# UofgCoastline/EUSIPCO-2026-Robust-Unet

Measured on AMD Instinct MI355X. Metric: train images/sec Robust U-Net 256x256 bs16/GPU, higher is better.
Workload: dtype f32; 1 GPU; Robust U-Net base64 (40.9M params) train step, 256x256 RGB+mask tiles, batch 16/GPU, fp32, BCE + Adam(lr 1e-4, wd 1e-4), dropout + batch-stat BN on; global_batch=16, image_size=256, parallelism=dp1

## Files before the change

eusipco-2026-robust-unet_amd/blocks.py:

```python
from __future__ import annotations

import os

import torch

from . import ops
from ._lib import check, lib

BN_EPS = 1e-5
BN_MOMENTUM = 0.1


class Small:

    CHUNK = 1 << 16

    def __init__(self, device):
        self.device = device
        self.buf = None
        self.off = 0

    def _take(self, n, dtype):
        n4 = (n + 3) // 4 * 4
        if n4 > self.CHUNK:
# ... 38 lines not shown

    def __init__(self, device):
        self.device = device
        self.g = {}

    def buf(self, prefix, items):
        total = sum(_numel(sh) for _, sh in items)
        flat = torch.empty(total, device=self.device, dtype=torch.float32)
        off = 0
        for name, sh in items:
            n = _numel(sh)
            self.g[prefix + name] = flat[off:off + n].view(sh)
            off += n
        return flat


def _numel(shape):
    n = 1
    for d in shape:
        n *= d
    return n


class BNState:
    __slots__ = ("weight", "bias", "running_mean", "running_var", "nbt")

    def __init__(self, weight, bias, running_mean, running_var, nbt):
        self.weight, self.bias, self.running_mean, self.running_var, self.nbt = weight, bias, running_mean, running_var, nbt


FUSED_BN_STATS = os.environ.get("RUNET_BN_STATS_3", "0") != "1"


def bn_coeff(x, bn: BNState, training, sm: Small, want_minmax=False, stats_hook=None, fused=None):
    n, h, w, c = x.shape
    hw = h * w
    st = ops.stream()
    scale, shift, mean, invstd = sm.f(c), sm.f(c), sm.f(c), sm.f(c)
    nc = None
    if training and not want_minmax and stats_hook is None and FUSED_BN_STATS and fused and "part" in fused:
        check(lib.runet_bn_stats_finalize(fused["part"].data_ptr(), fused["nparts"], c, bn.weight.data_ptr(), bn.bias.data_ptr(),
                                          bn.running_mean.data_ptr(), bn.running_var.data_ptr(), bn.nbt.data_ptr(), BN_MOMENTUM, BN_EPS,
                                          scale.data_ptr(), shift.data_ptr(), mean.data_ptr(), invstd.data_ptr(), st))
        return scale, shift, mean, invstd, None
    if training and not want_minmax and stats_hook is None and FUSED_BN_STATS:
        check(lib.runet_bn_stats(x.data_ptr(), ops.ld(x), n, hw, c, _ws(n, hw, c, x.device).data_ptr(), bn.weight.data_ptr(), bn.bias.data_ptr(),
                                 bn.running_mean.data_ptr(), bn.running_var.data_ptr(), bn.nbt.data_ptr(), BN_MOMENTUM, BN_EPS,
                                 scale.data_ptr(), shift.data_ptr(), mean.data_ptr(), invstd.data_ptr(), st))
        return scale, shift, mean, invstd, None
    if training or want_minmax:
        mean_nc, m2_nc = sm.f(n * c), sm.f(n * c)
        if want_minmax:
            max_nc, min_nc, imax, imin = sm.f(n * c), sm.f(n * c), sm.i(n * c), sm.i(n * c)
            nc = (mean_nc, m2_nc, max_nc, min_nc, imax, imin)
        ws = _ws(n, hw, c, x.device)
        check(lib.runet_chan_stats(x.data_ptr(), ops.ld(x), n, hw, c, ws.data_ptr(), mean_nc.data_ptr(), m2_nc.data_ptr(),
                                   nc[2].data_ptr() if nc else None, nc[3].data_ptr() if nc else None,
                                   nc[4].data_ptr() if nc else None, nc[5].data_ptr() if nc else None, int(want_minmax), st))
        mean_all, m2_all, n_eff = mean_nc, m2_nc, n
        if stats_hook is not None and training:
            mean_all, m2_all, n_eff = stats_hook.gather_stats(mean_nc, m2_nc, n, c)
    if training:
        check(lib.runet_bn_finalize(mean_all.data_ptr(), m2_all.data_ptr(), n_eff, c, hw, bn.weight.data_ptr(), bn.bias.data_ptr(),
                                    bn.running_mean.data_ptr(), bn.running_var.data_ptr(), bn.nbt.data_ptr(), BN_MOMENTUM, BN_EPS, 1,
                                    scale.data_ptr(), shift.data_ptr(), mean.data_ptr(), invstd.data_ptr(), st))
    else:
        check(lib.runet_bn_finalize(None, None, n, c, hw, bn.weight.data_ptr(), bn.bias.data_ptr(), bn.running_mean.data_ptr(),
                                    bn.running_var.data_ptr(), None, BN_MOMENTUM, BN_EPS, 0, scale.data_ptr(), shift.data_ptr(),
                                    mean.data_ptr(), invstd.data_ptr(), st))
    return scale, shift, mean, invstd, nc


def bn_coeff_pair(xa, bna: BNState, xb, bnb: BNState, training, sm: Small, stats_hook=None):
    if stats_hook is None or not training:
        return bn_coeff(xa, bna, training, sm)[:4], bn_coeff(xb, bnb, training, sm)[:4]
    st = ops.stream()
    local = []
    for x in (xa, xb):
        n, h, w, c = x.shape
        mean_nc, m2_nc = sm.f(n * c), sm.f(n * c)
        check(lib.runet_chan_stats(x.data_ptr(), ops.ld(x), n, h * w, c, _ws(n, h * w, c, x.device).data_ptr(), mean_nc.data_ptr(), m2_nc.data_ptr(),
                                   None, None, None, None, 0, st))
        local.append((mean_nc, m2_nc, n, c))
    res = []
    for x, bn, (mean_all, m2_all, n_eff) in zip((xa, xb), (bna, bnb), stats_hook.gather_stats_many(local)):
        n, h, w, c = x.shape
        scale, shift, mean, invstd = sm.f(c), sm.f(c), sm.f(c), sm.f(c)
        check(lib.runet_bn_finalize(mean_all.data_ptr(), m2_all.data_ptr(), n_eff, c, h * w, bn.weight.data_ptr(), bn.bias.data_ptr(),
                                    bn.running_mean.data_ptr(), bn.running_var.data_ptr(), bn.nbt.data_ptr(), BN_MOMENTUM, BN_EPS, 1,
                                    scale.data_ptr(), shift.data_ptr(), mean.data_ptr(), invstd.data_ptr(), st))
        res.append((scale, shift, mean, invstd))
    return res[0], res[1]


def bn_apply(x, scale, shift, mask=None, relu=False, out=None):
    n, h, w, c = x.shape
    if out is None:
        out = ops.empty_nhwc(n, h, w, c, x)
    check(lib.runet_bn_apply(x.data_ptr(), ops.ld(x), out.data_ptr(), ops.ld(out), n * h * w, h * w, c, scale.data_ptr(), shift.data_ptr(),
                             mask.data_ptr() if mask is not None else None, int(relu), ops.stream()))
    return out


def bn_bwd_reduce(dy, x, mean, invstd, scale, sums, act=None, mask=None, relu_shift=None):
    n, h, w, c = x.shape
    hw = h * w
    if relu_shift is not None:
        act = None
    actp, lda = (act.data_ptr(), ops.ld(act)) if act is not None else (None, 0)
    rsc, rsh = (scale.data_ptr(), relu_shift.data_ptr()) if relu_shift is not None else (None, None)
    check(lib.runet_bn_bwd_reduce(dy.data_ptr(), ops.ld(dy), x.data_ptr(), ops.ld(x), actp, lda, n, hw, c, mean.data_ptr(), invstd.data_ptr(),
                                  mask.data_ptr() if mask is not None else None, _ws(n, hw, c, x.device).data_ptr(), sums.data_ptr(), rsc, rsh,
                                  ops.stream()))


def bn_bwd_apply(dy, x, mean, invstd, scale, use, m_total, act=None, mask=None, out=None, relu_shift=None):
    n, h, w, c = x.shape
    hw = h * w
    if relu_shift is not None:
        act = None
    actp, lda = (act.data_ptr(), ops.ld(act)) if act is not None else (None, 0)
    if out is None:
        out = ops.empty_nhwc(n, h, w, c, x)
    check(lib.runet_bn_bwd_apply(dy.data_ptr(), ops.ld(dy), x.data_ptr(), ops.ld(x), actp, lda, out.data_ptr(), ops.ld(out), n * hw, hw, c,
                                 mean.data_ptr(), invstd.data_ptr(), scale.data_ptr(), use.data_ptr(), mask.data_ptr() if mask is not None else None,
                                 m_total, relu_shift.data_ptr() if relu_shift is not None else None, ops.stream()))
    return out


def dx_sums(sums, training, sync=None, count=0):
    if not training:
        return zeros(sums.numel(), sums.device), 0
    return (sums, 0) if sync is None else sync.reduce_sums(sums, count)


def bn_backward(dy, x, mean, invstd, scale, sums, act=None, mask=None, out=None, sync=None, relu_shift=None, training=True):
    n, h, w, c = x.shape
    bn_bwd_reduce(dy, x, mean, invstd, scale, sums, act, mask, relu_shift)
    use, m_total = dx_sums(sums, training, sync, n * h * w)
    return bn_bwd_apply(dy, x, mean, invstd, scale, use, m_total, act, mask, out, relu_shift)


CHAN_SUM_ON_SIDE = os.environ.get("RUNET_CHAN_SUM_MAIN", "0") != "1"
FUSED_SHORTCUT_BN_SUMS = os.environ.get("RUNET_FUSED_SHORTCUT_BN_SUMS", "0") == "1"
FUSED_GATE_BN_SUMS = os.environ.get("RUNET_NO_FUSED_GATE_BN_SUMS", "0") != "1"
FUSED_RB_EDGES = os.environ.get("RUNET_NO_FUSED_RB_EDGES", "0") != "1"
RB_EDGE_PARTS = frozenset(("out", "bwd1", "bwd3"))


def _edge(part):
    return FUSED_RB_EDGES and part in RB_EDGE_PARTS


def chan_sum(x, out):
    n, h, w, c = x.shape

    def run():
        ws = _ws(n, h * w, c, x.device)
        check(lib.runet_chan_sum(x.data_ptr(), ops.ld(x), n * h * w, c, ws.data_ptr(), out.data_ptr(), 0, ops.stream()))
        return out
    if CHAN_SUM_ON_SIDE and ops.side_stream() is not None:
        return ops._on_side(run, (x, out))
    return run()


def vec(n, device):
    return torch.empty(n, device=device, dtype=torch.float32)


def _ptr(t):
    return t.data_ptr() if t is not None else None


def conv_bn_coeff(x, w, bias, bn: BNState, training, sm: Small, stride=1, stats=True, save=True):
    fs = None
    if stride == 1:
        fs = {} if (stats and training) else None
        t = ops.conv_fwd(x, w, bias, stats=fs)
    else:
        t = ops.conv_general_fwd(x, w, bias, stride, w.shape[0] // 2)
    s, h, mean, invstd, _ = bn_coeff(t, bn, training, sm, fused=fs)
    return t, s, h, (dict(x=x, w=w, t=t, s=s, h=h, mean=mean, invstd=invstd, stride=stride) if save else None)


def conv_bn_relu_forward(x, w, bias, bn: BNState, training, sm: Small, stride=1, stats=True, save=True, out=None):
    t, s, h, cx = conv_bn_coeff(x, w, bias, bn, training, sm, stride, stats, save)
    return bn_apply(t, s, h, None, relu=True, out=out), cx


def conv_bn_relu_backward(cx, dy, G, seq, i, training, out=None):
    k, _, cin_w, c = cx["w"].shape
    sums = vec(2 * c, dy.device)
    dt = bn_backward(dy, cx["t"], cx["mean"], cx["invstd"], cx["s"], sums, relu_shift=cx["h"], out=out, training=training)
    G[f"{seq}.{i + 1}.weight"], G[f"{seq}.{i + 1}.bias"] = sums[:c], sums[c:]
    if cx["stride"] == 1:
        G[f"{seq}.{i}.weight"] = ops.conv_wgrad(cx["x"], dt, k, k, cin_w=cin_w)
    else:
        G[f"{seq}.{i}.weight"] = ops.conv_general_wgrad(cx["x"], dt, k, k, cx["stride"], k // 2, cin_w=cin_w)
    G[f"{seq}.{i}.bias"] = chan_sum(dt, vec(c, dy.device))
    return dt


class RBParams:
    __slots__ = ("w1", "bn1", "w2", "bn2", "w0p", "w2p", "wsa", "ws", "bns", "cin_w")

    def __init__(self, w1, bn1, w2, bn2, w0p, w2p, wsa, ws=None, bns=None):
        self.w1, self.bn1, self.w2, self.bn2, self.w0p, self.w2p, self.wsa, self.ws, self.bns = w1, bn1, w2, bn2, w0p, w2p, wsa, ws, bns
        self.cin_w = w1.shape[2]


def rb_forward(x, p: RBParams, training, mask=None, save=True, stats_hook=None, pool=False):
    n, h, w, _ = x.shape
    c = p.w1.shape[3]
    cr = p.w0p.shape[3]
    hw, P = h * w, n * h * w
    st = ops.stream()
    sm = Small(x.device)
    kv1, kv2 = ({}, {}) if save else (None, None)
    t1, br, fstem = None, None, (None, None)
    if p.ws is not None:
        if ops._stem_case(x.shape[3], p.cin_w, c, 3) and p.ws.shape[2] == p.cin_w:
            fstem = ({}, {}) if (training and stats_hook is None) else (None, None)
            t1, r = ops.stem_conv(x, p.w1, p.ws, stats3=fstem[0], stats1=fstem[1])
            if stats_hook is None:
                ss, hs, mean_s, invstd_s, _ = bn_coeff(r, p.bns, training, sm, fused=fstem[1])
        elif stats_hook is not None:
            r = ops.conv_fwd(x, p.ws)
        else:
            sm.f(4)
            r = ops.main_pool(ops.empty_nhwc(n, h, w, c, x))
            br = ops.side_branch(stats_hook is None)
            with br:
                fs = {} if training else None
                ops.conv_fwd(x, p.ws, out=r, stats=fs)
                ss, hs, mean_s, invstd_s, _ = bn_coeff(r, p.bns, training, sm, fused=fs)
    else:
        r, ss, hs, mean_s, invstd_s = x, None, None, None, None
    f1 = {} if (training and stats_hook is None) else None
    if t1 is None:
        t1 = ops.conv_fwd(x, p.w1, keep_v=kv1, stats=f1)
    elif fstem[0]:
        f1 = fstem[0]
    if p.ws is not None and stats_hook is not None:
        (ss, hs, mean_s, invstd_s), (s1, h1, mean1, invstd1) = bn_coeff_pair(r, p.bns, t1, p.bn1, training, sm, stats_hook)
    else:
        s1, h1, mean1, invstd1, _ = bn_coeff(t1, p.bn1, training, sm, stats_hook=stats_hook, fused=f1)
    use_mask = mask if training else None
    if ops.fuses_act_input(t1, p.w2):
        a1 = None
        t2 = ops.conv_fwd(t1, p.w2, keep_v=kv2, pre=(s1, h1, use_mask))
    else:
        a1 = bn_apply(t1, s1, h1, use_mask, relu=True)
        t2 = ops.conv_fwd(a1, p.w2, keep_v=kv2)
    if not save:
        del t1
    s2, h2, mean2, invstd2, nc = bn_coeff(t2, p.bn2, training, sm, want_minmax=True, stats_hook=stats_hook)
    mean_nc, _, max_nc, min_nc, imax, imin = nc
    A, B, ca, avg, mx, tval = (sm.f(n * c) for _ in range(6))
    idx = sm.i(n * c)
    check(lib.runet_ca_coeff(mean_nc.data_ptr(), max_nc.data_ptr(), min_nc.data_ptr(), imax.data_ptr(), imin.data_ptr(), s2.data_ptr(),
                             h2.data_ptr(), p.w0p.data_ptr(), p.w2p.data_ptr(), n, c, cr, A.data_ptr(), B.data_ptr(), ca.data_ptr(),
                             avg.data_ptr(), mx.data_ptr(), idx.data_ptr(), tval.data_ptr(), st))
    smap = torch.empty((P, 2), device=x.device, dtype=torch.float32)
    amax = torch.empty(P, device=x.device, dtype=torch.int32)
    check(lib.runet_sa_reduce(t2.data_ptr(), ops.ld(t2), A.data_ptr(), B.data_ptr(), P, hw, c, smap.data_ptr(), amax.data_ptr(), st))
    sa = torch.empty(P, device=x.device, dtype=torch.float32)
    check(lib.runet_sa_conv7(smap.data_ptr(), p.wsa.data_ptr(), sa.data_ptr(), n, h, w, st))
    out = ops.empty_nhwc(n, h, w, c, x)
    if br is not None:
        br.join(r)
    relu_bits = pooled = pool_idx = None
    if _edge("out"):
        if save and _edge("bwd1"):
            relu_bits = torch.empty((P, c // 4), device=x.device, dtype=torch.uint8)
        if pool:
            pooled = ops.empty_nhwc(n, h // 2, w // 2, c, x)
            pool_idx = torch.empty((n, h // 2, w // 2, c), device=x.device, dtype=torch.uint8)
    check(lib.runet_rb_out_ex(t2.data_ptr(), ops.ld(t2), A.data_ptr(), B.data_ptr(), sa.data_ptr(), r.data_ptr(), ops.ld(r), _ptr(ss), _ptr(hs),
                              out.data_ptr(), ops.ld(out), _ptr(relu_bits), _ptr(pooled), ops.ld(pooled) if pooled is not None else 0, _ptr(pool_idx),
                              n, h, w, c, st))
    if pool and pooled is None:
        pooled, pool_idx = maxpool_forward(out)
    if not save:
        return (out, None, pooled, pool_idx) if pool else (out, None)
    ctx = dict(x=x, r=r, t1=t1, a1=a1, t2=t2, out=out, mask=use_mask, p=p, training=training, sync=stats_hook if training else None, s1=s1, h1=h1, mean1=mean1, invstd1=invstd1, s2=s2, h2=h2,
               mean2=mean2, invstd2=invstd2, ss=ss, mean_s=mean_s, invstd_s=invstd_s, A=A, B=B, ca=ca, avg=avg, mx=mx, idx=idx,
               tval=tval, mean_nc=mean_nc, smap=smap, amax=amax, sa=sa, v1=kv1.get("V"), v2=kv2.get("V"), relu_bits=relu_bits, pool_idx=pool_idx)
    return (out, ctx, pooled, pool_idx) if pool else (out, ctx)


def rb_a1(ctx):
    if ctx["a1"] is not None:
        return ctx["a1"]
    return bn_apply(ctx["t1"], ctx["s1"], ctx["h1"], ctx["mask"], relu=True)


def rb_backward(ctx, dout, sink, pre="", need_dx=True, dpool=None, pool_idx=None):
    p: RBParams = ctx["p"]
    x, r, t1, a1, t2, out = ctx["x"], ctx["r"], ctx["t1"], ctx["a1"], ctx["t2"], ctx["out"]
    n, h, w, c = out.shape
    cr = p.w0p.shape[3]
    hw, P = h * w, n * h * w
    st = ops.stream()
    dev = x.device
    sm = Small(dev)
    A, B, sa, smap, amax = ctx["A"], ctx["B"], ctx["sa"], ctx["smap"], ctx["amax"]
    dv = ops.empty_nhwc(n, h, w, c, x)
    dq = torch.empty(P, device=dev, dtype=torch.float32)
    relu_bits = ctx.get("relu_bits") if _edge("bwd1") else None
    if dpool is not None and not _edge("bwd1"):
        dout, dpool = maxpool_backward(dpool, pool_idx, dx=dout), None
    check(lib.runet_rb_bwd1_ex(dout.data_ptr(), ops.ld(dout), _ptr(dpool), ops.ld(dpool) if dpool is not None else 0,
                               pool_idx.data_ptr() if dpool is not None else None, out.data_ptr(), ops.ld(out), _ptr(relu_bits), t2.data_ptr(),
                               ops.ld(t2), A.data_ptr(), B.data_ptr(), sa.data_ptr(), dv.data_ptr(), ops.ld(dv), dq.data_ptr(), n, h, w, c, st))
    dsm = torch.empty((P, 2), device=dev, dtype=torch.float32)
    dwsa = sink.buf(pre, [("sa.conv1.weight", (7, 7, 2, 1))])
    ws = scratch(lib.runet_sa_conv7_bwd_workspace_floats(n, h, w), dev)
    check(lib.runet_sa_conv7_bwd(smap.data_ptr(), dq.data_ptr(), p.wsa.data_ptr(), dsm.data_ptr(), dwsa.data_ptr(), ws.data_ptr(), n, h, w, st))
    sdu, sdut = sm.f(n * c), sm.f(n * c)
    sync, tr = ctx["sync"], ctx["training"]
    has_sc = p.ws is not None
    synced = sync is not None and tr
    sc_bwd3 = has_sc and tr and _edge("bwd3")
    sc_sums = None if not has_sc else "bwd2" if (FUSED_SHORTCUT_BN_SUMS and not synced) else "early" if (synced or sc_bwd3) else "late"
    sums_s = sink.buf(pre, [("shortcut.1.weight", (c,)), ("shortcut.1.bias", (c,))]) if has_sc else None

    def sc_reduce():
        bn_bwd_reduce(dv, r, ctx["mean_s"], ctx["invstd_s"], ctx["ss"], sums_s)

    if sc_sums == "bwd2":
        ws = scratch(lib.runet_rb_bwd2_bn_workspace_floats(n, hw, c), dev)
        check(lib.runet_rb_bwd2_bn(dv.data_ptr(), ops.ld(dv), t2.data_ptr(), ops.ld(t2), sa.data_ptr(), dsm.data_ptr(), amax.data_ptr(), r.data_ptr(),
                                   ops.ld(r), ctx["mean_s"].data_ptr(), ctx["invstd_s"].data_ptr(), n, hw, c, ws.data_ptr(), ws.numel(),
                                   sdu.data_ptr(), sdut.data_ptr(), sums_s.data_ptr(), st))
    else:
        ws = _ws(n, hw, c, dev)
        check(lib.runet_rb_bwd2(dv.data_ptr(), ops.ld(dv), t2.data_ptr(), ops.ld(t2), sa.data_ptr(), dsm.data_ptr(), amax.data_ptr(), n, hw, c,
                                ws.data_ptr(), sdu.data_ptr(), sdut.data_ptr(), st))
    davg, dmx = sm.f(n * c), sm.f(n * c)
    sums2 = sink.buf(pre, [("bn2.weight", (c,)), ("bn2.bias", (c,))])
    dw0p = sink.buf(pre, [("ca.fc.0.weight", (1, 1, c, cr))])
    dw2p = sink.buf(pre, [("ca.fc.2.weight", (1, 1, cr, c))])
    ws = scratch(lib.runet_ca_bwd_workspace_floats(n, c, cr), dev)
    check(lib.runet_ca_bwd(sdu.data_ptr(), sdut.data_ptr(), ctx["s2"].data_ptr(), ctx["h2"].data_ptr(), ctx["ca"].data_ptr(),
                           ctx["avg"].data_ptr(), ctx["mx"].data_ptr(), p.w0p.data_ptr(), p.w2p.data_ptr(), ctx["mean_nc"].data_ptr(),
                           ctx["tval"].data_ptr(), ctx["mean2"].data_ptr(), ctx["invstd2"].data_ptr(), n, c, cr, ws.data_ptr(),
                           davg.data_ptr(), dmx.data_ptr(), sums2.data_ptr(), dw0p.data_ptr(), dw2p.data_ptr(), st))
    dt2 = ops.empty_nhwc(n, h, w, c, x)
    if sc_sums == "early":
        sc_reduce()
    if has_sc and synced:
        (use2, m_total), (use_s, m_s) = sync.reduce_sums_many([sums2, sums_s], [P, P])
    else:
        use2, m_total = dx_sums(sums2, tr, sync, P)
        use_s, m_s = dx_sums(sums_s, tr) if has_sc else (None, 0)
    if sc_bwd3:
        check(lib.runet_rb_bwd3_sc(dv.data_ptr(), ops.ld(dv), t2.data_ptr(), ops.ld(t2), sa.data_ptr(), dsm.data_ptr(), amax.data_ptr(),
                                   ctx["ca"].data_ptr(), davg.data_ptr(), dmx.data_ptr(), ctx["idx"].data_ptr(), ctx["mean2"].data_ptr(),
                                   ctx["invstd2"].data_ptr(), ctx["s2"].data_ptr(), use2.data_ptr(), dt2.data_ptr(), ops.ld(dt2), r.data_ptr(),
                                   ops.ld(r), ctx["mean_s"].data_ptr(), ctx["invstd_s"].data_ptr(), ctx["ss"].data_ptr(), use_s.data_ptr(), m_s,
                                   P, hw, c, m_total, st))
    else:
        check(lib.runet_rb_bwd3(dv.data_ptr(), ops.ld(dv), t2.data_ptr(), ops.ld(t2), sa.data_ptr(), dsm.data_ptr(), amax.data_ptr(),
                                ctx["ca"].data_ptr(), davg.data_ptr(), dmx.data_ptr(), ctx["idx"].data_ptr(), ctx["mean2"].data_ptr(),
                                ctx["invstd2"].data_ptr(), ctx["s2"].data_ptr(), use2.data_ptr(), dt2.data_ptr(), ops.ld(dt2), P, hw, c, m_total, st))
    kz = {}
    da1 = ops.conv_dgrad(dt2, p.w2, keep_z=kz)
    if a1 is None:
        assert ctx.get("v2") is not None, "conv2 took its activation on the fly: its weight gradient needs the kept V"
        a1 = t1
    ops.conv_wgrad(a1, dt2, 3, 3, out=sink.buf(pre, [("conv2.weight", (3, 3, c, c))]), v=ctx.get("v2"), z=kz.get("Z"))
    ctx["v2"] = None
    del dt2, kz
    sums1 = sink.buf(pre, [("bn1.weight", (c,)), ("bn1.bias", (c,))])
    kz1, dx1 = {}, None
    fused_dt1 = need_dx and p.cin_w == x.shape[3] and ops.fuses_bn_bwd_input(da1, p.w1)
    if fused_dt1:
        bn_bwd_reduce(da1, t1, ctx["mean1"], ctx["invstd1"], ctx["s1"], sums1, None, ctx["mask"], ctx["h1"])
        use1, m1 = dx_sums(sums1, tr, sync, P)
        bn1 = dict(x=t1, mean=ctx["mean1"], invstd=ctx["invstd1"], scale=ctx["s1"], shift=ctx["h1"], sums=use1, m_total=m1, mask=ctx["mask"])
        if p.ws is not None:
            dx1 = ops.conv_dgrad(da1, p.w1, keep_z=kz1, bn=bn1)
        else:
            dx1 = ops.conv_dgrad(da1, p.w1, out=dv, accumulate=True, keep_z=kz1, bn=bn1)
        dt1 = da1
    else:
        dt1 = bn_backward(da1, t1, ctx["mean1"], ctx["invstd1"], ctx["s1"], sums1, mask=ctx["mask"], out=da1, sync=sync, relu_shift=ctx["h1"], training=tr)
        if need_dx and p.ws is not None:
            dx1 = ops.conv_dgrad(dt1, p.w1, keep_z=kz1)
    ops.conv_wgrad(x, dt1, 3, 3, cin_w=p.cin_w, out=sink.buf(pre, [("conv1.weight", (3, 3, p.cin_w, c))]), v=ctx.get("v1"), on_side=need_dx,
                   z=kz1.get("Z"))
    ctx["v1"] = None
    dx = None
    if has_sc:
        if sc_sums == "late":
            sc_reduce()
        dr = dv if sc_bwd3 else bn_bwd_apply(dv, r, ctx["mean_s"], ctx["invstd_s"], ctx["ss"], use_s, m_s, out=dv)
        ops.conv_wgrad(x, dr, 1, 1, cin_w=p.cin_w, out=sink.buf(pre, [("shortcut.0.weight", (1, 1, p.cin_w, c))]))
        if need_dx:
            dx = dx1
            ops.conv_dgrad(dr, p.ws, out=dx, accumulate=True)
    elif need_dx:
        dx = dv
        if not fused_dt1:
            ops.conv_dgrad(dt1, p.w1, out=dx, accumulate=True)
    return dx


def _consts(n, c, P, dev):
    one_c, zero_c = torch.ones(max(2 * c, n * c), device=dev), zeros(max(2 * c, n * c), dev)
    return one_c, zero_c


def ca_forward(x, w0p, w2p, save=True):
    n, h, w, c = x.shape
    cr = w0p.shape[3]
    dev, st = x.device, ops.stream()
    sm = Small(dev)
    mean_nc, m2_nc, max_nc, min_nc = sm.f(n * c), sm.f(n * c), sm.f(n * c), sm.f(n * c)
    imax, imin, idx = sm.i(n * c), sm.i(n * c), sm.i(n * c)
    check(lib.runet_chan_stats(x.data_ptr(), ops.ld(x), n, h * w, c, _ws(n, h * w, c, dev).data_ptr(), mean_nc.data_ptr(), m2_nc.data_ptr(),
                               max_nc.data_ptr(), min_nc.data_ptr(), imax.data_ptr(), imin.data_ptr(), 1, st))
    one, zero = _consts(n, c, 0, dev)
    A, B, ca, avg, mx, tval = (sm.f(n * c) for _ in range(6))
    check(lib.runet_ca_coeff(mean_nc.data_ptr(), max_nc.data_ptr(), min_nc.data_ptr(), imax.data_ptr(), imin.data_ptr(), one.data_ptr(),
                             zero.data_ptr(), w0p.data_ptr(), w2p.data_ptr(), n, c, cr, A.data_ptr(), B.data_ptr(), ca.data_ptr(), avg.data_ptr(),
                             mx.data_ptr(), idx.data_ptr(), tval.data_ptr(), st))
    y = bn_apply(x, one, zero, ca, relu=False)
    return y, (dict(x=x, w0p=w0p, w2p=w2p, ca=ca, avg=avg, mx=mx, idx=idx, tval=tval, mean_nc=mean_nc) if save else None)


def ca_backward(ctx, dy, sink, pre=""):
    x, w0p, w2p = ctx["x"], ctx["w0p"], ctx["w2p"]
    n, h, w, c = x.shape
    cr = w0p.shape[3]
    hw, P = h * w, n * h * w
    dev, st = x.device, ops.stream()
    sm = Small(dev)
    one, zero = _consts(n, c, P, dev)
    ones_p = torch.ones(P, device=dev)
    zeros_p2 = torch.zeros((P, 2), device=dev)
    none_p = torch.full((P,), -1, device=dev, dtype=torch.int32)
    sdu, sdut, davg, dmx = sm.f(n * c), sm.f(n * c), sm.f(n * c), sm.f(n * c)
    check(lib.runet_rb_bwd2(dy.data_ptr(), ops.ld(dy), x.data_ptr(), ops.ld(x), ones_p.data_ptr(), zeros_p2.data_ptr(), none_p.data_ptr(), n, hw, c,
                            _ws(n, hw, c, dev).data_ptr(), sdu.data_ptr(), sdut.data_ptr(), st))
    dw0p = sink.buf(pre, [("fc.0.weight", (1, 1, c, cr))])
    dw2p = sink.buf(pre, [("fc.2.weight", (1, 1, cr, c))])
    sums = sm.f(2 * c)
    ws = scratch(lib.runet_ca_bwd_workspace_floats(n, c, cr), dev)
    check(lib.runet_ca_bwd(sdu.data_ptr(), sdut.data_ptr(), one.data_ptr(), zero.data_ptr(), ctx["ca"].data_ptr(), ctx["avg"].data_ptr(),
                           ctx["mx"].data_ptr(), w0p.data_ptr(), w2p.data_ptr(), ctx["mean_nc"].data_ptr(), ctx["tval"].data_ptr(), zero.data_ptr(),
                           one.data_ptr(), n, c, cr, ws.data_ptr(), davg.data_ptr(), dmx.data_ptr(), sums.data_ptr(), dw0p.data_ptr(), dw2p.data_ptr(), st))
    dx = ops.empty_nhwc(n, h, w, c, x)
    check(lib.runet_rb_bwd3(dy.data_ptr(), ops.ld(dy), x.data_ptr(), ops.ld(x), ones_p.data_ptr(), zeros_p2.data_ptr(), none_p.data_ptr(),
                            ctx["ca"].data_ptr(), davg.data_ptr(), dmx.data_ptr(), ctx["idx"].data_ptr(), zero.data_ptr(), one.data_ptr(), one.data_ptr(),
                            zero.data_ptr(), dx.data_ptr(), ops.ld(dx), P, hw, c, 0, st))
    return dx


def sa_forward(x, wsa, save=True):
    n, h, w, c = x.shape
    P = n * h * w
    dev, st = x.device, ops.stream()
    one, zero = _consts(n, c, P, dev)
    smap = torch.empty((P, 2), device=dev, dtype=torch.float32)
    amax = torch.empty(P, device=dev, dtype=torch.int32)
    check(lib.runet_sa_reduce(x.data_ptr(), ops.ld(x), one.data_ptr(), zero.data_ptr(), P, h * w, c, smap.data_ptr(), amax.data_ptr(), st))
# ... 184 lines not shown
    xb = gate_x_branch(skip, p, training, sm, stats_hook)
    ops.convt_fwd(y, p.wup, p.bup, out=up)
    gc = gate_forward(up, skip, p, training, cat[..., :c], sm, stats_hook, xb=xb)
    if not save:
        return cat, None
    gc.update(y=y, skip=skip, cat=cat, p=p)
    return cat, gc


def upgate_backward(ctx, dcat, sink, pre_att, pre_up):
    p: UpGateParams = ctx["p"]
    y, skip, cat = ctx["y"], ctx["skip"], ctx["cat"]
    c = skip.shape[3]
    cin = y.shape[3]
    up, dup, datt = cat[..., c:], dcat[..., c:], dcat[..., :c]
    dskip = gate_backward(ctx, up, skip, p, datt, dup, sink, pre=pre_att)
    up_b = sink.buf(pre_up, [("weight", (2, 2, cin, c)), ("bias", (c,))])
    ops.convt_wgrad(y, dup, out=up_b[:4 * cin * c])
    chan_sum(dup, up_b[4 * cin * c:])
    dy = ops.convt_dgrad(dup, p.wup)
    return dy, dskip


def maxpool_forward(x):
    n, h, w, c = x.shape
    y = ops.empty_nhwc(n, h // 2, w // 2, c, x)
    idx = torch.empty((n, h // 2, w // 2, c), device=x.device, dtype=torch.uint8)
    check(lib.runet_maxpool2_fwd(x.data_ptr(), ops.ld(x), y.data_ptr(), ops.ld(y), idx.data_ptr(), n, h, w, c, ops.stream()))
    return y, idx


def maxpool_backward(dy, idx, dx=None):
    n, ho, wo, c = dy.shape
    acc = dx is not None
    if dx is None:
        dx = ops.empty_nhwc(n, 2 * ho, 2 * wo, c, dy)
    check(lib.runet_maxpool2_bwd(dy.data_ptr(), ops.ld(dy), idx.data_ptr(), dx.data_ptr(), ops.ld(dx), n, 2 * ho, 2 * wo, c, int(acc), ops.stream()))
    return dx


def bn_relu_maxpool_forward(t, scale, shift):
    n, h, w, c = t.shape
    y = ops.empty_nhwc(n, h // 2, w // 2, c, t)
    idx = torch.empty((n, h // 2, w // 2, c), device=t.device, dtype=torch.uint8)
    check(lib.runet_bn_relu_maxpool2_fwd(t.data_ptr(), ops.ld(t), scale.data_ptr(), shift.data_ptr(), y.data_ptr(), ops.ld(y), idx.data_ptr(), n, h, w,
                                         c, ops.stream()))
    return y, idx


def bn_backward_pooled(dpool, idx, x, mean, invstd, scale, sums, relu_shift, training=True):
    n, h, w, c = x.shape
    st = ops.stream()
    check(lib.runet_bn_bwd_reduce_pooled(dpool.data_ptr(), ops.ld(dpool), idx.data_ptr(), x.data_ptr(), ops.ld(x), n, h, w, c, mean.data_ptr(),
                                         invstd.data_ptr(), _ws(n, h * w, c, x.device).data_ptr(), sums.data_ptr(), scale.data_ptr(),
                                         relu_shift.data_ptr(), st))
    use = dx_sums(sums, training)[0]
    dx = ops.empty_nhwc(n, h, w, c, x)
    check(lib.runet_bn_bwd_apply_pooled(dpool.data_ptr(), ops.ld(dpool), idx.data_ptr(), x.data_ptr(), ops.ld(x), dx.data_ptr(), ops.ld(dx), n, h, w, c,
                                        mean.data_ptr(), invstd.data_ptr(), scale.data_ptr(), use.data_ptr(), 0, relu_shift.data_ptr(), st))
    return dx


FUSED_LEAKY_POOL = os.environ.get("RUNET_NO_FUSED_LEAKY_POOL", "0") != "1"


def bn_apply_leaky(x, scale, shift, slope, out=None):
    n, h, w, c = x.shape
    if out is None:
        out = ops.empty_nhwc(n, h, w, c, x)
    check(lib.runet_bn_apply_leaky(x.data_ptr(), ops.ld(x), out.data_ptr(), ops.ld(out), n * h * w, h * w, c, scale.data_ptr(), shift.data_ptr(),
                                   float(slope), ops.stream()))
    return out


def bn_backward_leaky(dy, x, mean, invstd, scale, sums, shift, slope, training=True, out=None):
    n, h, w, c = x.shape
    hw = h * w
    st = ops.stream()
    check(lib.runet_bn_bwd_reduce_leaky(dy.data_ptr(), ops.ld(dy), x.data_ptr(), ops.ld(x), n, hw, c, mean.data_ptr(), invstd.data_ptr(),
                                        _ws(n, hw, c, x.device).data_ptr(), sums.data_ptr(), scale.data_ptr(), shift.data_ptr(), float(slope), st))
    use = dx_sums(sums, training)[0]
    if out is None:
        out = ops.empty_nhwc(n, h, w, c, x)
    check(lib.runet_bn_bwd_apply_leaky(dy.data_ptr(), ops.ld(dy), x.data_ptr(), ops.ld(x), out.data_ptr(), ops.ld(out), n * hw, hw, c,
                                       mean.data_ptr(), invstd.data_ptr(), scale.data_ptr(), use.data_ptr(), 0, shift.data_ptr(), float(slope), st))
    return out


def bn_leaky_maxpool_forward(t, scale, shift, slope):
    n, h, w, c = t.shape
    if not FUSED_LEAKY_POOL:
        return maxpool_forward(bn_apply_leaky(t, scale, shift, slope))
    y = ops.empty_nhwc(n, h // 2, w // 2, c, t)
    idx = torch.empty((n, h // 2, w // 2, c), device=t.device, dtype=torch.uint8)
    check(lib.runet_bn_leaky_maxpool2_fwd(t.data_ptr(), ops.ld(t), scale.data_ptr(), shift.data_ptr(), float(slope), y.data_ptr(), ops.ld(y),
                                          idx.data_ptr(), n, h, w, c, ops.stream()))
    return y, idx


def bn_backward_pooled_leaky(dpool, idx, x, mean, invstd, scale, sums, shift, slope, training=True):
    if not FUSED_LEAKY_POOL:
        return bn_backward_leaky(maxpool_backward(dpool, idx), x, mean, invstd, scale, sums, shift, slope, training=training)
    n, h, w, c = x.shape
    st = ops.stream()
    check(lib.runet_bn_bwd_reduce_pooled_leaky(dpool.data_ptr(), ops.ld(dpool), idx.data_ptr(), x.data_ptr(), ops.ld(x), n, h, w, c, mean.data_ptr(),
                                               invstd.data_ptr(), _ws(n, h * w, c, x.device).data_ptr(), sums.data_ptr(), scale.data_ptr(),
                                               shift.data_ptr(), float(slope), st))
    use = dx_sums(sums, training)[0]
    dx = ops.empty_nhwc(n, h, w, c, x)
    check(lib.runet_bn_bwd_apply_pooled_leaky(dpool.data_ptr(), ops.ld(dpool), idx.data_ptr(), x.data_ptr(), ops.ld(x), dx.data_ptr(), ops.ld(dx), n,
                                              h, w, c, mean.data_ptr(), invstd.data_ptr(), scale.data_ptr(), use.data_ptr(), 0, shift.data_ptr(),
                                              float(slope), st))
    return dx


def maxunpool_forward(x, idx):
    return maxpool_backward(x, idx)


def maxunpool_backward(du, idx):
    n, h, w, c = du.shape
    dp = ops.empty_nhwc(n, h // 2, w // 2, c, du)
    check(lib.runet_maxunpool2_bwd(du.data_ptr(), ops.ld(du), idx.data_ptr(), dp.data_ptr(), ops.ld(dp), n, h, w, c, ops.stream()))
    return dp


def to_nhwc_pad(x_nchw, c_pad):
    n, c, h, w = x_nchw.shape
    y = torch.empty((n, h, w, c_pad), device=x_nchw.device, dtype=torch.float32)
    sn, sc, sh, sw = x_nchw.stride()
    check(lib.runet_to_nhwc_pad(x_nchw.data_ptr(), sn, sc, sh, sw, y.data_ptr(), n, c, h, w, c_pad, ops.stream()))
    return y


def outc_forward(x, w, b, want_logit=False):
    n, h, wd, c = x.shape
    prob = torch.empty((n, 1, h, wd), device=x.device, dtype=torch.float32)
    logit = torch.empty((n, 1, h, wd), device=x.device, dtype=torch.float32) if want_logit else None
    check(lib.runet_outc_fwd(x.data_ptr(), ops.ld(x), w.data_ptr(), b.data_ptr(), logit.data_ptr() if want_logit else None, prob.data_ptr(),
                             n * h * wd, c, ops.stream()))
    return prob, logit


def outc_backward(dprob, prob, x, w, sink, pre=""):
    n, h, wd, c = x.shape
    dx = ops.empty_nhwc(n, h, wd, c, x)
    dw_db = sink.buf(pre, [("weight", (1, 1, c, 1)), ("bias", (1,))])
    ws = _ws(n, h * wd, c, x.device)
    check(lib.runet_outc_bwd(dprob.data_ptr(), prob.data_ptr(), x.data_ptr(), ops.ld(x), w.data_ptr(), dx.data_ptr(), ops.ld(dx), ws.data_ptr(),
                             dw_db.data_ptr(), n * h * wd, c, ops.stream()))
    return dx


FUSED_HR_HEAD = os.environ.get("RUNET_NO_FUSED_HR_HEAD", "0") != "1"
FUSED_BN_UPSAMPLE = os.environ.get("RUNET_NO_FUSED_BN_UPSAMPLE", "0") != "1"


def _bilinear_nhwc(x, out):
    n, h, w, c = x.shape
    check(lib.runet_bilinear_nhwc_fwd(x.data_ptr(), ops.ld(x), out.data_ptr(), ops.ld(out), n, h, w, out.shape[1], out.shape[2], c, ops.stream()))
    return out


def _bilinear_nhwc_backward(dy, h, w):
    n, ho, wo, c = dy.shape
    dx = ops.empty_nhwc(n, h, w, c, dy)
    check(lib.runet_bilinear_nhwc_bwd(dy.data_ptr(), ops.ld(dy), dx.data_ptr(), ops.ld(dx), n, h, w, ho, wo, c, ops.stream()))
    return dx


def hr_head_forward(t, scale, shift, w, b, fused=None):
    n, h, wd, c = t.shape
    st = ops.stream()
    if FUSED_HR_HEAD if fused is None else fused:
        z = torch.empty((n, h, wd), device=t.device, dtype=torch.float32)
        prob = torch.empty((n, 1, 2 * h, 2 * wd), device=t.device, dtype=torch.float32)
        check(lib.runet_hr_head_fwd(t.data_ptr(), ops.ld(t), scale.data_ptr(), shift.data_ptr(), w.data_ptr(), b.data_ptr(), z.data_ptr(), n, h, wd, c, st))
        check(lib.runet_up2_sigmoid_fwd(z.data_ptr(), prob.data_ptr(), n, h, wd, st))
        return prob, None
    a = bn_apply(t, scale, shift, None, relu=True)
    up = _bilinear_nhwc(a, ops.empty_nhwc(n, 2 * h, 2 * wd, c, t))
    prob, _ = outc_forward(up, w, b)
    return prob, (a, up)


def hr_head_backward(dprob, prob, t, scale, shift, w, mean, invstd, saved=None, training=True):
    n, h, wd, c = t.shape
    dev = t.device
    st = ops.stream()
    out = torch.empty(3 * c + 1, device=dev, dtype=torch.float32)
    if saved is None:
        dz = torch.empty((n, h, wd), device=dev, dtype=torch.float32)
        check(lib.runet_up2_sigmoid_bwd(dprob.data_ptr(), prob.data_ptr(), dz.data_ptr(), n, h, wd, st))
        ws = scratch(lib.runet_hr_head_bwd_workspace_floats(n, h, wd, c), dev)
        check(lib.runet_hr_head_bwd_reduce(dz.data_ptr(), t.data_ptr(), ops.ld(t), scale.data_ptr(), shift.data_ptr(), w.data_ptr(), mean.data_ptr(),
                                           invstd.data_ptr(), ws.data_ptr(), ws.numel(), out.data_ptr(), n, h, wd, c, st))
        use = dx_sums(out, training)[0]
        dt = ops.empty_nhwc(n, h, wd, c, t)
        check(lib.runet_hr_head_bwd_apply(dz.data_ptr(), t.data_ptr(), ops.ld(t), w.data_ptr(), dt.data_ptr(), ops.ld(dt), n, h, wd, c, mean.data_ptr(),
                                          invstd.data_ptr(), scale.data_ptr(), shift.data_ptr(), use.data_ptr(), 0, st))
        return dt, out
    a, up = saved
    dup = ops.empty_nhwc(n, 2 * h, 2 * wd, c, t)
    check(lib.runet_outc_bwd(dprob.data_ptr(), prob.data_ptr(), up.data_ptr(), ops.ld(up), w.data_ptr(), dup.data_ptr(), ops.ld(dup),
                             _ws(n, 4 * h * wd, c, dev).data_ptr(), out[2 * c:].data_ptr(), n * 4 * h * wd, c, st))
    da = _bilinear_nhwc_backward(dup, h, wd)
    dt = bn_backward(da, t, mean, invstd, scale, out[:2 * c], relu_shift=shift, out=da, training=training)
    return dt, out


def bn_bilinear_forward(x, scale, shift, out, s, fused=None):
    n, h, w, c = x.shape
    if tuple(out.shape) != (n, s * h, s * w, c):
        raise ValueError(f"bn_bilinear_forward: out {tuple(out.shape)} is not {s} x {tuple(x.shape)}")
    if FUSED_BN_UPSAMPLE if fused is None else fused:
        check(lib.runet_bn_bilinear_nhwc_fwd(x.data_ptr(), ops.ld(x), out.data_ptr(), ops.ld(out), scale.data_ptr(), shift.data_ptr(), n, h, w, s, c,
                                             ops.stream()))
        return out
    return _bilinear_nhwc(bn_apply(x, scale, shift), out)


def bn_bilinear_backward(dy, x, mean, invstd, scale, sums, s, training=True, fused=None):
    n, h, w, c = x.shape
    if not (FUSED_BN_UPSAMPLE if fused is None else fused):
        g = _bilinear_nhwc_backward(dy, h, w)
        return bn_backward(g, x, mean, invstd, scale, sums, out=g, training=training)
    g = ops.empty_nhwc(n, h, w, c, x)
    ws = scratch(lib.runet_bilinear_nhwc_bwd_sums_workspace_floats(n, h, w, c), x.device)
    check(lib.runet_bilinear_nhwc_bwd_sums(dy.data_ptr(), ops.ld(dy), x.data_ptr(), ops.ld(x), mean.data_ptr(), invstd.data_ptr(), g.data_ptr(), ops.ld(g),
                                           ws.data_ptr(), ws.numel(), sums.data_ptr(), n, h, w, s, c, ops.stream()))
    use = dx_sums(sums, training)[0]
    return bn_bwd_apply(g, x, mean, invstd, scale, use, 0, out=g)



FUSED_WATER_INDEX = os.environ.get("RUNET_NO_FUSED_WATER_INDEX", "0") != "1"
WI_MID, WI_OUT = 16, 4


class WaterIndexParams:
    __slots__ = ("w1", "b1", "bn", "w2", "b2")

    def __init__(self, w1, b1, bn, w2, b2):
        self.w1, self.b1, self.bn, self.w2, self.b2 = w1, b1, bn, w2, b2


def _wi_src(x):
    n, c, h, w = x.shape
    if c != 3 or x.dtype != torch.float32:
        raise ValueError("water_index: expected a float32 image [N, 3, H, W]")
    return (x.data_ptr(),) + tuple(x.stride()) + (n, h, w)


def _wi_coef(p: WaterIndexParams):
    return (p.w1.data_ptr(), p.b1.data_ptr()), (p.w2.data_ptr(), p.b2.data_ptr())


def water_index_forward(x_nchw, p: WaterIndexParams, training, sm: Small, fused=None):
    n, _, h, w = x_nchw.shape
    dev, st = x_nchw.device, ops.stream()
    src = _wi_src(x_nchw)
    bn = p.bn
    buf = torch.empty((n, h, w, 8), device=dev, dtype=torch.float32)
    if FUSED_WATER_INDEX if fused is None else fused:
        c1, c2 = _wi_coef(p)
        scale, shift, mean, invstd = sm.f(WI_MID), sm.f(WI_MID), sm.f(WI_MID), sm.f(WI_MID)
        if training:
            nparts = lib.runet_water_index_parts(n, h, w)
            part = scratch(nparts * WI_MID * 3, dev)
            check(lib.runet_water_index_stats(*src, *c1, part.data_ptr(), part.numel(), st))
            check(lib.runet_bn_stats_finalize(part.data_ptr(), nparts, WI_MID, bn.weight.data_ptr(), bn.bias.data_ptr(), bn.running_mean.data_ptr(),
                                              bn.running_var.data_ptr(), bn.nbt.data_ptr(), BN_MOMENTUM, BN_EPS, scale.data_ptr(), shift.data_ptr(),
                                              mean.data_ptr(), invstd.data_ptr(), st))
        else:
            check(lib.runet_bn_finalize(None, None, n, WI_MID, h * w, bn.weight.data_ptr(), bn.bias.data_ptr(), bn.running_mean.data_ptr(),
                                        bn.running_var.data_ptr(), None, BN_MOMENTUM, BN_EPS, 0, scale.data_ptr(), shift.data_ptr(),
                                        mean.data_ptr(), invstd.data_ptr(), st))
        check(lib.runet_water_index_fwd(*src, *c1, scale.data_ptr(), shift.data_ptr(), *c2, buf.data_ptr(), 8, st))
        return buf, dict(x=x_nchw, p=p, scale=scale, shift=shift, mean=mean, invstd=invstd, training=training, fused=True)
    P = n * h * w
    x4 = to_nhwc_pad(x_nchw, 4)
    z = ops.conv_fwd(x4, p.w1, p.b1)
    scale, shift, mean, invstd, _ = bn_coeff(z, bn, training, sm)
    a = bn_apply(z, scale, shift, None, relu=True)
    u = ops.conv_fwd(a, p.w2, p.b2)
    check(lib.runet_copy_nhwc(x4.data_ptr(), 4, buf.data_ptr(), 8, P, 3, st))
    check(lib.runet_sigmoid_nhwc_fwd(u.data_ptr(), WI_OUT, buf[..., 3:].data_ptr(), 8, P, WI_OUT, st))
    check(lib.runet_copy_nhwc(x4[..., 3:].data_ptr(), 4, buf[..., 7:].data_ptr(), 8, P, 1, st))
    return buf, dict(x4=x4, z=z, a=a, buf=buf, p=p, scale=scale, shift=shift, mean=mean, invstd=invstd, training=training, fused=False)


def water_index_backward(ctx, g):
    p: WaterIndexParams = ctx["p"]
    n, h, w, c = g.shape
    if c != WI_OUT:
        raise ValueError("water_index_backward: g must have 4 channels")
    dev, st = g.device, ops.stream()
    ldg = ops.ld(g)
    training = ctx["training"]
    out_red = torch.empty(2 * WI_MID + WI_MID * WI_OUT + WI_OUT, device=dev, dtype=torch.float32)
    out_app = torch.empty(4 * WI_MID, device=dev, dtype=torch.float32)
    scale, shift, mean, invstd = ctx["scale"], ctx["shift"], ctx["mean"], ctx["invstd"]
    if ctx["fused"]:
        src = _wi_src(ctx["x"])
        c1, c2 = _wi_coef(p)
        ws = scratch(lib.runet_water_index_workspace_floats(n, h, w), dev)
# ... 635 lines not shown
```

eusipco-2026-robust-unet_amd/csrc/attention.hip:

```cpp
#include "runet_common.h"
#include "../../include/runet_hip.h"
#include <float.h>

namespace {
constexpr int TPB = 256;
constexpr int LPP = 16;
constexpr int PPB = TPB / LPP;

__device__ __forceinline__ float grp_sum16(float v) {
#pragma unroll
    for (int o = 8; o > 0; o >>= 1) v += __shfl_xor(v, o, 64);
    return v;
}

__device__ __forceinline__ void ca_hidden(const float* __restrict__ W0p, const float* avg, const float* mxv, int C, int Cr, float* hid,
                                          float* part ) {
    const int tid = threadIdx.x, TPB = blockDim.x;
    const int P = TPB / Cr;
    const int j = tid % Cr, pt = tid / Cr;
    float pa = 0.f, pm = 0.f;
    if (pt < P)
        for (int c = pt; c < C; c += P) {
            const float w = W0p[c * Cr + j];
            pa += w * avg[c];
            pm += w * mxv[c];
        }
    part[tid] = pa; part[TPB + tid] = pm;
    __syncthreads();
    for (int o = tid; o < 2 * Cr; o += TPB) {
        const float* src = part + (o < Cr ? 0 : TPB) + (o % Cr);
        float acc = 0.f;
        for (int q = 0; q < P; ++q) acc += src[q * Cr];
        hid[o] = acc;
    }
}

constexpr int CA_TPB = 1024;

__global__ __launch_bounds__(CA_TPB) void ca_coeff_kernel(const float* __restrict__ mean_nc, const float* __restrict__ max_nc,
                                                       const float* __restrict__ min_nc, const int* __restrict__ imax_nc,
                                                       const int* __restrict__ imin_nc, const float* __restrict__ s2,
                                                       const float* __restrict__ h2, const float* __restrict__ W0p,
                                                       const float* __restrict__ W2p, int C, int Cr, float* __restrict__ A,
                                                       float* __restrict__ B, float* __restrict__ ca_out, float* __restrict__ avg_out,
                                                       float* __restrict__ mx_out, int* __restrict__ idx_out, float* __restrict__ tval_out) {
    extern __shared__ __attribute__((aligned(16))) float sm[];
    float* avg = sm;
    float* mxv = sm + C;
    float* hid = sm + 2 * C;
    const int n = blockIdx.x, tid = threadIdx.x, TPB = blockDim.x;
    for (int c = tid; c < C; c += TPB) {
        const float s = s2[c], h = h2[c];
        const bool pos = s >= 0.f;
        const float tv = pos ? max_nc[n * C + c] : min_nc[n * C + c];
        avg[c] = s * mean_nc[n * C + c] + h;
        mxv[c] = s * tv + h;
        if (avg_out) { avg_out[n * C + c] = avg[c]; mx_out[n * C + c] = mxv[c]; idx_out[n * C + c] = pos ? imax_nc[n * C + c] : imin_nc[n * C + c]; tval_out[n * C + c] = tv; }
    }
    __syncthreads();
    ca_hidden(W0p, avg, mxv, C, Cr, hid, sm + 2 * C + 2 * Cr);
    __syncthreads();
    for (int c = tid; c < C; c += TPB) {
        float za = 0.f, zm = 0.f;
        for (int j = 0; j < Cr; ++j) {
            za += W2p[j * C + c] * fmaxf(hid[j], 0.f);
            zm += W2p[j * C + c] * fmaxf(hid[Cr + j], 0.f);
        }
        const float ca = sigmoidf_(za + zm);
        A[n * C + c] = s2[c] * ca;
        B[n * C + c] = h2[c] * ca;
        if (ca_out) ca_out[n * C + c] = ca;
    }
}

__global__ __launch_bounds__(TPB) void sa_reduce_kernel(const float* __restrict__ t2, int ld, const float* __restrict__ A,
                                                        const float* __restrict__ B, long P, int HW, int C,
                                                        float* __restrict__ smap, int* __restrict__ amax) {
    const int sub = threadIdx.x & (LPP - 1);
    for (long p = (long)blockIdx.x * PPB + (threadIdx.x / LPP); p < P; p += (long)gridDim.x * PPB) {
        const int n = (int)(p / HW);
        const float* a = A + (long)n * C;
        const float* b = B + (long)n * C;
        float s = 0.f, m = -FLT_MAX;
        int im = 0;
        for (int c = sub * 4; c < C; c += LPP * 4) {
            const f32x4 t = *reinterpret_cast<const f32x4*>(t2 + p * ld + c);
            const f32x4 av = *reinterpret_cast<const f32x4*>(a + c);
            const f32x4 bv = *reinterpret_cast<const f32x4*>(b + c);
#pragma unroll
            for (int q = 0; q < 4; ++q) {
                const float u = t[q] * av[q] + bv[q];
                s += u;
                if (u > m) { m = u; im = c + q; }
            }
        }
        s = grp_sum16(s);
#pragma unroll
        for (int o = 8; o > 0; o >>= 1) {
            const float om = __shfl_xor(m, o, 64);
            const int oi = __shfl_xor(im, o, 64);
            if (om > m || (om == m && oi < im)) { m = om; im = oi; }
        }
        if (sub == 0) {
            smap[p * 2] = s / (float)C;
            smap[p * 2 + 1] = m;
            amax[p] = im;
        }
    }
}

__global__ __launch_bounds__(256) void sa_conv7_kernel(const float* __restrict__ smap, const float* __restrict__ Wp,
                                                       float* __restrict__ sa, int H, int W) {
    __shared__ float tile[22][22][2];
    __shared__ float wsm[98];
    const int tx = threadIdx.x & 15, ty = threadIdx.x >> 4;
    const int n = blockIdx.z, h0 = blockIdx.y * 16, w0 = blockIdx.x * 16;
    if (threadIdx.x < 98) wsm[threadIdx.x] = Wp[threadIdx.x];
    for (int i = threadIdx.x; i < 22 * 22; i += 256) {
        const int r = i / 22, c = i % 22;
        const int h = h0 + r - 3, w = w0 + c - 3;
        float a = 0.f, b = 0.f;
        if ((unsigned)h < (unsigned)H && (unsigned)w < (unsigned)W) {
            const long p = ((long)n * H + h) * W + w;
            a = smap[p * 2]; b = smap[p * 2 + 1];
        }
        tile[r][c][0] = a; tile[r][c][1] = b;
    }
    __syncthreads();
    const int h = h0 + ty, w = w0 + tx;
    if (h < H && w < W) {
        float q = 0.f;
#pragma unroll
        for (int dy = 0; dy < 7; ++dy)
#pragma unroll
            for (int dx = 0; dx < 7; ++dx)
                q += wsm[(dy * 7 + dx) * 2] * tile[ty + dy][tx + dx][0] + wsm[(dy * 7 + dx) * 2 + 1] * tile[ty + dy][tx + dx][1];
        sa[((long)n * H + h) * W + w] = sigmoidf_(q);
    }
}

__device__ __forceinline__ unsigned int relu_bits4(const f32x4 o) {
    return (o[0] > 0.f ? 1u : 0u) | (o[1] > 0.f ? 2u : 0u) | (o[2] > 0.f ? 4u : 0u) | (o[3] > 0.f ? 8u : 0u);
}
#define RB_EDGE_WAVES __attribute__((amdgpu_waves_per_eu(8, 8)))
template <bool BITS>
__device__ __forceinline__ void rb_out_body(const float* t2, int ld, const float* A, const float* B, const float* sa, const float* r, int ldr,
                                            const float* rs, const float* rh, float* out, int ldo, unsigned char* bits, int HW, int C,
                                            int pix_per_chunk) {
    const int cvec = C / 4, rows = TPB / cvec, tid = threadIdx.x;
    const int col = tid % cvec, row = tid / cvec;
    if (row >= rows) return;
    const int n = blockIdx.y, c = col * 4;
    const int p0 = blockIdx.x * pix_per_chunk, p1 = min(HW, p0 + pix_per_chunk);
    const f32x4 a = *reinterpret_cast<const f32x4*>(A + (long)n * C + c);
    const f32x4 b = *reinterpret_cast<const f32x4*>(B + (long)n * C + c);
    f32x4 s4 = {1.f, 1.f, 1.f, 1.f}, h4 = {0.f, 0.f, 0.f, 0.f};
    if (rs) { s4 = *reinterpret_cast<const f32x4*>(rs + c); h4 = *reinterpret_cast<const f32x4*>(rh + c); }
    const long ib = (long)n * HW;
    for (int p = p0 + row; p < p1; p += rows) {
        const f32x4 t = *reinterpret_cast<const f32x4*>(t2 + (ib + p) * ld + c);
        const f32x4 res = *reinterpret_cast<const f32x4*>(r + (ib + p) * ldr + c) * s4 + h4;
        const float s = sa[ib + p];
        f32x4 o = (t * a + b) * s + res;
#pragma unroll
        for (int q = 0; q < 4; ++q) o[q] = fmaxf(o[q], 0.f);
        *reinterpret_cast<f32x4*>(out + (ib + p) * ldo + c) = o;
        if constexpr (BITS) bits[(ib + p) * cvec + col] = (unsigned char)relu_bits4(o);
    }
}
__global__ __launch_bounds__(TPB) void rb_out_kernel(const float* __restrict__ t2, int ld, const float* __restrict__ A,
                                                     const float* __restrict__ B, const float* __restrict__ sa,
                                                     const float* __restrict__ r, int ldr, const float* __restrict__ rs,
                                                     const float* __restrict__ rh, float* __restrict__ out, int ldo, int HW, int C,
                                                     int pix_per_chunk) {
    rb_out_body<false>(t2, ld, A, B, sa, r, ldr, rs, rh, out, ldo, nullptr, HW, C, pix_per_chunk);
}
__global__ __launch_bounds__(TPB) void rb_out_bits_kernel(const float* __restrict__ t2, int ld, const float* __restrict__ A,
                                                          const float* __restrict__ B, const float* __restrict__ sa,
                                                          const float* __restrict__ r, int ldr, const float* __restrict__ rs,
                                                          const float* __restrict__ rh, float* __restrict__ out, int ldo,
                                                          unsigned char* __restrict__ bits, int HW, int C, int pix_per_chunk) {
    rb_out_body<true>(t2, ld, A, B, sa, r, ldr, rs, rh, out, ldo, bits, HW, C, pix_per_chunk);
}
template <bool BITS>
__global__ __launch_bounds__(TPB) RB_EDGE_WAVES void rb_out_pool_kernel(const float* __restrict__ t2, int ld, const float* __restrict__ A,
                                                          const float* __restrict__ B, const float* __restrict__ sa,
                                                          const float* __restrict__ r, int ldr, const float* __restrict__ rs,
                                                          const float* __restrict__ rh, float* __restrict__ out, int ldo,
                                                          unsigned char* __restrict__ bits, float* __restrict__ pooled, int ldp,
                                                          unsigned char* __restrict__ pool_idx, int HW, int W, int C, int pix_per_chunk) {
    const int cvec = C / 4, rows = TPB / cvec, tid = threadIdx.x;
    const int col = tid % cvec, row = tid / cvec;
    if (row >= rows) return;
    const int n = blockIdx.y, c = col * 4;
    const int HWo = HW >> 2, Wo = W >> 1;
    const int q0 = blockIdx.x * pix_per_chunk, q1 = min(HWo, q0 + pix_per_chunk);
    const f32x4 a = *reinterpret_cast<const f32x4*>(A + (long)n * C + c);
    const f32x4 b = *reinterpret_cast<const f32x4*>(B + (long)n * C + c);
    f32x4 s4 = {1.f, 1.f, 1.f, 1.f}, h4 = {0.f, 0.f, 0.f, 0.f};
    if (rs) { s4 = *reinterpret_cast<const f32x4*>(rs + c); h4 = *reinterpret_cast<const f32x4*>(rh + c); }
    const long ib = (long)n * HW, ibo = (long)n * HWo;
    for (int q = q0 + row; q < q1; q += rows) {
        const int ho = q / Wo, wo = q - ho * Wo;
        const long pb = ib + (long)(ho * 2) * W + wo * 2;
        f32x4 m;
        unsigned int sel[4] = {0, 0, 0, 0};
#pragma unroll
        for (int kr = 0; kr < 4; kr += 2) {
            const long pr = pb + (kr >> 1) * W;
            f32x4 t[2], res[2];
            float s[2];
#pragma unroll
            for (int j = 0; j < 2; ++j) {
                t[j] = *reinterpret_cast<const f32x4*>(t2 + (pr + j) * ld + c);
                res[j] = *reinterpret_cast<const f32x4*>(r + (pr + j) * ldr + c);
                s[j] = sa[pr + j];
            }
#pragma unroll
            for (int j = 0; j < 2; ++j) {
                const int k = kr + j;
                f32x4 o = (t[j] * a + b) * s[j] + (res[j] * s4 + h4);
#pragma unroll
                for (int e = 0; e < 4; ++e) o[e] = fmaxf(o[e], 0.f);
                *reinterpret_cast<f32x4*>(out + (pr + j) * ldo + c) = o;
                if constexpr (BITS) bits[(pr + j) * cvec + col] = (unsigned char)relu_bits4(o);
                if (k == 0) m = o;
                else {
#pragma unroll
                    for (int e = 0; e < 4; ++e)
                        if (o[e] > m[e] || o[e] != o[e]) { m[e] = o[e]; sel[e] = k; }
                }
            }
        }
        *reinterpret_cast<f32x4*>(pooled + (ibo + q) * ldp + c) = m;
        *reinterpret_cast<unsigned int*>(pool_idx + (ibo + q) * C + c) = sel[0] | (sel[1] << 8) | (sel[2] << 16) | (sel[3] << 24);
    }
}

template <bool POOL, bool BITS>
__global__ __launch_bounds__(TPB) RB_EDGE_WAVES void rb_bwd1_ex_kernel(const float* __restrict__ dout, int lddo, const float* __restrict__ dpool, int ldp,
                                                         const unsigned char* __restrict__ pidx, const float* __restrict__ out, int ldo,
                                                         const unsigned char* __restrict__ bits, const float* __restrict__ t2, int ld,
                                                         const float* __restrict__ A, const float* __restrict__ B,
                                                         const float* __restrict__ sa, float* __restrict__ dv, int lddv,
                                                         float* __restrict__ dq, int HW, int W, int C) {
    const int sub = threadIdx.x & (LPP - 1);
    const int cvec = C / 4;
    const int n = blockIdx.y;
    for (int pi = blockIdx.x * PPB + (threadIdx.x / LPP); pi < HW; pi += gridDim.x * PPB) {
        const long p = (long)n * HW + pi;
        long pq = 0;
        unsigned int pk = 0;
        if constexpr (POOL) {
            const int hh = pi / W, ww = pi - hh * W;
            pq = (long)n * (HW >> 2) + (long)(hh >> 1) * (W >> 1) + (ww >> 1);
            pk = (unsigned)((hh & 1) * 2 + (ww & 1));
        }
        float s = 0.f;
        for (int c = sub * 4; c < C; c += LPP * 4) {
            f32x4 g = *reinterpret_cast<const f32x4*>(dout + p * lddo + c);
            if constexpr (POOL) g += pooled_grad4_at(dpool, ldp, pidx, C, pq, pk, c);
            f32x4 o = {1.f, 1.f, 1.f, 1.f};
            unsigned int m = 0xfu;
            if constexpr (BITS) m = bits[p * cvec + (c >> 2)];
            else if (out) o = *reinterpret_cast<const f32x4*>(out + p * ldo + c);
            const f32x4 t = *reinterpret_cast<const f32x4*>(t2 + p * ld + c);
            const f32x4 a = *reinterpret_cast<const f32x4*>(A + (long)n * C + c);
            const f32x4 b = *reinterpret_cast<const f32x4*>(B + (long)n * C + c);
            f32x4 d;
#pragma unroll
            for (int q = 0; q < 4; ++q) {
                const bool on = BITS ? ((m >> q) & 1u) != 0u : o[q] > 0.f;
                d[q] = on ? g[q] : 0.f;
                s += d[q] * (t[q] * a[q] + b[q]);
            }
            *reinterpret_cast<f32x4*>(dv + p * lddv + c) = d;
        }
        s = grp_sum16(s);
        if (sub == 0) {
            const float v = sa[p];
            dq[p] = s * v * (1.f - v);
        }
    }
}

__global__ __launch_bounds__(256) void sa_conv7_bwd_kernel(const float* __restrict__ smap, const float* __restrict__ dq,
                                                           const float* __restrict__ Wp, float* __restrict__ dsm,
                                                           float* __restrict__ dw_part, int H, int W) {
    __shared__ float dqt[22][22];
    __shared__ float smt[22][22][2];
    __shared__ float wsm[98];
    const int tx = threadIdx.x & 15, ty = threadIdx.x >> 4;
    const int n = blockIdx.z, h0 = blockIdx.y * 16, w0 = blockIdx.x * 16;
    if (threadIdx.x < 98) wsm[threadIdx.x] = Wp[threadIdx.x];
    for (int i = threadIdx.x; i < 22 * 22; i += 256) {
        const int r = i / 22, c = i % 22;
        const int h = h0 + r - 3, w = w0 + c - 3;
        float d = 0.f, a = 0.f, b = 0.f;
        if ((unsigned)h < (unsigned)H && (unsigned)w < (unsigned)W) {
            const long p = ((long)n * H + h) * W + w;
            d = dq[p]; a = smap[p * 2]; b = smap[p * 2 + 1];
        }
        dqt[r][c] = d; smt[r][c][0] = a; smt[r][c][1] = b;
    }
    __syncthreads();
    const int h = h0 + ty, w = w0 + tx;
    if (h < H && w < W) {
        float g0 = 0.f, g1 = 0.f;
#pragma unroll
        for (int dy = 0; dy < 7; ++dy)
#pragma unroll
            for (int dx = 0; dx < 7; ++dx) {
                const float d = dqt[ty + 6 - dy][tx + 6 - dx];
                g0 += wsm[(dy * 7 + dx) * 2] * d;
                g1 += wsm[(dy * 7 + dx) * 2 + 1] * d;
            }
        const long p = ((long)n * H + h) * W + w;
        dsm[p * 2] = g0; dsm[p * 2 + 1] = g1;
    }
    if (threadIdx.x < 98) {
        const int ch = threadIdx.x & 1, k = threadIdx.x >> 1, dy = k / 7, dx = k % 7;
        float acc = 0.f;
        for (int y = 0; y < 16; ++y)
            for (int x = 0; x < 16; ++x) acc += smt[y + dy][x + dx][ch] * dqt[y + 3][x + 3];
        const long blk = ((long)blockIdx.z * gridDim.y + blockIdx.y) * gridDim.x + blockIdx.x;
        dw_part[blk * 98 + threadIdx.x] = acc;
    }
}
__device__ __forceinline__ double sum4(const double* red) { return red[0] + red[1] + red[2] + red[3]; }
__device__ __forceinline__ void col_sum_rows(const float* __restrict__ part, long nrows, int ncols, int col, double* red) {
    double acc = 0;
    for (long r = threadIdx.x; r < nrows; r += blockDim.x) acc += part[r * ncols + col];
    acc = wave_sum_d(acc);
    if ((threadIdx.x & 63) == 0) red[threadIdx.x >> 6] = acc;
    __syncthreads();
}
__global__ void reduce_rows_kernel(const float* __restrict__ part, long nrows, int ncols, float* __restrict__ out) {
    __shared__ double red[4];
    const int c = blockIdx.x;
    col_sum_rows(part, nrows, ncols, c, red);
    if (threadIdx.x == 0) out[c] = (float)sum4(red);
}

template <bool BN>
__global__ __launch_bounds__(TPB) void rb_bwd2_partial(const float* __restrict__ dv, int lddv, const float* __restrict__ t2, int ld,
                                                       const float* __restrict__ sa, const float* __restrict__ dsm,
                                                       const int* __restrict__ amax, int HW, int C, int pix_per_chunk,
                                                       float* __restrict__ part, const float* __restrict__ r, int ldr,
                                                       const float* __restrict__ mean_s, const float* __restrict__ invstd_s) {
    extern __shared__ __attribute__((aligned(16))) float sm[];
    constexpr int NV = BN ? 4 : 2;
    const int cvec = C / 4, rows = TPB / cvec, tid = threadIdx.x;
    const int col = tid % cvec, row = tid / cvec;
    const int n = blockIdx.y, chunk = blockIdx.x;
    const int p0 = chunk * pix_per_chunk, p1 = min(HW, p0 + pix_per_chunk);
    float s[4] = {0, 0, 0, 0}, st[4] = {0, 0, 0, 0}, sv[4] = {0, 0, 0, 0}, svr[4] = {0, 0, 0, 0};
    const float invC = 1.0f / (float)C;
    if (row < rows) {
        float ms[4], is[4];
        if constexpr (BN) {
#pragma unroll
            for (int q = 0; q < 4; ++q) { ms[q] = mean_s[col * 4 + q]; is[q] = invstd_s[col * 4 + q]; }
        }
        const long ib = (long)n * HW;
        for (int p = p0 + row; p < p1; p += rows) {
            const f32x4 d = *reinterpret_cast<const f32x4*>(dv + (ib + p) * lddv + col * 4);
            const f32x4 t = *reinterpret_cast<const f32x4*>(t2 + (ib + p) * ld + col * 4);
            f32x4 rr = {0.f, 0.f, 0.f, 0.f};
            if constexpr (BN) rr = *reinterpret_cast<const f32x4*>(r + (ib + p) * ldr + col * 4);
            const float v = sa[ib + p], g0 = dsm[(ib + p) * 2] * invC, g1 = dsm[(ib + p) * 2 + 1];
            const int am = amax[ib + p];
#pragma unroll
            for (int q = 0; q < 4; ++q) {
                const float du = d[q] * v + g0 + ((col * 4 + q) == am ? g1 : 0.f);
                s[q] += du;
                st[q] += du * t[q];
                if constexpr (BN) { sv[q] += d[q]; svr[q] += d[q] * ((rr[q] - ms[q]) * is[q]); }
            }
        }
#pragma unroll
        for (int q = 0; q < 4; ++q) {
            float* o = sm + (row * C + col * 4 + q) * NV;
            o[0] = s[q]; o[1] = st[q];
            if constexpr (BN) { o[2] = sv[q]; o[3] = svr[q]; }
        }
    }
    __syncthreads();
    for (int c = tid; c < C; c += TPB) {
        double a[NV];
#pragma unroll
        for (int j = 0; j < NV; ++j) a[j] = 0;
        for (int rw = 0; rw < rows; ++rw)
#pragma unroll
            for (int j = 0; j < NV; ++j) a[j] += sm[(rw * C + c) * NV + j];
        float* o = part + (((long)n * gridDim.x + chunk) * C + c) * NV;
#pragma unroll
        for (int j = 0; j < NV; ++j) o[j] = (float)a[j];
    }
}
__global__ void rb_bwd2_final(const float* __restrict__ part, int N, int C, int nchunks, int nv, float* __restrict__ sdu, float* __restrict__ sdut) {
    const int i = blockIdx.x * blockDim.x + threadIdx.x;
    if (i >= N * C) return;
    const int n = i / C, c = i - n * C;
    double a = 0, b = 0;
    for (int k = 0; k < nchunks; ++k) {
        const float* o = part + (((long)n * nchunks + k) * C + c) * nv;
        a += o[0]; b += o[1];
    }
    sdu[i] = (float)a; sdut[i] = (float)b;
}
__global__ void rb_bwd2_bn_final(const float* __restrict__ part, long nrows, int C, float* __restrict__ sums_s) {
    const int c = blockIdx.x;
    double a = 0, b = 0;
// ... 158 lines not shown
__global__ __launch_bounds__(TPB) RB_EDGE_WAVES void rb_bwd3_sc_kernel(float* dv, int lddv, const float* __restrict__ t2, int ld,
                                                         const float* __restrict__ sa, const float* __restrict__ dsm,
                                                         const int* __restrict__ amax, const float* __restrict__ ca,
                                                         const float* __restrict__ davg, const float* __restrict__ dmx,
                                                         const int* __restrict__ idx, const float* __restrict__ mean2,
                                                         const float* __restrict__ invstd2, const float* __restrict__ s2,
                                                         const float* __restrict__ sums2, float* __restrict__ dt2, int lddt, int HW, int C,
                                                         int pix_per_chunk, float inv_m, RbScArgs sc) {
    rb_bwd3_body<true>(dv, dv, lddv, t2, ld, sa, dsm, amax, ca, davg, dmx, idx, mean2, invstd2, s2, sums2, dt2, lddt, HW, C, pix_per_chunk, inv_m,
                       sc);
}

__global__ __launch_bounds__(TPB) void ag_psi_kernel(const float* __restrict__ g1, int ldg, const float* __restrict__ x1, int ldx,
                                                     const float* __restrict__ sg, const float* __restrict__ hg,
                                                     const float* __restrict__ sx, const float* __restrict__ hx,
                                                     const float* __restrict__ wpsi, const float* __restrict__ bpsi,
                                                     float* __restrict__ s, long P, int F) {
    const int sub = threadIdx.x & (LPP - 1);
    for (long p = (long)blockIdx.x * PPB + (threadIdx.x / LPP); p < P; p += (long)gridDim.x * PPB) {
        float acc = 0.f;
        for (int f = sub * 4; f < F; f += LPP * 4) {
            const f32x4 a = *reinterpret_cast<const f32x4*>(g1 + p * ldg + f);
            const f32x4 b = *reinterpret_cast<const f32x4*>(x1 + p * ldx + f);
#pragma unroll
            for (int q = 0; q < 4; ++q) {
                const float pre = a[q] * sg[f + q] + hg[f + q] + b[q] * sx[f + q] + hx[f + q];
                acc += wpsi[f + q] * fmaxf(pre, 0.f);
            }
        }
        acc = grp_sum16(acc);
        if (sub == 0) s[p] = acc + bpsi[0];
    }
}
__global__ __launch_bounds__(TPB) void ag_out_kernel(const float* __restrict__ xs, int ldx, const float* __restrict__ s,
                                                     const float* __restrict__ sp, const float* __restrict__ hp,
                                                     float* __restrict__ out, int ldo, long P, int C, long pix_per_chunk) {
    const int cvec = C / 4, rows = TPB / cvec, tid = threadIdx.x;
    const int col = tid % cvec, row = tid / cvec;
    if (row >= rows) return;
    const int c = col * 4;
    const long p0 = (long)blockIdx.x * pix_per_chunk;
    const long p1 = p0 + pix_per_chunk < P ? p0 + pix_per_chunk : P;
    const float a = sp[0], b = hp[0];
    for (long p = p0 + row; p < p1; p += rows) {
        const float sig = sigmoidf_(s[p] * a + b);
        *reinterpret_cast<f32x4*>(out + p * ldo + c) = *reinterpret_cast<const f32x4*>(xs + p * ldx + c) * sig;
    }
}

__global__ __launch_bounds__(TPB) void ag_bwd1_kernel(const float* __restrict__ datt, int ldd, const float* __restrict__ xs, int ldx,
                                                      const float* __restrict__ s, const float* __restrict__ sp,
                                                      const float* __restrict__ hp, float* __restrict__ dxs, int lddx,
                                                      float* __restrict__ dsbn, long P, int C) {
    const int sub = threadIdx.x & (LPP - 1);
    const float a = sp[0], b = hp[0];
    for (long p = (long)blockIdx.x * PPB + (threadIdx.x / LPP); p < P; p += (long)gridDim.x * PPB) {
        const float sig = sigmoidf_(s[p] * a + b);
        float acc = 0.f;
        for (int c = sub * 4; c < C; c += LPP * 4) {
            const f32x4 d = *reinterpret_cast<const f32x4*>(datt + p * ldd + c);
            const f32x4 x = *reinterpret_cast<const f32x4*>(xs + p * ldx + c);
            acc += d[0] * x[0] + d[1] * x[1] + d[2] * x[2] + d[3] * x[3];
            *reinterpret_cast<f32x4*>(dxs + p * lddx + c) = d * sig;
        }
        acc = grp_sum16(acc);
        if (sub == 0) dsbn[p] = acc * sig * (1.f - sig);
    }
}
template <bool BN>
__global__ __launch_bounds__(TPB) void ag_bwd2_partial(const float* __restrict__ ds, const float* __restrict__ g1, int ldg,
                                                       const float* __restrict__ x1, int ldx, const float* __restrict__ sg,
                                                       const float* __restrict__ hg, const float* __restrict__ sx,
                                                       const float* __restrict__ hx, const float* __restrict__ wpsi,
                                                       float* __restrict__ dpre, int ldp, long P, int F, long pix_per_chunk,
                                                       float* __restrict__ part, const float* __restrict__ mean_g,
                                                       const float* __restrict__ invstd_g, const float* __restrict__ mean_x,
                                                       const float* __restrict__ invstd_x) {
    extern __shared__ __attribute__((aligned(16))) float sm[];
    const int NC = BN ? 4 * F + 1 : F + 1;
    const int cvec = F / 4, rows = TPB / cvec, tid = threadIdx.x;
    const int col = tid % cvec, row = tid / cvec;
    const long p0 = (long)blockIdx.x * pix_per_chunk;
    const long p1 = p0 + pix_per_chunk < P ? p0 + pix_per_chunk : P;
    float sw[4] = {0, 0, 0, 0}, sb = 0.f;
    float so[4] = {0, 0, 0, 0}, sog[4] = {0, 0, 0, 0}, sox[4] = {0, 0, 0, 0};
    if (row < rows) {
        float a_g[4], b_g[4], a_x[4], b_x[4], wp[4], mg[4], ig[4], mx[4], ix[4];
#pragma unroll
        for (int q = 0; q < 4; ++q) {
            const int f = col * 4 + q;
            a_g[q] = sg[f]; b_g[q] = hg[f]; a_x[q] = sx[f]; b_x[q] = hx[f]; wp[q] = wpsi[f];
            if constexpr (BN) { mg[q] = mean_g[f]; ig[q] = invstd_g[f]; mx[q] = mean_x[f]; ix[q] = invstd_x[f]; }
        }
        for (long p = p0 + row; p < p1; p += rows) {
            const f32x4 a = *reinterpret_cast<const f32x4*>(g1 + p * ldg + col * 4);
            const f32x4 b = *reinterpret_cast<const f32x4*>(x1 + p * ldx + col * 4);
            const float d = ds[p];
            f32x4 o;
#pragma unroll
            for (int q = 0; q < 4; ++q) {
                const float pre = a[q] * a_g[q] + b_g[q] + b[q] * a_x[q] + b_x[q];
                o[q] = pre > 0.f ? d * wp[q] : 0.f;
                sw[q] += d * fmaxf(pre, 0.f);
                if constexpr (BN) {
                    so[q] += o[q];
                    sog[q] += o[q] * ((a[q] - mg[q]) * ig[q]);
                    sox[q] += o[q] * ((b[q] - mx[q]) * ix[q]);
                }
            }
            if (col == 0) sb += d;
            *reinterpret_cast<f32x4*>(dpre + p * ldp + col * 4) = o;
        }
#pragma unroll
        for (int q = 0; q < 4; ++q) {
            sm[row * NC + col * 4 + q] = sw[q];
            if constexpr (BN) {
                sm[row * NC + F + 1 + col * 4 + q] = sog[q];
                sm[row * NC + 2 * F + 1 + col * 4 + q] = so[q];
                sm[row * NC + 3 * F + 1 + col * 4 + q] = sox[q];
            }
        }
        if (col == 0) sm[row * NC + F] = sb;
    }
    __syncthreads();
    for (int c = tid; c < NC; c += TPB) {
        double a = 0;
        for (int r = 0; r < rows; ++r) a += sm[r * NC + c];
        part[(long)blockIdx.x * NC + c] = (float)a;
    }
}
__global__ void ag_bwd2_bn_final(const float* __restrict__ part, long nrows, int F, float* __restrict__ dwpsi_db, float* __restrict__ sums_g,
                                 float* __restrict__ sums_x) {
    __shared__ double red[4];
    const int c = blockIdx.x, NC = 4 * F + 1;
    col_sum_rows(part, nrows, NC, c, red);
    if (threadIdx.x == 0) {
        const float v = (float)sum4(red);
        if (c <= F) dwpsi_db[c] = v;
        else if (c < 2 * F + 1) sums_g[c - (F + 1)] = v;
        else if (c < 3 * F + 1) { sums_g[F + c - (2 * F + 1)] = v; sums_x[F + c - (2 * F + 1)] = v; }
        else sums_x[c - (3 * F + 1)] = v;
    }
}

__global__ __launch_bounds__(TPB) void outc_fwd_kernel(const float* __restrict__ x, int ld, const float* __restrict__ w,
                                                       const float* __restrict__ b, float* __restrict__ logit,
                                                       float* __restrict__ prob, long P, int C) {
    const int sub = threadIdx.x & (LPP - 1);
    for (long p = (long)blockIdx.x * PPB + (threadIdx.x / LPP); p < P; p += (long)gridDim.x * PPB) {
        float acc = 0.f;
        for (int c = sub * 4; c < C; c += LPP * 4) {
            const f32x4 v = *reinterpret_cast<const f32x4*>(x + p * ld + c);
            const f32x4 k = *reinterpret_cast<const f32x4*>(w + c);
            acc += v[0] * k[0] + v[1] * k[1] + v[2] * k[2] + v[3] * k[3];
        }
        acc = grp_sum16(acc);
        if (sub == 0) {
            const float l = acc + b[0];
            if (logit) logit[p] = l;
            prob[p] = sigmoidf_(l);
        }
    }
}
__global__ __launch_bounds__(TPB) void outc_bwd_partial(const float* __restrict__ dprob, const float* __restrict__ prob,
                                                        const float* __restrict__ x, int ld, const float* __restrict__ w,
                                                        float* __restrict__ dx, int lddx, long P, int C, long pix_per_chunk,
                                                        float* __restrict__ part) {
    extern __shared__ __attribute__((aligned(16))) float sm[];
    const int cvec = C / 4, rows = TPB / cvec, tid = threadIdx.x;
    const int col = tid % cvec, row = tid / cvec;
    const long p0 = (long)blockIdx.x * pix_per_chunk;
    const long p1 = p0 + pix_per_chunk < P ? p0 + pix_per_chunk : P;
    float sw[4] = {0, 0, 0, 0}, sb = 0.f;
    if (row < rows) {
        const f32x4 wv = *reinterpret_cast<const f32x4*>(w + col * 4);
        for (long p = p0 + row; p < p1; p += rows) {
            float dl = dprob[p];
            if (prob) {
                const float pr = prob[p];
                dl = dl * pr * (1.f - pr);
            }
            const f32x4 v = *reinterpret_cast<const f32x4*>(x + p * ld + col * 4);
#pragma unroll
            for (int q = 0; q < 4; ++q) sw[q] += dl * v[q];
            if (col == 0) sb += dl;
            *reinterpret_cast<f32x4*>(dx + p * lddx + col * 4) = wv * dl;
        }
#pragma unroll
        for (int q = 0; q < 4; ++q) sm[row * (C + 1) + col * 4 + q] = sw[q];
        if (col == 0) sm[row * (C + 1) + C] = sb;
    }
    __syncthreads();
    for (int c = tid; c < C + 1; c += TPB) {
        double a = 0;
        for (int r = 0; r < rows; ++r) a += sm[r * (C + 1) + c];
        part[(long)blockIdx.x * (C + 1) + c] = (float)a;
    }
}

inline int px_grid(long P) {
    long b = (P + PPB - 1) / PPB;
    if (b > 8192) b = 8192;
    if (b < 1) b = 1;
    return (int)b;
}
inline int stream_chunks(int hw, int px, int C, int& ppc) {
    const int rows = TPB / (C / 4);
    long per_img = ((long)hw * C + 16383) / 16384;
    const long maxc = (px + rows - 1) / rows;
    if (per_img > maxc) per_img = maxc;
    if (per_img > 4096) per_img = 4096;
    if (per_img < 1) per_img = 1;
    ppc = (int)((px + per_img - 1) / per_img);
    return (int)((px + ppc - 1) / ppc);
}
inline long rb_bwd2_chunks(int hw, int c, int& ppc) {
    const int rows = TPB / (c / 4);
    long per_img = ((long)hw * c + 32767) / 32768;
    if (per_img > 1024) per_img = 1024;
    const long maxc = (hw + rows - 1) / rows;
    if (per_img > maxc) per_img = maxc;
    if (per_img < 1) per_img = 1;
    ppc = (int)((hw + per_img - 1) / per_img);
    return per_img;
}
inline void chunking(long P, int C, long& chunks, long& ppc) {
    chunks = (P * C + 32767) / 32768;
    if (chunks > 2048) chunks = 2048;
    if (chunks < 1) chunks = 1;
    ppc = (P + chunks - 1) / chunks;
    chunks = (P + ppc - 1) / ppc;
}
inline size_t part_lds(int c, int ncols) { return (size_t)(TPB / (c / 4)) * ncols * sizeof(float); }

void launch_rb_out(const float* t2, int ld, const float* A, const float* B, const float* sa, const float* r, int ldr, const float* rs,
                   const float* rh, float* out, int ldo, unsigned char* relu_bits, float* pooled, int ldp, unsigned char* pool_idx, int n_img,
                   int hw, int w, int c, void* stream) {
    int ppc;
    const int chunks = stream_chunks(hw, pooled ? hw / 4 : hw, c, ppc);
    const dim3 grid(chunks, n_img);
    if (pooled)
        hipLaunchKernelGGL(relu_bits ? rb_out_pool_kernel<true> : rb_out_pool_kernel<false>, grid, dim3(TPB), 0, (hipStream_t)stream, t2, ld, A, B, sa, r,
                           ldr, rs, rh, out, ldo, relu_bits, pooled, ldp, pool_idx, hw, w, c, ppc);
    else if (relu_bits)
        hipLaunchKernelGGL(rb_out_bits_kernel, grid, dim3(TPB), 0, (hipStream_t)stream, t2, ld, A, B, sa, r, ldr, rs, rh, out, ldo, relu_bits, hw, c, ppc);
    else
        hipLaunchKernelGGL(rb_out_kernel, grid, dim3(TPB), 0, (hipStream_t)stream, t2, ld, A, B, sa, r, ldr, rs, rh, out, ldo, hw, c, ppc);
}

void launch_rb_bwd1(const float* dout, int lddo, const float* dpool, int ldp, const unsigned char* pool_idx, const float* out, int ldo,
                    const unsigned char* relu_bits, const float* t2, int ld, const float* A, const float* B, const float* sa, float* dv, int lddv,
                    float* dq, int n_img, int hw, int w, int c, void* stream) {
    if (n_img < 1) return;
    int gx = px_grid(hw);
    if (gx > 8192 / n_img) gx = 8192 / n_img > 0 ? 8192 / n_img : 1;
    auto kernel = dpool ? (relu_bits ? rb_bwd1_ex_kernel<true, true> : rb_bwd1_ex_kernel<true, false>)
                        : (relu_bits ? rb_bwd1_ex_kernel<false, true> : rb_bwd1_ex_kernel<false, false>);
    hipLaunchKernelGGL(kernel, dim3(gx, n_img), dim3(TPB), 0, (hipStream_t)stream, dout, lddo, dpool, ldp, pool_idx, out, ldo, relu_bits, t2, ld, A, B, sa,
                       dv, lddv, dq, hw, w, c);
}

template <bool BN>
void launch_rb_bwd2(const float* dv, int lddv, const float* t2, int ld, const float* sa, const float* dsm, const int* amax, const float* r, int ldr,
                    const float* mean_s, const float* invstd_s, int n_img, int hw, int c, float* workspace, float* sdu, float* sdut, float* sums_s,
                    void* stream) {
    hipStream_t st = (hipStream_t)stream;
    constexpr int NV = BN ? 4 : 2;
    int ppc;
    const long per_img = rb_bwd2_chunks(hw, c, ppc);
    hipLaunchKernelGGL(rb_bwd2_partial<BN>, dim3((int)per_img, n_img), dim3(TPB), part_lds(c, c * NV), st, dv, lddv, t2, ld, sa, dsm, amax, hw, c, ppc,
                       workspace, r, ldr, mean_s, invstd_s);
    hipLaunchKernelGGL(rb_bwd2_final, dim3(cdiv((long)n_img * c, 128)), dim3(128), 0, st, workspace, n_img, c, (int)per_img, NV, sdu, sdut);
    if constexpr (BN) hipLaunchKernelGGL(rb_bwd2_bn_final, dim3(c), dim3(256), 0, st, workspace, (long)n_img * per_img, c, sums_s);
}

void launch_rb_bwd3(float* dv, int lddv, const float* t2, int ld, const float* sa, const float* dsm, const int* amax, const float* ca,
                    const float* davg, const float* dmx, const int* idx, const float* mean2, const float* invstd2, const float* s2,
                    const float* sums2, float* dt2, int lddt, long pixels, int hw, int c, long m_total, const RbScArgs* sc, void* stream) {
    int ppc;
    const int chunks = stream_chunks(hw, hw, c, ppc);
    const dim3 grid(chunks, (int)(pixels / hw));
    const float inv_m = 1.0f / (float)(m_total > 0 ? m_total : pixels);
    if (sc)
        hipLaunchKernelGGL(rb_bwd3_sc_kernel, grid, dim3(TPB), 0, (hipStream_t)stream, dv, lddv, t2, ld, sa, dsm, amax, ca, davg, dmx, idx, mean2, invstd2,
                           s2, sums2, dt2, lddt, hw, c, ppc, inv_m, *sc);
    else
        hipLaunchKernelGGL(rb_bwd3_kernel, grid, dim3(TPB), 0, (hipStream_t)stream, dv, lddv, t2, ld, sa, dsm, amax, ca, davg, dmx, idx, mean2, invstd2, s2,
                           sums2, dt2, lddt, hw, c, ppc, inv_m);
}

template <bool BN>
void launch_ag_bwd2(const float* ds, const float* g1, int ldg, const float* x1, int ldx, const float* sg, const float* hg, const float* sx,
                    const float* hx, const float* wpsi, const float* mean_g, const float* invstd_g, const float* mean_x, const float* invstd_x,
                    float* dpre, int ldp, float* workspace, float* dwpsi_db, float* sums_g, float* sums_x, long pixels, int f, void* stream) {
    hipStream_t st = (hipStream_t)stream;
    const int nc = BN ? 4 * f + 1 : f + 1;
    long chunks, ppc;
    chunking(pixels, f, chunks, ppc);
    hipLaunchKernelGGL(ag_bwd2_partial<BN>, dim3((int)chunks), dim3(TPB), part_lds(f, nc), st, ds, g1, ldg, x1, ldx, sg, hg, sx, hx, wpsi, dpre, ldp,
                       pixels, f, ppc, workspace, mean_g, invstd_g, mean_x, invstd_x);
    if constexpr (BN) hipLaunchKernelGGL(ag_bwd2_bn_final, dim3(nc), dim3(256), 0, st, workspace, chunks, f, dwpsi_db, sums_g, sums_x);
    else hipLaunchKernelGGL(reduce_rows_kernel, dim3(nc), dim3(256), 0, st, workspace, chunks, nc, dwpsi_db);
}
}

#define REQ_C4(C) RUNET_REQUIRE((C) >= 4 && (C) <= 1024 && (C) % 4 == 0, "channels must be a multiple of 4 in [4, 1024]")

extern "C" int runet_ca_coeff(const float* mean_nc, const float* max_nc, const float* min_nc, const int* imax_nc, const int* imin_nc,
                              const float* s2, const float* h2, const float* w0p, const float* w2p, int n_img, int c, int cr,
                              float* A, float* B, float* ca, float* avg, float* mx, int* idx, float* tval, void* stream) {
    RUNET_REQUIRE(mean_nc && max_nc && min_nc && imax_nc && imin_nc && s2 && h2 && w0p && w2p && A && B, "null pointer");
    REQ_C4(c);
    RUNET_REQUIRE(cr >= 1 && cr <= c, "bad hidden width");
    RUNET_REQUIRE(!avg || (mx && idx && tval), "save buffers must come together");
    const size_t lds = (2 * c + 2 * cr + 2 * CA_TPB) * sizeof(float);
    hipLaunchKernelGGL(ca_coeff_kernel, dim3(n_img), dim3(CA_TPB), lds, (hipStream_t)stream, mean_nc, max_nc, min_nc, imax_nc, imin_nc, s2, h2,
                       w0p, w2p, c, cr, A, B, ca, avg, mx, idx, tval);
    RUNET_CHECK_LAUNCH();
}

extern "C" int runet_sa_reduce(const float* t2, int ld, const float* A, const float* B, long pixels, int hw, int c, float* smap,
                               int* amax, void* stream) {
    RUNET_REQUIRE(t2 && A && B && smap && amax, "null pointer");
    REQ_C4(c);
    hipLaunchKernelGGL(sa_reduce_kernel, dim3(px_grid(pixels)), dim3(TPB), 0, (hipStream_t)stream, t2, ld, A, B, pixels, hw, c, smap, amax);
    RUNET_CHECK_LAUNCH();
}

extern "C" int runet_sa_conv7(const float* smap, const float* wp, float* sa, int n_img, int h, int w, void* stream) {
    RUNET_REQUIRE(smap && wp && sa, "null pointer");
    hipLaunchKernelGGL(sa_conv7_kernel, dim3(cdiv(w, 16), cdiv(h, 16), n_img), dim3(256), 0, (hipStream_t)stream, smap, wp, sa, h, w);
    RUNET_CHECK_LAUNCH();
}

extern "C" int runet_rb_out(const float* t2, int ld, const float* A, const float* B, const float* sa, const float* r, int ldr,
                            const float* rs, const float* rh, float* out, int ldo, long pixels, int hw, int c, void* stream) {
    RUNET_REQUIRE(t2 && A && B && sa && r && out, "null pointer");
    REQ_C4(c);
    RUNET_REQUIRE(pixels % hw == 0, "pixels must be a whole number of images");
    launch_rb_out(t2, ld, A, B, sa, r, ldr, rs, rh, out, ldo, nullptr, nullptr, 0, nullptr, (int)(pixels / hw), hw, 0, c, stream);
    RUNET_CHECK_LAUNCH();
}

extern "C" int runet_rb_bwd1(const float* dout, int lddo, const float* out, int ldo, const float* t2, int ld, const float* A,
                             const float* B, const float* sa, float* dv, int lddv, float* dq, long pixels, int hw, int c, void* stream) {
    RUNET_REQUIRE(dout && t2 && A && B && sa && dv && dq, "null pointer");
    REQ_C4(c);
    RUNET_REQUIRE(pixels % hw == 0, "pixels must be a whole number of images");
    launch_rb_bwd1(dout, lddo, nullptr, 0, nullptr, out, ldo, nullptr, t2, ld, A, B, sa, dv, lddv, dq, (int)(pixels / hw), hw, 0, c, stream);
    RUNET_CHECK_LAUNCH();
}

extern "C" int runet_rb_out_ex(const float* t2, int ld, const float* A, const float* B, const float* sa, const float* r, int ldr,
                               const float* rs, const float* rh, float* out, int ldo, unsigned char* relu_bits, float* pooled, int ldp,
                               unsigned char* pool_idx, int n_img, int h, int w, int c, void* stream) {
    RUNET_REQUIRE(t2 && A && B && sa && r && out, "null pointer");
    REQ_C4(c);
    RUNET_REQUIRE(n_img >= 1 && h >= 1 && w >= 1, "bad shape");
    RUNET_REQUIRE((pooled == nullptr) == (pool_idx == nullptr), "pooled and pool_idx come together");
    RUNET_REQUIRE((long)h * w < (1L << 31), "image too large");
    if (pooled) {
        RUNET_REQUIRE(h % 2 == 0 && w % 2 == 0, "h and w must be even");
        RUNET_REQUIRE(ldp >= c && ldp % 4 == 0, "bad pooled stride");
    }
    launch_rb_out(t2, ld, A, B, sa, r, ldr, rs, rh, out, ldo, relu_bits, pooled, ldp, pool_idx, n_img, h * w, w, c, stream);
    RUNET_CHECK_LAUNCH();
}

extern "C" int runet_rb_bwd1_ex(const float* dout, int lddo, const float* dpool, int ldp, const unsigned char* pool_idx, const float* out, int ldo,
                                const unsigned char* relu_bits, const float* t2, int ld, const float* A, const float* B, const float* sa,
                                float* dv, int lddv, float* dq, int n_img, int h, int w, int c, void* stream) {
    RUNET_REQUIRE(dout && t2 && A && B && sa && dv && dq, "null pointer");
    REQ_C4(c);
    RUNET_REQUIRE(n_img >= 1 && h >= 1 && w >= 1 && (long)h * w < (1L << 31), "bad shape");
    RUNET_REQUIRE((dpool == nullptr) == (pool_idx == nullptr), "dpool and pool_idx come together");
    RUNET_REQUIRE(!dpool || (h % 2 == 0 && w % 2 == 0 && ldp >= c && ldp % 4 == 0), "pooled gradient: h and w must be even, stride a multiple of 4");
    launch_rb_bwd1(dout, lddo, dpool, ldp, pool_idx, out, ldo, relu_bits, t2, ld, A, B, sa, dv, lddv, dq, n_img, h * w, w, c, stream);
    RUNET_CHECK_LAUNCH();
}

extern "C" long runet_sa_conv7_bwd_workspace_floats(int n_img, int h, int w) { return (long)n_img * cdiv(h, 16) * cdiv(w, 16) * 98; }

extern "C" int runet_sa_conv7_bwd(const float* smap, const float* dq, const float* wp, float* dsm, float* dwp, float* workspace,
                                  int n_img, int h, int w, void* stream) {
    RUNET_REQUIRE(smap && dq && wp && dsm && dwp && workspace, "null pointer");
    hipStream_t st = (hipStream_t)stream;
    dim3 grid(cdiv(w, 16), cdiv(h, 16), n_img);
    hipLaunchKernelGGL(sa_conv7_bwd_kernel, grid, dim3(256), 0, st, smap, dq, wp, dsm, workspace, h, w);
    hipLaunchKernelGGL(reduce_rows_kernel, dim3(98), dim3(256), 0, st, workspace, (long)grid.x * grid.y * grid.z, 98, dwp);
    RUNET_CHECK_LAUNCH();
}

extern "C" int runet_rb_bwd2(const float* dv, int lddv, const float* t2, int ld, const float* sa, const float* dsm, const int* amax,
                             int n_img, int hw, int c, float* workspace, float* sdu, float* sdut, void* stream) {
    RUNET_REQUIRE(dv && t2 && sa && dsm && amax && workspace && sdu && sdut, "null pointer");
    REQ_C4(c);
    launch_rb_bwd2<false>(dv, lddv, t2, ld, sa, dsm, amax, nullptr, 0, nullptr, nullptr, n_img, hw, c, workspace, sdu, sdut, nullptr, stream);
    RUNET_CHECK_LAUNCH();
}

extern "C" long runet_rb_bwd2_bn_workspace_floats(int n_img, int hw, int c) {
    int ppc;
    return (long)n_img * rb_bwd2_chunks(hw, c, ppc) * c * 4 + 64;
}
extern "C" int runet_rb_bwd2_bn(const float* dv, int lddv, const float* t2, int ld, const float* sa, const float* dsm, const int* amax, const float* r,
                                int ldr, const float* mean_s, const float* invstd_s, int n_img, int hw, int c, float* workspace,
                                long workspace_floats, float* sdu, float* sdut, float* sums_s, void* stream) {
    RUNET_REQUIRE(dv && t2 && sa && dsm && amax && r && mean_s && invstd_s && workspace && sdu && sdut && sums_s, "null pointer");
    REQ_C4(c);
    RUNET_REQUIRE(ldr >= c && ldr % 4 == 0 && workspace_floats >= runet_rb_bwd2_bn_workspace_floats(n_img, hw, c), "bad stride / workspace too small");
    const size_t lds = part_lds(c, 4 * c);
    RUNET_REQUIRE(lds <= 64 * 1024, "LDS budget");
    launch_rb_bwd2<true>(dv, lddv, t2, ld, sa, dsm, amax, r, ldr, mean_s, invstd_s, n_img, hw, c, workspace, sdu, sdut, sums_s, stream);
    RUNET_CHECK_LAUNCH();
}

extern "C" long runet_ca_bwd_workspace_floats(int n_img, int c, int cr) { return (long)n_img * (c + 3L * cr) + 64; }

extern "C" int runet_ca_bwd(const float* sdu, const float* sdut, const float* s2, const float* h2, const float* ca, const float* avg,
                            const float* mx, const float* w0p, const float* w2p, const float* mean_nc, const float* tval,
                            const float* mean2, const float* invstd2, int n_img, int c, int cr, float* workspace, float* davg,
                            float* dmx, float* sums2, float* dw0p, float* dw2p, void* stream) {
    RUNET_REQUIRE(sdu && sdut && s2 && h2 && ca && avg && mx && w0p && w2p && mean_nc && tval && mean2 && invstd2 && workspace && davg && dmx &&
                  sums2 && dw0p && dw2p, "null pointer");
    REQ_C4(c);
    hipStream_t st = (hipStream_t)stream;
    float* dz = workspace;
    float* hvec = workspace + (long)n_img * c;
    const size_t lds = (c + 3 * cr + 2 * CA_TPB) * sizeof(float);
    hipLaunchKernelGGL(ca_bwd_image_kernel, dim3(n_img), dim3(CA_TPB), lds, st, sdu, sdut, s2, h2, ca, avg, mx, w0p, w2p, c, cr, davg, dmx, dz, hvec);
    const int tot = c * cr > c ? c * cr : c;
    hipLaunchKernelGGL(ca_bwd_final_kernel, dim3(cdiv(tot, 128)), dim3(128), 0, st, sdu, sdut, ca, davg, dmx, mean_nc, tval, mean2, invstd2, avg, mx,
                       dz, hvec, n_img, c, cr, sums2, dw0p, dw2p);
    RUNET_CHECK_LAUNCH();
}

extern "C" int runet_rb_bwd3(const float* dv, int lddv, const float* t2, int ld, const float* sa, const float* dsm, const int* amax,
                             const float* ca, const float* davg, const float* dmx, const int* idx, const float* mean2,
                             const float* invstd2, const float* s2, const float* sums2, float* dt2, int lddt, long pixels, int hw, int c,
                             long m_total, void* stream) {
    RUNET_REQUIRE(dv && t2 && sa && dsm && amax && ca && davg && dmx && idx && mean2 && invstd2 && s2 && sums2 && dt2, "null pointer");
    REQ_C4(c);
    RUNET_REQUIRE(pixels % hw == 0, "pixels must be a whole number of images");
    launch_rb_bwd3(const_cast<float*>(dv), lddv, t2, ld, sa, dsm, amax, ca, davg, dmx, idx, mean2, invstd2, s2, sums2, dt2, lddt, pixels, hw, c, m_total,
                   nullptr, stream);
    RUNET_CHECK_LAUNCH();
}

extern "C" int runet_rb_bwd3_sc(float* dv, int lddv, const float* t2, int ld, const float* sa, const float* dsm, const int* amax, const float* ca,
                                const float* davg, const float* dmx, const int* idx, const float* mean2, const float* invstd2, const float* s2,
                                const float* sums2, float* dt2, int lddt, const float* r, int ldr, const float* mean_s, const float* invstd_s,
                                const float* scale_s, const float* sums_s, long m_total_s, long pixels, int hw, int c, long m_total, void* stream) {
    RUNET_REQUIRE(dv && t2 && sa && dsm && amax && ca && davg && dmx && idx && mean2 && invstd2 && s2 && sums2 && dt2, "null pointer");
    RUNET_REQUIRE(r && mean_s && invstd_s && scale_s && sums_s, "null pointer (shortcut BatchNorm)");
    REQ_C4(c);
    RUNET_REQUIRE(pixels % hw == 0, "pixels must be a whole number of images");
    RUNET_REQUIRE(ldr >= c && ldr % 4 == 0, "bad stride");
    const RbScArgs sc{r, ldr, mean_s, invstd_s, scale_s, sums_s, 1.0f / (float)(m_total_s > 0 ? m_total_s : pixels)};
    launch_rb_bwd3(dv, lddv, t2, ld, sa, dsm, amax, ca, davg, dmx, idx, mean2, invstd2, s2, sums2, dt2, lddt, pixels, hw, c, m_total, &sc, stream);
    RUNET_CHECK_LAUNCH();
}

extern "C" int runet_ag_psi(const float* g1, int ldg, const float* x1, int ldx, const float* sg, const float* hg, const float* sx,
                            const float* hx, const float* wpsi, const float* bpsi, float* s, long pixels, int f, void* stream) {
    RUNET_REQUIRE(g1 && x1 && sg && hg && sx && hx && wpsi && bpsi && s, "null pointer");
    REQ_C4(f);
    hipLaunchKernelGGL(ag_psi_kernel, dim3(px_grid(pixels)), dim3(TPB), 0, (hipStream_t)stream, g1, ldg, x1, ldx, sg, hg, sx, hx, wpsi, bpsi, s, pixels, f);
    RUNET_CHECK_LAUNCH();
}

extern "C" int runet_ag_out(const float* xs, int ldx, const float* s, const float* sp, const float* hp, float* out, int ldo, long pixels,
                            int c, void* stream) {
    RUNET_REQUIRE(xs && s && sp && hp && out, "null pointer");
    REQ_C4(c);
    long chunks, ppc;
    chunking(pixels, c, chunks, ppc);
    hipLaunchKernelGGL(ag_out_kernel, dim3((int)chunks), dim3(TPB), 0, (hipStream_t)stream, xs, ldx, s, sp, hp, out, ldo, pixels, c, ppc);
    RUNET_CHECK_LAUNCH();
}

extern "C" int runet_ag_bwd1(const float* datt, int ldd, const float* xs, int ldx, const float* s, const float* sp, const float* hp,
                             float* dxs, int lddx, float* dsbn, long pixels, int c, void* stream) {
    RUNET_REQUIRE(datt && xs && s && sp && hp && dxs && dsbn, "null pointer");
    REQ_C4(c);
    hipLaunchKernelGGL(ag_bwd1_kernel, dim3(px_grid(pixels)), dim3(TPB), 0, (hipStream_t)stream, datt, ldd, xs, ldx, s, sp, hp, dxs, lddx, dsbn, pixels, c);
    RUNET_CHECK_LAUNCH();
}

extern "C" int runet_ag_bwd2(const float* ds, const float* g1, int ldg, const float* x1, int ldx, const float* sg, const float* hg,
                             const float* sx, const float* hx, const float* wpsi, float* dpre, int ldp, float* workspace,
                             float* dwpsi_db, long pixels, int f, void* stream) {
    RUNET_REQUIRE(ds && g1 && x1 && sg && hg && sx && hx && wpsi && dpre && workspace && dwpsi_db, "null pointer");
    REQ_C4(f);
    launch_ag_bwd2<false>(ds, g1, ldg, x1, ldx, sg, hg, sx, hx, wpsi, nullptr, nullptr, nullptr, nullptr, dpre, ldp, workspace, dwpsi_db, nullptr, nullptr,
                          pixels, f, stream);
    RUNET_CHECK_LAUNCH();
}

extern "C" long runet_ag_bwd2_bn_workspace_floats(long pixels, int f) {
    long chunks, ppc;
    chunking(pixels, f, chunks, ppc);
    return chunks * (4L * f + 1) + 64;
}

extern "C" int runet_ag_bwd2_bn(const float* ds, const float* g1, int ldg, const float* x1, int ldx, const float* sg, const float* hg,
                                const float* sx, const float* hx, const float* wpsi, const float* mean_g, const float* invstd_g,
                                const float* mean_x, const float* invstd_x, float* dpre, int ldp, float* workspace, long workspace_floats,
                                float* dwpsi_db, float* sums_g, float* sums_x, long pixels, int f, void* stream) {
    RUNET_REQUIRE(ds && g1 && x1 && sg && hg && sx && hx && wpsi && mean_g && invstd_g && mean_x && invstd_x && dpre && workspace && dwpsi_db &&
                  sums_g && sums_x, "null pointer");
    REQ_C4(f);
    RUNET_REQUIRE(workspace_floats >= runet_ag_bwd2_bn_workspace_floats(pixels, f), "workspace too small (runet_ag_bwd2_bn_workspace_floats)");
    const size_t lds = part_lds(f, 4 * f + 1);
    RUNET_REQUIRE(lds <= 64 * 1024, "LDS budget");
    launch_ag_bwd2<true>(ds, g1, ldg, x1, ldx, sg, hg, sx, hx, wpsi, mean_g, invstd_g, mean_x, invstd_x, dpre, ldp, workspace, dwpsi_db, sums_g, sums_x,
                         pixels, f, stream);
    RUNET_CHECK_LAUNCH();
}

extern "C" int runet_outc_fwd(const float* x, int ld, const float* w, const float* b, float* logit, float* prob, long pixels, int c,
                              void* stream) {
    RUNET_REQUIRE(x && w && b && prob, "null pointer");
    REQ_C4(c);
    hipLaunchKernelGGL(outc_fwd_kernel, dim3(px_grid(pixels)), dim3(TPB), 0, (hipStream_t)stream, x, ld, w, b, logit, prob, pixels, c);
    RUNET_CHECK_LAUNCH();
}

extern "C" int runet_outc_bwd(const float* dprob, const float* prob, const float* x, int ld, const float* w, float* dx, int lddx,
                              float* workspace, float* dw_db, long pixels, int c, void* stream) {
    RUNET_REQUIRE(dprob && x && w && dx && workspace && dw_db, "null pointer");
    REQ_C4(c);
    hipStream_t st = (hipStream_t)stream;
    long chunks, ppc;
    chunking(pixels, c, chunks, ppc);
    hipLaunchKernelGGL(outc_bwd_partial, dim3((int)chunks), dim3(TPB), part_lds(c, c + 1), st, dprob, prob, x, ld, w, dx, lddx, pixels, c, ppc, workspace);
    hipLaunchKernelGGL(reduce_rows_kernel, dim3(c + 1), dim3(256), 0, st, workspace, chunks, c + 1, dw_db);
    RUNET_CHECK_LAUNCH();
}
```

eusipco-2026-robust-unet_amd/csrc/conv_stem.hip:

```cpp
#include "runet_common.h"
#include "../../include/runet_hip.h"

namespace {

constexpr int TR = 8, TC = 32;
constexpr int HC = TC + 2;
constexpr int HALO_FLOATS = (TR + 2) * HC * 4;

struct StemFwd {
    const float* x; int ldx;
    const float* w3; const float* w1;
    float* y3; int ldy3; float* y1; int ldy1;
    int H, W, cin_w, cout;
    float* stats3; float* stats1;
};

__device__ __forceinline__ void load_halo(float* halo, const float* __restrict__ x, int ldx, int n, int r0, int c0, int H, int W) {
    for (int i = threadIdx.x; i < (TR + 2) * HC; i += 256) {
        const int hr = i / HC, hc = i - hr * HC;
        const int ih = r0 + hr - 1, iw = c0 + hc - 1;
        f32x4 v = {0.f, 0.f, 0.f, 0.f};
        if ((unsigned)ih < (unsigned)H && (unsigned)iw < (unsigned)W) v = *reinterpret_cast<const f32x4*>(x + (((long)n * H + ih) * W + iw) * ldx);
        *reinterpret_cast<f32x4*>(halo + i * 4) = v;
    }
}

__device__ __forceinline__ int tap_offset(int k, int cin_w, int taps) {
    if (k >= taps * cin_w) return -1;
    const int tap = k / cin_w, c = k - tap * cin_w;
    if (taps == 1) return (HC + 1) * 4 + c;
    return ((tap / 3) * HC + (tap % 3)) * 4 + c;
}

template <int NT>
__global__ __launch_bounds__(256) void stem_conv_kernel(StemFwd a) {
    __shared__ __attribute__((aligned(16))) float halo[HALO_FLOATS + 4];
    __shared__ float bmat[32 * NT * 32];
    const int tid = threadIdx.x, lane = tid & 63, wid = tid >> 6, li = lane & 31, kk = lane >> 5;
    const int tiles_x = (a.W + TC - 1) / TC;
    const int n = blockIdx.y, ty = blockIdx.x / tiles_x, tx = blockIdx.x - ty * tiles_x;
    const int r0 = ty * TR, c0 = tx * TC;
    const int n3 = a.cout / 32;
    for (int i = tid; i < 32 * NT * 32; i += 256) {
        const int k = i / (NT * 32), col = i - k * (NT * 32);
        float v = 0.f;
        if (k < 9 * a.cin_w) {
            if (col < a.cout) v = a.w3[(long)k * a.cout + col];
            else {
                const int tap = k / a.cin_w, c = k - tap * a.cin_w;
                if (tap == 4) v = a.w1[(long)c * a.cout + (col - a.cout)];
            }
        }
        bmat[i] = v;
    }
    load_halo(halo, a.x, a.ldx, n, r0, c0, a.H, a.W);
    if (tid < 4) halo[HALO_FLOATS + tid] = 0.f;
    __syncthreads();
    float breg[16][NT];
    int aoff[16];
#pragma unroll
    for (int s = 0; s < 16; ++s) {
        aoff[s] = tap_offset(2 * s + kk, a.cin_w, 9);
#pragma unroll
        for (int t = 0; t < NT; ++t) breg[s][t] = bmat[(2 * s + kk) * (NT * 32) + t * 32 + li];
    }
    float scnt = 0.f, smean[NT], sm2[NT];
#pragma unroll
    for (int t = 0; t < NT; ++t) { smean[t] = 0.f; sm2[t] = 0.f; }
#pragma unroll 1
    for (int seg = 0; seg < 2; ++seg) {
        const int r = 2 * wid + seg;
        if (r0 + r >= a.H) break;
        const int base = (r * HC + li) * 4;
        f32x16 acc[NT];
#pragma unroll
        for (int t = 0; t < NT; ++t)
#pragma unroll
            for (int i = 0; i < 16; ++i) acc[t][i] = 0.f;
#pragma unroll
        for (int s = 0; s < 16; ++s) {
            const float av = halo[aoff[s] >= 0 ? base + aoff[s] : HALO_FLOATS];
#pragma unroll
            for (int t = 0; t < NT; ++t) acc[t] = __builtin_amdgcn_mfma_f32_32x32x2f32(av, breg[s][t], acc[t], 0, 0, 0);
        }
        const long rowpix = ((long)n * a.H + r0 + r) * a.W + c0;
#pragma unroll
        for (int t = 0; t < NT; ++t) {
            float* y = t < n3 ? a.y3 : a.y1;
            const int ldy = t < n3 ? a.ldy3 : a.ldy1;
            const int ch = (t < n3 ? t : t - n3) * 32 + li;
#pragma unroll
            for (int i = 0; i < 16; ++i) {
                const int m = (i & 3) + 8 * (i >> 2) + 4 * kk;
                if (c0 + m < a.W) y[(rowpix + m) * ldy + ch] = acc[t][i];
            }
        }
        if (a.stats3) {
            float cnt = 0.f;
#pragma unroll
            for (int i = 0; i < 16; ++i) cnt += (c0 + (i & 3) + 8 * (i >> 2) + 4 * kk < a.W) ? 1.f : 0.f;
            if (cnt > 0.f) {
                const float nt = scnt + cnt, f = cnt / nt, wgt = scnt * f;
#pragma unroll
                for (int t = 0; t < NT; ++t) {
                    float s1 = 0.f, q = 0.f;
#pragma unroll
                    for (int i = 0; i < 16; ++i) s1 += (c0 + (i & 3) + 8 * (i >> 2) + 4 * kk < a.W) ? acc[t][i] : 0.f;
                    const float mu = s1 / cnt;
#pragma unroll
                    for (int i = 0; i < 16; ++i) {
                        const float d = acc[t][i] - mu;
                        q += (c0 + (i & 3) + 8 * (i >> 2) + 4 * kk < a.W) ? d * d : 0.f;
                    }
                    const float dl = mu - smean[t];
                    smean[t] += dl * f;
                    sm2[t] += q + dl * dl * wgt;
                }
                scnt = nt;
            }
        }
    }
    if (a.stats3) {
        float* xch = bmat;
        __syncthreads();
        const float ocnt = __shfl_xor(scnt, 32, 64);
#pragma unroll
        for (int t = 0; t < NT; ++t) {
            const float omean = __shfl_xor(smean[t], 32, 64), om2 = __shfl_xor(sm2[t], 32, 64);
            const float nt = scnt + ocnt;
            float mu = smean[t], q = sm2[t];
            if (ocnt > 0.f) { const float f = ocnt / nt, dl = omean - mu; mu += dl * f; q += om2 + dl * dl * (scnt * f); }
            if (kk == 0) { float* o = xch + ((wid * NT + t) * 32 + li) * 3; o[0] = nt; o[1] = mu; o[2] = q; }
        }
        __syncthreads();
        for (int col = tid; col < NT * 32; col += 256) {
            float cnt = 0.f, mu = 0.f, q = 0.f;
            for (int wv = 0; wv < 4; ++wv) {
                const float* o = xch + (wv * NT * 32 + col) * 3;
                if (o[0] > 0.f) { const float nt = cnt + o[0], f = o[0] / nt, dl = o[1] - mu; mu += dl * f; q += o[2] + dl * dl * (cnt * f); cnt = nt; }
            }
            const int t = col >> 5;
            float* dst = (t < n3 ? a.stats3 : a.stats1) + (((long)blockIdx.y * gridDim.x + blockIdx.x) * a.cout + (t < n3 ? t : t - n3) * 32 + (col & 31)) * 3;
            dst[0] = cnt; dst[1] = mu; dst[2] = q;
        }
    }
}

struct StemWgrad {
    const float* x; int ldx; const float* dy; int ldy;
    float* slabs;
    int Nimg, H, W, cin_w, cout, taps;
    int tiles_y, tiles_x, total_tiles, tiles_per_block;
};

template <int NT>
__global__ __launch_bounds__(256) void stem_wgrad_kernel2(StemWgrad a) {
    __shared__ __attribute__((aligned(16))) float smem[4 * NT * 16 * 64 > HALO_FLOATS + 4 ? 4 * NT * 16 * 64 : HALO_FLOATS + 4];
    float* halo = smem;
    const int tid = threadIdx.x, lane = tid & 63, wid = tid >> 6, li = lane & 31, kk = lane >> 5;
    const int K = a.taps * a.cin_w;
    const int moff = tap_offset(li, a.cin_w, a.taps);
    f32x16 acc[NT];
#pragma unroll
    for (int t = 0; t < NT; ++t)
#pragma unroll
        for (int i = 0; i < 16; ++i) acc[t][i] = 0.f;
    const int t_begin = blockIdx.x * a.tiles_per_block;
    const int t_end = min(a.total_tiles, t_begin + a.tiles_per_block);
    const int per_img = a.tiles_y * a.tiles_x;
    for (int tile = t_begin; tile < t_end; ++tile) {
        const int n = tile / per_img, rem = tile - n * per_img;
        const int ty = rem / a.tiles_x, tx = rem - ty * a.tiles_x;
        const int r0 = ty * TR, c0 = tx * TC;
        __syncthreads();
        load_halo(halo, a.x, a.ldx, n, r0, c0, a.H, a.W);
        if (tid < 4) halo[HALO_FLOATS + tid] = 0.f;
        float breg[2][16][NT];
#pragma unroll
        for (int seg = 0; seg < 2; ++seg) {
            const int r = r0 + 2 * wid + seg;
            const float* row = a.dy + (((long)n * a.H + r) * a.W + c0) * a.ldy + li;
#pragma unroll
            for (int s = 0; s < 16; ++s) {
                const int c = 2 * s + kk;
                const bool ok = r < a.H && c0 + c < a.W;
#pragma unroll
                for (int t = 0; t < NT; ++t) breg[seg][s][t] = ok ? row[(long)c * a.ldy + t * 32] : 0.f;
            }
        }
        __syncthreads();
#pragma unroll
        for (int seg = 0; seg < 2; ++seg) {
            const int base = ((2 * wid + seg) * HC + kk) * 4;
#pragma unroll
            for (int s = 0; s < 16; ++s) {
                const float av = halo[moff >= 0 ? base + 8 * s + moff : HALO_FLOATS];
#pragma unroll
                for (int t = 0; t < NT; ++t) acc[t] = __builtin_amdgcn_mfma_f32_32x32x2f32(av, breg[seg][s][t], acc[t], 0, 0, 0);
            }
        }
    }
    __syncthreads();
    float* red = smem;
#pragma unroll
    for (int t = 0; t < NT; ++t)
#pragma unroll
        for (int i = 0; i < 16; ++i) red[((wid * NT + t) * 16 + i) * 64 + lane] = acc[t][i];
    __syncthreads();
    float* slab = a.slabs + (long)blockIdx.x * K * a.cout;
    for (int e = tid; e < NT * 16 * 64; e += 256) {
        const int l = e & 63, i = (e >> 6) & 15, t = e >> 10;
        const int m = (i & 3) + 8 * (i >> 2) + 4 * (l >> 5);
        if (m < K) {
            const float v = (red[((0 * NT + t) * 16 + i) * 64 + l] + red[((1 * NT + t) * 16 + i) * 64 + l]) +
                            (red[((2 * NT + t) * 16 + i) * 64 + l] + red[((3 * NT + t) * 16 + i) * 64 + l]);
            slab[(long)m * a.cout + t * 32 + (l & 31)] = v;
        }
    }
}

__global__ __launch_bounds__(256) void stem_slab_reduce(const float* __restrict__ slabs, float* __restrict__ out, int n, int nslabs) {
    __shared__ float red[256];
    const int col = threadIdx.x & 7, kl = threadIdx.x >> 3;
    const int i = blockIdx.x * 8 + col;
    float s = 0.f;
    if (i < n)
        for (int b = kl; b < nslabs; b += 32) s += slabs[(long)b * n + i];
    red[threadIdx.x] = s;
    __syncthreads();
    if (kl == 0 && i < n) {
        for (int j = 1; j < 32; ++j) s += red[j * 8 + col];
        out[i] = s;
    }
}

int wgrad_blocks(int total_tiles) { return total_tiles < 1024 ? total_tiles : 1024; }

}

extern "C" int runet_stem_supported(int cin_w, int cout) { return (cin_w >= 1 && cin_w <= 3 && cout % 32 == 0 && cout >= 32 && cout <= 64) ? 1 : 0; }

static int stem_conv_launch(const float* x, int ldx, const float* w3, const float* w1, float* y3, int ldy3, float* y1, int ldy1, int n_img, int h, int w,
                            int cin_w, int cout, float* stats3, float* stats1, void* stream);

extern "C" int runet_stem_conv(const float* x, int ldx, const float* w3, const float* w1, float* y3, int ldy3, float* y1, int ldy1, int n_img,
                               int h, int w, int cin_w, int cout, void* stream) {
    return stem_conv_launch(x, ldx, w3, w1, y3, ldy3, y1, ldy1, n_img, h, w, cin_w, cout, nullptr, nullptr, stream);
}

extern "C" int runet_stem_conv_stats_parts(int n_img, int h, int w) { return n_img * cdiv(h, TR) * cdiv(w, TC); }

extern "C" int runet_stem_conv_stats(const float* x, int ldx, const float* w3, const float* w1, float* y3, int ldy3, float* y1, int ldy1, int n_img,
                                     int h, int w, int cin_w, int cout, float* stats3, float* stats1, void* stream) {
    RUNET_REQUIRE(stats3 && (!w1 || stats1), "stats3 (and stats1 with a 1x1 filter) must not be NULL");
    return stem_conv_launch(x, ldx, w3, w1, y3, ldy3, y1, ldy1, n_img, h, w, cin_w, cout, stats3, stats1, stream);
}

static int stem_conv_launch(const float* x, int ldx, const float* w3, const float* w1, float* y3, int ldy3, float* y1, int ldy1, int n_img, int h, int w,
                            int cin_w, int cout, float* stats3, float* stats1, void* stream) {
    RUNET_REQUIRE(x && w3 && y3 && (!w1 || y1), "null pointer");
    RUNET_REQUIRE(runet_stem_supported(cin_w, cout), "stem kernel: 1..3 input channels, 32 or 64 output channels");
    RUNET_REQUIRE(ldx >= 4 && ldx % 4 == 0 && ((uintptr_t)x % 16) == 0, "x must be NHWC padded to (a multiple of) 4 channels, 16-byte aligned");
    RUNET_REQUIRE(n_img > 0 && h > 0 && w > 0 && ldy3 >= cout && (!w1 || ldy1 >= cout), "bad shape");
    StemFwd a{x, ldx, w3, w1, y3, ldy3, y1, ldy1, h, w, cin_w, cout, stats3, stats1};
    const dim3 grid(cdiv(h, TR) * cdiv(w, TC), n_img);
    const int nt = (cout / 32) * (w1 ? 2 : 1);
    hipStream_t st = (hipStream_t)stream;
    if (nt == 1) hipLaunchKernelGGL(stem_conv_kernel<1>, grid, dim3(256), 0, st, a);
    else if (nt == 2) hipLaunchKernelGGL(stem_conv_kernel<2>, grid, dim3(256), 0, st, a);
    else hipLaunchKernelGGL(stem_conv_kernel<4>, grid, dim3(256), 0, st, a);
    RUNET_CHECK_LAUNCH();
}

extern "C" long runet_stem_wgrad_workspace_floats(int n_img, int h, int w, int cin_w, int cout, int ksize) {
    return (long)wgrad_blocks(n_img * cdiv(h, TR) * cdiv(w, TC)) * ksize * ksize * cin_w * cout;
}

extern "C" int runet_stem_wgrad(const float* x, int ldx, const float* dy, int ldy, float* dw, float* workspace, long workspace_floats, int n_img,
                                int h, int w, int cin_w, int cout, int ksize, void* stream) {
    RUNET_REQUIRE(x && dy && dw && workspace, "null pointer");
    RUNET_REQUIRE(runet_stem_supported(cin_w, cout) && (ksize == 1 || ksize == 3), "stem kernel: 1..3 input channels, 32 or 64 output channels, 1x1 or 3x3");
    RUNET_REQUIRE(ldx >= 4 && ldx % 4 == 0 && ((uintptr_t)x % 16) == 0 && ldy >= cout, "x must be NHWC padded to 4 channels, 16-byte aligned");
    RUNET_REQUIRE(workspace_floats >= runet_stem_wgrad_workspace_floats(n_img, h, w, cin_w, cout, ksize), "workspace too small (runet_stem_wgrad_workspace_floats)");
    StemWgrad a{};
    a.x = x; a.ldx = ldx; a.dy = dy; a.ldy = ldy; a.slabs = workspace;
    a.Nimg = n_img; a.H = h; a.W = w; a.cin_w = cin_w; a.cout = cout; a.taps = ksize * ksize;
    a.tiles_y = cdiv(h, TR); a.tiles_x = cdiv(w, TC); a.total_tiles = n_img * a.tiles_y * a.tiles_x;
    const int blocks0 = wgrad_blocks(a.total_tiles);
    a.tiles_per_block = cdiv(a.total_tiles, blocks0);
    const int blocks = cdiv(a.total_tiles, a.tiles_per_block);
    hipStream_t st = (hipStream_t)stream;
    if (cout == 32) hipLaunchKernelGGL(stem_wgrad_kernel2<1>, dim3(blocks), dim3(256), 0, st, a);
    else hipLaunchKernelGGL(stem_wgrad_kernel2<2>, dim3(blocks), dim3(256), 0, st, a);
    const int nout = a.taps * cin_w * cout;
    hipLaunchKernelGGL(stem_slab_reduce, dim3(cdiv(nout, 8)), dim3(256), 0, st, workspace, dw, nout, blocks);
    RUNET_CHECK_LAUNCH();
}
```

eusipco-2026-robust-unet_amd/model.py:

```python
from __future__ import annotations

import math

import torch
import torch.nn as nn

from . import blocks as B
from . import ops


class _Holder(nn.Module):
    def forward(self, *a, **k):
        raise NotImplementedError(f"{type(self).__name__} is a parameter holder; call the enclosing block "
                                  "(ResidualBlock / DilatedBlock / AttentionGate / RobustUNet)")


class Conv2d(_Holder):
    def __init__(self, in_channels, out_channels, kernel_size, padding=0, dilation=1, bias=True, stride=1):
        super().__init__()
        k = kernel_size
        self.in_channels, self.out_channels, self.kernel_size = in_channels, out_channels, (k, k)
        self.padding, self.dilation, self.stride = (padding, padding), (dilation, dilation), (stride, stride)
        self.weight = nn.Parameter(torch.empty(k, k, in_channels, out_channels).permute(3, 2, 0, 1))
        if bias:
# ... 306 lines not shown
        self.kernel_size = kernel_size

    def forward(self, x):
        _require_cuda(x)
        return _PoolFn.apply(x)


class _PoolFn(torch.autograd.Function):
    @staticmethod
    def forward(ctx, x):
        y, idx = B.maxpool_forward(_nhwc(x))
        ctx.idx = idx
        return _nchw(y)

    @staticmethod
    def backward(ctx, dy):
        return _nchw(B.maxpool_backward(_nhwc(dy), ctx.idx))


class RobustUNet(nn.Module):

    LEVEL_DROPOUT = {"inc": 0.1, "down1": 0.1, "down2": 0.2, "down3": 0.2, "bottleneck": 0.3, "dec4": 0.2, "dec3": 0.2,
                     "dec2": 0.1, "dec1": 0.1}

    def __init__(self, n_channels=3, n_classes=1, base_channels=64):
        super().__init__()
        if n_classes != 1:
            raise ValueError("the fused output head implements the reference's n_classes=1 sigmoid head")
        if base_channels % 16 != 0:
            raise ValueError("base_channels must be a multiple of 16 (ChannelAttention uses C // 16)")
        b = base_channels
        self.n_channels, self.n_classes, self.base_channels = n_channels, n_classes, b
        self.inc = ResidualBlock(n_channels, b, dropout_rate=0.1)
        self.down1 = nn.Sequential(MaxPool2d(2), ResidualBlock(b, b * 2, dropout_rate=0.1))
        self.down2 = nn.Sequential(MaxPool2d(2), ResidualBlock(b * 2, b * 4, dropout_rate=0.2))
        self.down3 = nn.Sequential(MaxPool2d(2), ResidualBlock(b * 4, b * 8, dropout_rate=0.2))
        self.bottleneck = nn.Sequential(MaxPool2d(2), DilatedBlock(b * 8, b * 16), ResidualBlock(b * 16, b * 16, dropout_rate=0.3))
        self.att4 = AttentionGate(b * 8, b * 8, b * 4)
        self.att3 = AttentionGate(b * 4, b * 4, b * 2)
        self.att2 = AttentionGate(b * 2, b * 2, b)
        self.att1 = AttentionGate(b, b, b // 2)
        self.up4 = ConvTranspose2d(b * 16, b * 8, 2, stride=2)
        self.dec4 = ResidualBlock(b * 16, b * 8, dropout_rate=0.2)
        self.up3 = ConvTranspose2d(b * 8, b * 4, 2, stride=2)
        self.dec3 = ResidualBlock(b * 8, b * 4, dropout_rate=0.2)
        self.up2 = ConvTranspose2d(b * 4, b * 2, 2, stride=2)
        self.dec2 = ResidualBlock(b * 4, b * 2, dropout_rate=0.1)
        self.up1 = ConvTranspose2d(b * 2, b, 2, stride=2)
        self.dec1 = ResidualBlock(b * 2, b, dropout_rate=0.1)
        self.outc = nn.Sequential(Conv2d(b, n_classes, 1), _Act())
        self.sync_bn_hook = None
        self.precision = "f32"
        self._arena = None
        self._named = None
        self._initialize_weights()

    def _initialize_weights(self):
        for m in self.modules():
            if isinstance(m, Conv2d):
                nn.init.kaiming_normal_(m.weight, mode="fan_out", nonlinearity="relu")
            elif isinstance(m, BatchNorm2d):
                nn.init.constant_(m.weight, 1)
                nn.init.constant_(m.bias, 0)

    def named_params(self):
        if self._named is None:
            self._named = list(self.named_parameters())
        return self._named

    def _apply(self, fn, recurse=True):
        self._named = None
        return super()._apply(fn, recurse)

    def _rbs(self):
        return {"inc": self.inc, "down1.1": self.down1[1], "down2.1": self.down2[1], "down3.1": self.down3[1],
                "bottleneck.2": self.bottleneck[2], "dec4": self.dec4, "dec3": self.dec3, "dec2": self.dec2, "dec1": self.dec1}

    def grad_arena(self):
        dev = self.outc[0].weight.device
        if self._arena is None or self._arena.device != dev:
            self._arena = GradArena(self)
        return self._arena

    def set_precision(self, mode):
        if mode not in ops.PRECISIONS:
            raise ValueError(f"precision must be one of {ops.PRECISIONS}")
        self.precision = mode
        return self

    def set_dropout_masks(self, masks):
        for k, rb in self._rbs().items():
            rb.dropout.mask = None if masks is None else masks[k]

    def _check_input(self, x):
        if x.shape[2] % 16 or x.shape[3] % 16:
            raise ValueError("H and W must be multiples of 16 (four 2x2 poolings)")

    def forward(self, x, return_logits=False):
        _require_cuda(x)
        self._check_input(x)
        named = self.named_params()
        names = [k for k, _ in named]
        params = [p for _, p in named]
        if torch.is_grad_enabled() and any(p.requires_grad for p in params):
            prob, logit = _NetFn.apply(x, self, names, return_logits, *params)
        else:
            prob, logit, _ = net_forward(self, x, save=False, want_logit=return_logits)
        return (prob, logit) if return_logits else prob


def _draw_masks(net, rbs, n, dev):
    if any(rb.dropout.mask is not None for rb in rbs.values()):
        return {k: rb.dropout.draw(n, rb.out_channels, dev) for k, rb in rbs.items()}
    key = (str(dev), n, tuple((k, rb.out_channels, rb.dropout.p) for k, rb in rbs.items()))
    plan = getattr(net, "_mask_plan", None)
    if plan is None or plan[0] != key:
        keep = torch.cat([torch.full((n * rb.out_channels,), 1.0 - rb.dropout.p) for rb in rbs.values()])
        inv = torch.where(keep > 0, 1.0 / keep.clamp_min(1e-12), torch.zeros_like(keep))
        offs, o = {}, 0
        for k, rb in rbs.items():
            offs[k] = (o, o + n * rb.out_channels)
            o += n * rb.out_channels
        plan = net._mask_plan = (key, keep.to(dev), inv.to(dev), offs)
    _, keep, inv, offs = plan
    m = torch.bernoulli(keep).mul_(inv)
    return {k: (m[a:b].view(n, rb.out_channels) if rb.dropout.p > 0.0 else None) for (k, rb), (a, b) in zip(rbs.items(), offs.values())}


def net_forward(net: RobustUNet, x, save, want_logit=False):
    with ops.precision(net.precision):
        return _net_forward(net, x, save, want_logit)


def _net_forward(net: RobustUNet, x, save, want_logit=False):
    tr = net.training
    hook = net.sync_bn_hook if tr else None
    n = x.shape[0]
    dev = x.device
    ops.branches_pay(n, x.shape[2], x.shape[3])
    if save:
        ops.prefetch_derived()
    x0 = B.to_nhwc_pad(x, (net.n_channels + 3) // 4 * 4)
    rbs = net._rbs()
    masks = _draw_masks(net, rbs, n, dev) if tr else {k: None for k in rbs}
    C = {}
    x1, C["inc"], pooled, C["pool1"] = B.rb_forward(x0, rbs["inc"].handles(), tr, masks["inc"], save, hook, pool=True)
    skips = [x1]
    for lvl in (1, 2, 3):
        cur, C[f"down{lvl}.1"], pooled, C[f"pool{lvl + 1}"] = B.rb_forward(pooled, rbs[f"down{lvl}.1"].handles(), tr, masks[f"down{lvl}.1"], save,
                                                                           hook, pool=True)
        skips.append(cur)
    xd, C["bottleneck.1"] = B.dilated_forward(pooled, net.bottleneck[1].handles(), tr, save, hook)
    y, C["bottleneck.2"] = B.rb_forward(xd, rbs["bottleneck.2"].handles(), tr, masks["bottleneck.2"], save, hook)
    for lvl in (4, 3, 2, 1):
        att, up = getattr(net, f"att{lvl}"), getattr(net, f"up{lvl}")
        cat, C[f"upgate{lvl}"] = B.upgate_forward(y, skips[lvl - 1], att.handles(up), tr, save, hook)
        y, C[f"dec{lvl}"] = B.rb_forward(cat, rbs[f"dec{lvl}"].handles(), tr, masks[f"dec{lvl}"], save, hook)
    w, b = ops.hwio(net.outc[0].weight), net.outc[0].bias
    prob, logit = B.outc_forward(y, w, b, want_logit)
    if save:
        C["head"] = (y, w, prob)
        C["precision"] = net.precision
    return prob, logit, (C if save else None)


BACKWARD_ORDER = ("outc.0", "dec1", "att1", "up1", "dec2", "att2", "up2", "dec3", "att3", "up3", "dec4", "att4", "up4",
                  "bottleneck.2", "bottleneck.1", "down3.1", "down2.1", "down1.1", "inc")


class GradArena:

    def __init__(self, net):
        named = list(net.named_parameters())
        self.device = named[0][1].device
        self.off, self.numel, self.block_end = {}, {}, {}
        cur, seen = 0, set()
        for blk in BACKWARD_ORDER:
            prev = None
            for name, p in named:
                if not name.startswith(blk + "."):
                    continue
                packed = prev is not None and name.endswith(".bias") and prev == name[:-5] + ".weight"
                if not packed:
                    cur = (cur + 3) // 4 * 4
                self.off[name], self.numel[name] = cur, p.numel()
                cur += p.numel()
                prev = name
                seen.add(name)
            self.block_end[blk] = cur
        assert len(seen) == len(named), "BACKWARD_ORDER does not cover every parameter"
        self.total = (cur + 3) // 4 * 4
        self.flat = torch.zeros(self.total, device=self.device, dtype=torch.float32)
        self.on_block_done = None

    def buf(self, prefix, items):
        off0 = self.off[prefix + items[0][0]]
        cur = off0
        for name, sh in items:
            n = B._numel(sh)
            assert self.off[prefix + name] == cur and self.numel[prefix + name] == n, f"arena layout mismatch at {prefix + name}"
            cur += n
        return self.flat[off0:cur]

    def grad_view(self, name, p):
        return torch.as_strided(self.flat, p.shape, p.stride(), self.off[name])

    def done(self, blk):
        if self.on_block_done is not None:
            self.on_block_done(self.block_end[blk])


def net_backward(C, dprob, sink, done=lambda blk: None):
    with ops.precision(C.get("precision", "f32")), ops.wgrad_side_stream():
        _net_backward(C, dprob, sink, done)


def _net_backward(C, dprob, sink, done):
    y, w, prob = C["head"]
    dy = B.outc_backward(dprob, prob, y, w, sink, pre="outc.0.")
    done("outc.0")
    dskip = {}
    for lvl in (1, 2, 3, 4):
        dcat = B.rb_backward(C[f"dec{lvl}"], dy, sink, pre=f"dec{lvl}.")
        done(f"dec{lvl}")
        dy, dskip[lvl] = B.upgate_backward(C[f"upgate{lvl}"], dcat, sink, f"att{lvl}.", f"up{lvl}.")
        done(f"up{lvl}")
    dxd = B.rb_backward(C["bottleneck.2"], dy, sink, pre="bottleneck.2.")
    done("bottleneck.2")
    dpool = B.dilated_backward(C["bottleneck.1"], dxd, sink, pre="bottleneck.1.")
    done("bottleneck.1")
    for lvl in (3, 2, 1):
        dpool = B.rb_backward(C[f"down{lvl}.1"], dskip[lvl + 1], sink, pre=f"down{lvl}.1.", dpool=dpool, pool_idx=C[f"pool{lvl + 1}"])
        done(f"down{lvl}.1")
    B.rb_backward(C["inc"], dskip[1], sink, pre="inc.", need_dx=False, dpool=dpool, pool_idx=C["pool1"])
    done("inc")


class _NetFn(torch.autograd.Function):

    @staticmethod
    def forward(ctx, x, net, names, want_logit, *params):
        prob, logit, C = net_forward(net, x, save=True, want_logit=want_logit)
        ctx.C, ctx.net = C, net
        if logit is None:
            logit = prob.new_empty(0)
        ctx.mark_non_differentiable(logit)
        return prob, logit

    @staticmethod
    def backward(ctx, dprob, _dlogit):
        if ctx.C is None:
            raise RuntimeError("RobustUNet backward called twice (activations were released after the first pass)")
        net = ctx.net
        named = net.named_params()
        arena = net.grad_arena()
        if all(p.grad is None for _, p in named):
            net_backward(ctx.C, dprob.contiguous(), arena, arena.done)
            for k, p in named:
                if p.requires_grad:
                    p.grad = arena.grad_view(k, p)
        else:
            sink = B.DictSink(dprob.device)
            net_backward(ctx.C, dprob.contiguous(), sink)
            for k, p in named:
                if not p.requires_grad:
                    continue
                g = _logical(sink.g[k], isinstance(net.get_submodule(k.rpartition(".")[0]), ConvTranspose2d))
                if p.grad is None:
                    p.grad = g
                else:
                    p.grad.add_(g)
        ctx.C = None
        return (None, None, None, None) + (None,) * len(named)
```

include/runet_hip.h:

```cpp
#ifndef RUNET_HIP_H
#define RUNET_HIP_H
#ifdef __cplusplus
extern "C" {
#endif

const char* runet_last_error(void);
void runet_set_error(const char* msg);
int runet_abi_version(void);

enum { RUNET_CONV_FWD = 0, RUNET_CONV_DGRAD = 1, RUNET_CONVT_FWD = 2, RUNET_CONVT_DGRAD = 3, RUNET_CONV_DGRAD_T = 4, RUNET_CONVT_DGRAD_T = 5 };

int runet_conv_igemm(const float* x, int ldx, const float* w, const float* bias, float* y, int ldy,
                     int n_img, int h, int w_, int cin, int cin_w, int cout, int kh, int kw, int dil,
                     int mode, int accumulate, void* stream);

int runet_transpose_taps(const float* w, float* wt, int taps, int cin, int cout, void* stream);

const char* runet_conv_igemm_kernel_name(int n_img, int h, int w_, int cin, int cout, int kh, int mode);
int runet_igemm_force_variant(int variant);
int runet_igemm_lowp_force_variant(int variant);

long runet_conv_wgrad_workspace_floats(int n_img, int h, int w_, int cin_w, int cout, int kh, int kw);
int runet_conv_wgrad(const float* x, int ldx, const float* dy, int ldy, float* dw, float* workspace,
                     long workspace_floats, int n_img, int h, int w_, int cin, int cin_w, int cout,
                     int kh, int kw, int dil, int transposed, void* stream);


int runet_wino_supported(int h, int w, int cin, int cout);
int runet_wino_fits(int n_img, int h, int w, int ldx, int ldy, int cin, int cout);
int runet_wino_weights(const float* w_hwio, float* U, int cin, int cout, int dgrad, void* stream);
int runet_wino_conv(const float* x, int ldx, const float* U, const float* bias, float* y, int ldy, int n_img, int h, int w, int k, int n,
                    int accumulate, void* stream);

long runet_wino_x3_pack_elems(int k, int n);
int runet_wino_weights_x3(const float* w_hwio, void* Upacked, int cin, int cout, int dgrad, void* stream);
int runet_wino_conv_x3(const float* x, int ldx, const void* Upacked, const float* bias, float* y, int ldy, int n_img, int h, int w, int k, int n,
                       int accumulate, void* stream);
int runet_wino_conv_x3_stats_parts(int n_img, int h, int w);
int runet_wino_conv_x3_stats(const float* x, int ldx, const void* Upacked, const float* bias, float* y, int ldy, int n_img, int h, int w, int k,
                             int n, int accumulate, float* stats, void* stream);

long runet_wino_wgrad_workspace_floats(int n_img, int h, int w, int cin, int cout);
int runet_wino_wgrad(const float* x, int ldx, const float* dy, int ldy, float* dw, float* workspace, long workspace_floats, int n_img,
                     int h, int w, int cin, int cout, void* stream);

long runet_reduce_workspace_floats(int n_img, int hw, int c);

int runet_chan_stats(const float* x, int ld, int n_img, int hw, int c, float* workspace, float* mean_nc, float* m2_nc,
                     float* max_nc, float* min_nc, int* imax_nc, int* imin_nc, int want_minmax, void* stream);

int runet_bn_stats_finalize(const float* part, int nparts, int c, const float* gamma, const float* beta, float* run_mean, float* run_var,
                            long long* num_batches_tracked, float momentum, float eps, float* scale, float* shift, float* save_mean,
                            float* save_invstd, void* stream);
int runet_bn_finalize(const float* mean_nc, const float* m2_nc, int n_img, int c, long hw, const float* gamma, const float* beta,
                      float* run_mean, float* run_var, long long* num_batches_tracked, float momentum, float eps, int training,
                      float* scale, float* shift, float* save_mean, float* save_invstd, void* stream);

int runet_bn_stats(const float* x, int ld, int n_img, int hw, int c, float* workspace, const float* gamma, const float* beta,
                   float* run_mean, float* run_var, long long* num_batches_tracked, float momentum, float eps, float* scale,
                   float* shift, float* save_mean, float* save_invstd, void* stream);

int runet_bn_apply(const float* x, int ldx, float* y, int ldy, long pixels, int hw, int c, const float* scale, const float* shift,
                   const float* mask_nc, int relu, void* stream);

int runet_bn_bwd_reduce(const float* dy, int lddy, const float* x, int ldx, const float* act, int ldact, int n_img, int hw, int c,
                        const float* mean, const float* invstd, const float* mask_nc, float* workspace, float* sums, const float* relu_scale,
                        const float* relu_shift, void* stream);
int runet_bn_bwd_apply(const float* dy, int lddy, const float* x, int ldx, const float* act, int ldact, float* dx, int lddx,
                       long pixels, int hw, int c, const float* mean, const float* invstd, const float* scale, const float* sums,
                       const float* mask_nc, long m_total, const float* relu_shift, void* stream);
int runet_chan_sum(const float* x, int ld, long pixels, int c, float* workspace, float* out, int accumulate, void* stream);

int runet_ca_coeff(const float* mean_nc, const float* max_nc, const float* min_nc, const int* imax_nc, const int* imin_nc,
                   const float* s2, const float* h2, const float* w0p, const float* w2p, int n_img, int c, int cr, float* A, float* B,
                   float* ca, float* avg, float* mx, int* idx, float* tval, void* stream);
int runet_sa_reduce(const float* t2, int ld, const float* A, const float* B, long pixels, int hw, int c, float* smap, int* amax,
                    void* stream);
int runet_sa_conv7(const float* smap, const float* wp, float* sa, int n_img, int h, int w, void* stream);
int runet_rb_out(const float* t2, int ld, const float* A, const float* B, const float* sa, const float* r, int ldr, const float* rs,
                 const float* rh, float* out, int ldo, long pixels, int hw, int c, void* stream);
int runet_rb_bwd1(const float* dout, int lddo, const float* out, int ldo, const float* t2, int ld, const float* A, const float* B,
                  const float* sa, float* dv, int lddv, float* dq, long pixels, int hw, int c, void* stream);
int runet_rb_out_ex(const float* t2, int ld, const float* A, const float* B, const float* sa, const float* r, int ldr, const float* rs,
                    const float* rh, float* out, int ldo, unsigned char* relu_bits, float* pooled, int ldp, unsigned char* pool_idx, int n_img,
                    int h, int w, int c, void* stream);
int runet_rb_bwd1_ex(const float* dout, int lddo, const float* dpool, int ldp, const unsigned char* pool_idx, const float* out, int ldo,
                     const unsigned char* relu_bits, const float* t2, int ld, const float* A, const float* B, const float* sa, float* dv,
                     int lddv, float* dq, int n_img, int h, int w, int c, void* stream);
long runet_sa_conv7_bwd_workspace_floats(int n_img, int h, int w);
int runet_sa_conv7_bwd(const float* smap, const float* dq, const float* wp, float* dsm, float* dwp, float* workspace, int n_img, int h,
                       int w, void* stream);
int runet_rb_bwd2(const float* dv, int lddv, const float* t2, int ld, const float* sa, const float* dsm, const int* amax, int n_img,
                  int hw, int c, float* workspace, float* sdu, float* sdut, void* stream);
long runet_rb_bwd2_bn_workspace_floats(int n_img, int hw, int c);
int runet_rb_bwd2_bn(const float* dv, int lddv, const float* t2, int ld, const float* sa, const float* dsm, const int* amax, const float* r, int ldr,
                     const float* mean_s, const float* invstd_s, int n_img, int hw, int c, float* workspace, long workspace_floats, float* sdu,
                     float* sdut, float* sums_s, void* stream);
long runet_ca_bwd_workspace_floats(int n_img, int c, int cr);
int runet_ca_bwd(const float* sdu, const float* sdut, const float* s2, const float* h2, const float* ca, const float* avg, const float* mx,
                 const float* w0p, const float* w2p, const float* mean_nc, const float* tval, const float* mean2, const float* invstd2,
                 int n_img, int c, int cr, float* workspace, float* davg, float* dmx, float* sums2, float* dw0p, float* dw2p, void* stream);
int runet_rb_bwd3(const float* dv, int lddv, const float* t2, int ld, const float* sa, const float* dsm, const int* amax, const float* ca,
                  const float* davg, const float* dmx, const int* idx, const float* mean2, const float* invstd2, const float* s2,
                  const float* sums2, float* dt2, int lddt, long pixels, int hw, int c, long m_total, void* stream);
int runet_rb_bwd3_sc(float* dv, int lddv, const float* t2, int ld, const float* sa, const float* dsm, const int* amax, const float* ca,
                     const float* davg, const float* dmx, const int* idx, const float* mean2, const float* invstd2, const float* s2,
                     const float* sums2, float* dt2, int lddt, const float* r, int ldr, const float* mean_s, const float* invstd_s,
                     const float* scale_s, const float* sums_s, long m_total_s, long pixels, int hw, int c, long m_total, void* stream);

int runet_ag_psi(const float* g1, int ldg, const float* x1, int ldx, const float* sg, const float* hg, const float* sx, const float* hx,
                 const float* wpsi, const float* bpsi, float* s, long pixels, int f, void* stream);
int runet_ag_out(const float* xs, int ldx, const float* s, const float* sp, const float* hp, float* out, int ldo, long pixels, int c,
                 void* stream);
int runet_ag_bwd1(const float* datt, int ldd, const float* xs, int ldx, const float* s, const float* sp, const float* hp, float* dxs,
                  int lddx, float* dsbn, long pixels, int c, void* stream);
int runet_ag_bwd2(const float* ds, const float* g1, int ldg, const float* x1, int ldx, const float* sg, const float* hg, const float* sx,
                  const float* hx, const float* wpsi, float* dpre, int ldp, float* workspace, float* dwpsi_db, long pixels, int f,
                  void* stream);
long runet_ag_bwd2_bn_workspace_floats(long pixels, int f);
int runet_ag_bwd2_bn(const float* ds, const float* g1, int ldg, const float* x1, int ldx, const float* sg, const float* hg, const float* sx,
                     const float* hx, const float* wpsi, const float* mean_g, const float* invstd_g, const float* mean_x, const float* invstd_x,
                     float* dpre, int ldp, float* workspace, long workspace_floats, float* dwpsi_db, float* sums_g, float* sums_x, long pixels, int f,
                     void* stream);

int runet_outc_fwd(const float* x, int ld, const float* w, const float* b, float* logit, float* prob, long pixels, int c, void* stream);
int runet_outc_bwd(const float* dprob, const float* prob, const float* x, int ld, const float* w, float* dx, int lddx, float* workspace,
                   float* dw_db, long pixels, int c, void* stream);

int runet_maxpool2_fwd(const float* x, int ldx, float* y, int ldy, unsigned char* idx, int n_img, int h, int w, int c, void* stream);
int runet_maxpool2_bwd(const float* dy, int lddy, const unsigned char* idx, float* dx, int lddx, int n_img, int h, int w, int c,
                       int accumulate, void* stream);
int runet_to_nhwc_pad(const float* x, long sn, long sc, long sh, long sw, float* y, int n_img, int c, int h, int w, int c_pad, void* stream);

int runet_bce_fwd(const float* prob, const float* target, long n, double* workspace1024, float* loss, void* stream);
int runet_bce_bwd(const float* prob, const float* target, const float* grad_out, float* dprob, long n, void* stream);

int runet_adam_chunk_elems(void);
int runet_adam_multi(const long long* table, int n_tensors, const int* chunks, int n_chunks, float lr, float beta1, float beta2, float eps,
                     float weight_decay, int step, float grad_scale, const int* skip_flag, void* stream);

int runet_adam_multi_dev(const long long* table, int n_tensors, const int* chunks, int n_chunks, const float* hyper, int* step_dev,
                         const int* skip_flag, void* stream);
int runet_nonfinite_flag(const float* buf, long n, int* flag2, void* stream);
int runet_stream_wait(void* waiter, void* waited);


int runet_seg_counts(const float* pred, const float* target, long long* counts, int n_img, long per_img, float threshold, void* stream);

int runet_gemm_batched(const float* a, int lda, long stride_a, const float* b, long stride_b, float* c, int ldc, long stride_c, int batch, int rows,
                       int k, int n, void* stream);
int runet_gemm_tn_batched(const float* a, int lda, long stride_a, const float* b, int ldb, long stride_b, float* c, int batch, int rows, int k, int n,
                          int rows_per_split, void* stream);
const char* runet_gemm_batched_kernel_name(int batch, int rows, int k, int n);

int runet_gemm_x3_supported(int rows, int k, int n);
long runet_gemm_x3_pack_elems(int batch, int k, int n);
int runet_gemm_x3_pack(const float* b, long stride_b, void* packed, int batch, int k, int n, void* stream);
int runet_gemm_x3_batched(const float* a, int lda, long stride_a, const void* packed_b, float* c, int ldc, long stride_c, int batch, int rows,
                          int k, int n, void* stream);
int runet_gemm_x3_tn_batched(const float* a, int lda, long stride_a, const float* b, int ldb, long stride_b, float* c, int batch, int rows, int k,
                             int n, int rows_per_split, void* stream);
const char* runet_gemm_x3_kernel_name(int batch, int rows, int k, int n);
int runet_gemm_x3_tn_convt(const float* x, int ldx, const float* dy, int ldy, float* c, int n_img, int h, int w, int cin, int cout,
                           int rows_per_split, void* stream);

int runet_conv_x3_supported(int cin, int cout, int mode);
long runet_conv_x3_pack_elems(int cin, int cout, int mode);
int runet_conv_x3_pack(const float* w, void* packed, int cin, int cout, int mode, void* stream);
int runet_conv_x3(const float* x, int ldx, const void* wpacked, const float* bias, float* y, int ldy, int n_img, int h, int w, int cin, int cout,
                  int mode, int accumulate, void* stream);
const char* runet_conv_x3_kernel_name(int n_img, int h, int w, int cout, int mode);

int runet_conv1x1_stream_supported(int cin, int cout, int mode);
int runet_conv1x1_stream_blocks(int n_img, int h, int w, int cin, int cout);
int runet_conv1x1_stream(const float* x, int ldx, const float* w, const float* bias, float* y, int ldy, int n_img, int h, int w_, int cin,
                         int cout, int mode, int accumulate, void* stream);
const char* runet_conv1x1_stream_kernel_name(int cin, int cout, int accumulate);
int runet_conv1x1_wgrad_stream_supported(int cin, int cout);
int runet_conv1x1_wgrad_stream_slabs(int n_img, int h, int w);
long runet_conv1x1_wgrad_stream_workspace_floats(int n_img, int h, int w, int cin, int cout);
int runet_conv1x1_wgrad_stream(const float* x, int ldx, const float* dy, int ldy, float* dw, float* workspace, long workspace_floats,
                               int n_img, int h, int w_, int cin, int cout, void* stream);

enum { RUNET_DERIVE_WINO4 = 0, RUNET_DERIVE_WINO2 = 1, RUNET_DERIVE_PACK = 2 };
int runet_derive_desc_bytes(void);
int runet_derive_desc(void* host_table, int index, int kind, const float* w, void* dst, int cin, int cout, int mode, int first_block);
int runet_derive_multi(const void* table, int n_desc, int total_blocks, void* stream);
int runet_conv_x3_stats_parts(int n_img, int h, int w);
int runet_conv_x3_stats(const float* x, int ldx, const void* wpacked, const float* bias, float* y, int ldy, int n_img, int h, int w, int cin, int cout,
                        int mode, int accumulate, float* stats, void* stream);

int runet_wino4_supported(int h, int w, int k, int n);
long runet_wino4_workspace_floats(int n_img, int h, int w, int k, int n);
int runet_wino4_weights(const float* w_hwio, float* U, int cin, int cout, int dgrad, void* stream);
int runet_wino4_conv(const float* x, int ldx, const float* U, const float* bias, float* y, int ldy, int n_img, int h, int w, int k, int n,
                     int dil, int accumulate, float* workspace, long workspace_floats, void* stream);
int runet_wino4_weights_x3(const float* w_hwio, void* Upacked, int cin, int cout, int dgrad, void* stream);
int runet_wino4_conv_x3(const float* x, int ldx, const void* Upacked, const float* bias, float* y, int ldy, int n_img, int h, int w, int k, int n,
                        int dil, int accumulate, float* workspace, long workspace_floats, void* stream);
int runet_wino4_input(const float* src, int ld, int c, int n_img, int h, int w, int dil, int mode, float* V, void* stream);
int runet_wino4_input_act(const float* t, int ld, int c, int n_img, int h, int w, int dil, const float* scale, const float* shift,
                          const float* factor_nc, float* V, void* stream);
int runet_wino4_input_bn_bwd(const float* dy, int lddy, const float* x, int ldx, int c, int n_img, int h, int w, int dil, const float* mean,
                             const float* invstd, const float* scale, const float* shift, const float* sums, const float* factor_nc,
                             long m_total, float* Z, void* stream);
int runet_wino4_output(const float* M, int n, int n_img, int h, int w, int dil, const float* bias, float* y, int ldy, int accumulate, void* stream);
int runet_wino4_output_stats_parts(int n_img, int h, int w, int n, int dil);
int runet_wino4_output_stats(const float* M, int n, int n_img, int h, int w, const float* bias, float* y, int ldy, int accumulate, float* stats, void* stream);
int runet_wino4_output_adj(const float* M, int n, int n_img, int h, int w, int dil, float* y, int ldy, int accumulate, void* stream);
int runet_wino4_wgrad_output(const float* dU, int splits, int cin, int cout, float* dw, void* stream);
int runet_wino4_wgrad_rows_per_split(int n_img, int h, int w, int cin, int cout);
long runet_wino4_wgrad_workspace_floats(int n_img, int h, int w, int cin, int cout);
int runet_wino4_wgrad(const float* x, int ldx, const float* dy, int ldy, float* dw, float* workspace, long workspace_floats, int n_img, int h, int w,
                      int cin, int cout, int dil, void* stream);

int runet_stem_supported(int cin_w, int cout);
int runet_stem_conv(const float* x, int ldx, const float* w3, const float* w1, float* y3, int ldy3, float* y1, int ldy1, int n_img,
                    int h, int w, int cin_w, int cout, void* stream);
int runet_stem_conv_stats_parts(int n_img, int h, int w);
int runet_stem_conv_stats(const float* x, int ldx, const float* w3, const float* w1, float* y3, int ldy3, float* y1, int ldy1, int n_img,
                          int h, int w, int cin_w, int cout, float* stats3, float* stats1, void* stream);
long runet_stem_wgrad_workspace_floats(int n_img, int h, int w, int cin_w, int cout, int ksize);
int runet_stem_wgrad(const float* x, int ldx, const float* dy, int ldy, float* dw, float* workspace, long workspace_floats, int n_img,
                     int h, int w, int cin_w, int cout, int ksize, void* stream);

int runet_conv2d_general(const float* x, int ldx, const float* w, const float* bias, float* y, int ldy, int n_img, int hin, int win, int cin,
                         int cin_w, int cout, int kh, int kw, int stride, int pad, int dil, int mode, int accumulate, void* stream);
int runet_convt4_igemm(const float* x, int ldx, const float* w, const float* bias, float* y, int ldy, int n_img, int h, int w_, int cin, int cout,
                       int mode, int accumulate, void* stream);
long runet_conv_wgrad_general_workspace_floats(int pixels, int cin_w, int cout, int kh, int kw);
int runet_conv_wgrad_general(const float* x, int ldx, const float* dy, int ldy, float* dw, float* workspace, long workspace_floats, int n_img,
                             int hin, int win, int cin, int cin_w, int cout, int kh, int kw, int stride, int pad, int dil, int transposed4,
                             void* stream);
int runet_maxpool3s2_fwd(const float* x, int ldx, float* y, int ldy, unsigned char* idx, int n_img, int h, int w, int c, void* stream);
int runet_maxpool3s2_bwd(const float* dy, int lddy, const unsigned char* idx, float* dx, int lddx, int n_img, int h, int w, int c, void* stream);
int runet_add_inplace(float* dst, const float* src, long n, void* stream);
int runet_broadcast_nc(const float* v_nc, float* y, int ldy, int n_img, int hw, int c, void* stream);
int runet_head3x3_fwd(const float* x, int ld, const float* w, const float* b, float* prob, int n_img, int h, int w_, int c, void* stream);
long runet_head3x3_bwd_workspace_floats(int n_img, int h, int w_, int c);
int runet_head3x3_bwd(const float* dprob, const float* prob, const float* x, int ld, const float* w, float* dx, int lddx, float* workspace,
                      float* dw_db, int n_img, int h, int w_, int c, void* stream);


long runet_bf16_pack_elems(int taps, int k, int n);
int runet_bf16_pack_weights(const float* w_hwio, void* packed, int taps, int cin, int cout, int transpose, void* stream);
int runet_conv_igemm_bf16(const float* x, int ldx, const void* wpacked, const float* bias, float* y, int ldy, int n_img, int h, int w_,
                          int cin, int cout, int kh, int kw, int dil, int mode, int accumulate, void* stream);
long runet_conv_wgrad_bf16_workspace_floats(int n_img, int h, int w_, int cin, int cout, int kh, int kw, int dil, int transposed);
int runet_conv_wgrad_bf16(const float* x, int ldx, const float* dy, int ldy, float* dw, float* workspace, long workspace_floats,
                          int n_img, int h, int w_, int cin, int cout, int kh, int kw, int dil, int transposed, void* stream);

long runet_fp16_pack_elems(int taps, int k, int n);
int runet_fp16_pack_weights(const float* w_hwio, void* packed, int taps, int cin, int cout, int transpose, void* stream);
int runet_conv_igemm_fp16(const float* x, int ldx, const void* wpacked, const float* bias, float* y, int ldy, int n_img, int h, int w_,
                          int cin, int cout, int kh, int kw, int dil, int mode, int accumulate, void* stream);
long runet_conv_wgrad_fp16_workspace_floats(int n_img, int h, int w_, int cin, int cout, int kh, int kw, int dil, int transposed);
int runet_conv_wgrad_fp16(const float* x, int ldx, const float* dy, int ldy, float* dw, float* workspace, long workspace_floats,
                          int n_img, int h, int w_, int cin, int cout, int kh, int kw, int dil, int transposed, void* stream);

int runet_bilinear_fwd(const float* x, float* y, long planes, int h, int w, int ho, int wo, void* stream);
int runet_bilinear_bwd(const float* dy, float* dx, long planes, int h, int w, int ho, int wo, void* stream);
int runet_mul_pixel(const float* x, int ldx, const float* s, float* y, int ldy, long pixels, int c, void* stream);

int runet_nhwc_to_nchw(const float* x, int ld, float* y, int n_img, int c, long hw, void* stream);
int runet_ce_fwd(const float* logits_nchw, const long long* target, int n_img, int classes, long hw, double* partials1024, float* loss, void* stream);
int runet_ce_bwd(const float* logits_nchw, const long long* target, const float* gout, float* dlogits_nchw, int n_img, int classes, long hw,
                 void* stream);

int runet_bn_relu_maxpool2_fwd(const float* t, int ldt, const float* scale, const float* shift, float* y, int ldy, unsigned char* idx,
                               int n_img, int h, int w, int c, void* stream);
int runet_bn_bwd_reduce_pooled(const float* dpool, int ldp, const unsigned char* idx, const float* x, int ldx, int n_img, int h, int w, int c,
                               const float* mean, const float* invstd, float* workspace, float* sums, const float* relu_scale,
                               const float* relu_shift, void* stream);
int runet_bn_bwd_apply_pooled(const float* dpool, int ldp, const unsigned char* idx, const float* x, int ldx, float* dx, int lddx, int n_img,
                              int h, int w, int c, const float* mean, const float* invstd, const float* scale, const float* sums, long m_total,
                              const float* relu_shift, void* stream);
int runet_maxunpool2_bwd(const float* du, int lddu, const unsigned char* idx, float* dpool, int ldp, int n_img, int h, int w, int c,
                         void* stream);

int runet_bn_apply_leaky(const float* x, int ldx, float* y, int ldy, long pixels, int hw, int c, const float* scale, const float* shift,
// ... 247 lines not shown
```

Measured before the change: 605.9 images/s.

## Fuse 1x1 output head into last residual block and use rank-1 head gradient

The final 1x1 output conv plus sigmoid is folded into the dec1 residual-block output kernel, so the 64-channel activation no longer has to be reread. In backward, the head no longer materializes a full 64-channel dx. It writes a per-pixel dlogit, and the bwd1 kernel rebuilds the gradient as w*dl on the fly. The stem conv kernel also becomes a persistent grid sized to the CU count. This adds code paths restricted to c==64 and disables fp contraction in the head dot product to keep results consistent.

```diff
diff --git a/eusipco-2026-robust-unet_amd/blocks.py b/eusipco-2026-robust-unet_amd/blocks.py
--- a/eusipco-2026-robust-unet_amd/blocks.py
+++ b/eusipco-2026-robust-unet_amd/blocks.py
@@ -214,6 +214,16 @@
     return FUSED_RB_EDGES and part in RB_EDGE_PARTS
 
 
+FUSED_HEAD = os.environ.get("RUNET_NO_FUSED_HEAD", "0") != "1"
+HEAD_PARTS = frozenset(("fwd", "bwd"))
+
+
+def fuses_head(part, c):
+    if not (FUSED_HEAD and part in HEAD_PARTS and lib.runet_rb_out_head_supported(c)):
+        return False
+    return _edge("out") if part == "fwd" else _edge("bwd1")
+
+
 def chan_sum(x, out):
     n, h, w, c = x.shape
 
@@ -271,7 +281,7 @@
         self.cin_w = w1.shape[2]
 
 
-def rb_forward(x, p: RBParams, training, mask=None, save=True, stats_hook=None, pool=False):
+def rb_forward(x, p: RBParams, training, mask=None, save=True, stats_hook=None, pool=False, head=None):
     n, h, w, _ = x.shape
     c = p.w1.shape[3]
     cr = p.w0p.shape[3]
@@ -338,9 +348,17 @@
         if pool:
             pooled = ops.empty_nhwc(n, h // 2, w // 2, c, x)
             pool_idx = torch.empty((n, h // 2, w // 2, c), device=x.device, dtype=torch.uint8)
-    check(lib.runet_rb_out_ex(t2.data_ptr(), ops.ld(t2), A.data_ptr(), B.data_ptr(), sa.data_ptr(), r.data_ptr(), ops.ld(r), _ptr(ss), _ptr(hs),
-                              out.data_ptr(), ops.ld(out), _ptr(relu_bits), _ptr(pooled), ops.ld(pooled) if pooled is not None else 0, _ptr(pool_idx),
-                              n, h, w, c, st))
+    if head is not None:
+        assert not pool and fuses_head("fwd", c)
+        head["prob"] = torch.empty((n, 1, h, w), device=x.device, dtype=torch.float32)
+        head["logit"] = torch.empty((n, 1, h, w), device=x.device, dtype=torch.float32) if head["want_logit"] else None
+        check(lib.runet_rb_out_head(t2.data_ptr(), ops.ld(t2), A.data_ptr(), B.data_ptr(), sa.data_ptr(), r.data_ptr(), ops.ld(r), _ptr(ss), _ptr(hs),
+                                    out.data_ptr(), ops.ld(out), _ptr(relu_bits), head["w"].data_ptr(), head["b"].data_ptr(), _ptr(head["logit"]),
+                                    head["prob"].data_ptr(), n, h, w, c, st))
+    else:
+        check(lib.runet_rb_out_ex(t2.data_ptr(), ops.ld(t2), A.data_ptr(), B.data_ptr(), sa.data_ptr(), r.data_ptr(), ops.ld(r), _ptr(ss), _ptr(hs),
+                                  out.data_ptr(), ops.ld(out), _ptr(relu_bits), _ptr(pooled), ops.ld(pooled) if pooled is not None else 0,
+                                  _ptr(pool_idx), n, h, w, c, st))
     if pool and pooled is None:
         pooled, pool_idx = maxpool_forward(out)
     if not save:
@@ -357,7 +375,7 @@
     return bn_apply(ctx["t1"], ctx["s1"], ctx["h1"], ctx["mask"], relu=True)
 
 
-def rb_backward(ctx, dout, sink, pre="", need_dx=True, dpool=None, pool_idx=None):
+def rb_backward(ctx, dout, sink, pre="", need_dx=True, dpool=None, pool_idx=None, head_grad=None):
     p: RBParams = ctx["p"]
     x, r, t1, a1, t2, out = ctx["x"], ctx["r"], ctx["t1"], ctx["a1"], ctx["t2"], ctx["out"]
     n, h, w, c = out.shape
@@ -372,9 +390,14 @@
     relu_bits = ctx.get("relu_bits") if _edge("bwd1") else None
     if dpool is not None and not _edge("bwd1"):
         dout, dpool = maxpool_backward(dpool, pool_idx, dx=dout), None
-    check(lib.runet_rb_bwd1_ex(dout.data_ptr(), ops.ld(dout), _ptr(dpool), ops.ld(dpool) if dpool is not None else 0,
-                               pool_idx.data_ptr() if dpool is not None else None, out.data_ptr(), ops.ld(out), _ptr(relu_bits), t2.data_ptr(),
-                               ops.ld(t2), A.data_ptr(), B.data_ptr(), sa.data_ptr(), dv.data_ptr(), ops.ld(dv), dq.data_ptr(), n, h, w, c, st))
+    if head_grad is not None:
+        assert dout is None and dpool is None and relu_bits is not None
+        check(lib.runet_rb_bwd1_rank1(head_grad[0].data_ptr(), head_grad[1].data_ptr(), relu_bits.data_ptr(), t2.data_ptr(), ops.ld(t2), A.data_ptr(),
+                                      B.data_ptr(), sa.data_ptr(), dv.data_ptr(), ops.ld(dv), dq.data_ptr(), n, h, w, c, st))
+    else:
+        check(lib.runet_rb_bwd1_ex(dout.data_ptr(), ops.ld(dout), _ptr(dpool), ops.ld(dpool) if dpool is not None else 0,
+                                   pool_idx.data_ptr() if dpool is not None else None, out.data_ptr(), ops.ld(out), _ptr(relu_bits), t2.data_ptr(),
+                                   ops.ld(t2), A.data_ptr(), B.data_ptr(), sa.data_ptr(), dv.data_ptr(), ops.ld(dv), dq.data_ptr(), n, h, w, c, st))
     dsm = torch.empty((P, 2), device=dev, dtype=torch.float32)
     dwsa = sink.buf(pre, [("sa.conv1.weight", (7, 7, 2, 1))])
     ws = scratch(lib.runet_sa_conv7_bwd_workspace_floats(n, h, w), dev)
@@ -865,6 +888,16 @@
     return dx
 
 
+def outc_backward_dl(dprob, prob, x, sink, pre=""):
+    n, h, wd, c = x.shape
+    dl = torch.empty(n * h * wd, device=x.device, dtype=torch.float32)
+    dw_db = sink.buf(pre, [("weight", (1, 1, c, 1)), ("bias", (1,))])
+    ws = _ws(n, h * wd, c, x.device)
+    check(lib.runet_outc_bwd_dl(dprob.data_ptr(), prob.data_ptr(), x.data_ptr(), ops.ld(x), dl.data_ptr(), ws.data_ptr(), dw_db.data_ptr(), n * h * wd, c,
+                                ops.stream()))
+    return dl
+
+
 FUSED_HR_HEAD = os.environ.get("RUNET_NO_FUSED_HR_HEAD", "0") != "1"
 FUSED_BN_UPSAMPLE = os.environ.get("RUNET_NO_FUSED_BN_UPSAMPLE", "0") != "1"
 
diff --git a/eusipco-2026-robust-unet_amd/csrc/attention.hip b/eusipco-2026-robust-unet_amd/csrc/attention.hip
--- a/eusipco-2026-robust-unet_amd/csrc/attention.hip
+++ b/eusipco-2026-robust-unet_amd/csrc/attention.hip
@@ -142,11 +142,16 @@
 __device__ __forceinline__ unsigned int relu_bits4(const f32x4 o) {
     return (o[0] > 0.f ? 1u : 0u) | (o[1] > 0.f ? 2u : 0u) | (o[2] > 0.f ? 4u : 0u) | (o[3] > 0.f ? 8u : 0u);
 }
+__device__ __forceinline__ float head_dot4(const f32x4 v, const f32x4 k) {
+#pragma clang fp contract(off)
+    return v[0] * k[0] + v[1] * k[1] + v[2] * k[2] + v[3] * k[3];
+}
 #define RB_EDGE_WAVES __attribute__((amdgpu_waves_per_eu(8, 8)))
-template <bool BITS>
+template <bool BITS, bool HEAD = false>
 __device__ __forceinline__ void rb_out_body(const float* t2, int ld, const float* A, const float* B, const float* sa, const float* r, int ldr,
                                             const float* rs, const float* rh, float* out, int ldo, unsigned char* bits, int HW, int C,
-                                            int pix_per_chunk) {
+                                            int pix_per_chunk, const float* hw = nullptr, const float* hb = nullptr, float* logit = nullptr,
+                                            float* prob = nullptr) {
     const int cvec = C / 4, rows = TPB / cvec, tid = threadIdx.x;
     const int col = tid % cvec, row = tid / cvec;
     if (row >= rows) return;
@@ -157,6 +162,8 @@
     f32x4 s4 = {1.f, 1.f, 1.f, 1.f}, h4 = {0.f, 0.f, 0.f, 0.f};
     if (rs) { s4 = *reinterpret_cast<const f32x4*>(rs + c); h4 = *reinterpret_cast<const f32x4*>(rh + c); }
     const long ib = (long)n * HW;
+    f32x4 k = {0.f, 0.f, 0.f, 0.f};
+    if constexpr (HEAD) k = *reinterpret_cast<const f32x4*>(hw + c);
     for (int p = p0 + row; p < p1; p += rows) {
         const f32x4 t = *reinterpret_cast<const f32x4*>(t2 + (ib + p) * ld + c);
         const f32x4 res = *reinterpret_cast<const f32x4*>(r + (ib + p) * ldr + c) * s4 + h4;
@@ -166,6 +173,16 @@
         for (int q = 0; q < 4; ++q) o[q] = fmaxf(o[q], 0.f);
         *reinterpret_cast<f32x4*>(out + (ib + p) * ldo + c) = o;
         if constexpr (BITS) bits[(ib + p) * cvec + col] = (unsigned char)relu_bits4(o);
+        if constexpr (HEAD) {
+            float acc = 0.f;
+            acc += head_dot4(o, k);
+            acc = grp_sum16(acc);
+            if (col == 0) {
+                const float l = acc + hb[0];
+                if (logit) logit[ib + p] = l;
+                prob[ib + p] = sigmoidf_(l);
+            }
+        }
     }
 }
 __global__ __launch_bounds__(TPB) void rb_out_kernel(const float* __restrict__ t2, int ld, const float* __restrict__ A,
@@ -181,6 +198,16 @@
                                                           const float* __restrict__ rh, float* __restrict__ out, int ldo,
                                                           unsigned char* __restrict__ bits, int HW, int C, int pix_per_chunk) {
     rb_out_body<true>(t2, ld, A, B, sa, r, ldr, rs, rh, out, ldo, bits, HW, C, pix_per_chunk);
+}
+template <bool BITS>
+__global__ __launch_bounds__(TPB) void rb_out_head_kernel(const float* __restrict__ t2, int ld, const float* __restrict__ A,
+                                                          const float* __restrict__ B, const float* __restrict__ sa,
+                                                          const float* __restrict__ r, int ldr, const float* __restrict__ rs,
+                                                          const float* __restrict__ rh, float* __restrict__ out, int ldo,
+                                                          unsigned char* __restrict__ bits, int HW, int pix_per_chunk,
+                                                          const float* __restrict__ hw, const float* __restrict__ hb,
+                                                          float* __restrict__ logit, float* __restrict__ prob) {
+    rb_out_body<BITS, true>(t2, ld, A, B, sa, r, ldr, rs, rh, out, ldo, bits, HW, 64, pix_per_chunk, hw, hb, logit, prob);
 }
 template <bool BITS>
 __global__ __launch_bounds__(TPB) RB_EDGE_WAVES void rb_out_pool_kernel(const float* __restrict__ t2, int ld, const float* __restrict__ A,
@@ -237,13 +264,14 @@
     }
 }
 
-template <bool POOL, bool BITS>
+template <bool POOL, bool BITS, bool RANK1 = false>
 __global__ __launch_bounds__(TPB) RB_EDGE_WAVES void rb_bwd1_ex_kernel(const float* __restrict__ dout, int lddo, const float* __restrict__ dpool, int ldp,
                                                          const unsigned char* __restrict__ pidx, const float* __restrict__ out, int ldo,
                                                          const unsigned char* __restrict__ bits, const float* __restrict__ t2, int ld,
                                                          const float* __restrict__ A, const float* __restrict__ B,
                                                          const float* __restrict__ sa, float* __restrict__ dv, int lddv,
-                                                         float* __restrict__ dq, int HW, int W, int C) {
+                                                         float* __restrict__ dq, int HW, int W, int C, const float* __restrict__ dl = nullptr,
+                                                         const float* __restrict__ hw = nullptr) {
     const int sub = threadIdx.x & (LPP - 1);
     const int cvec = C / 4;
     const int n = blockIdx.y;
@@ -258,7 +286,9 @@
         }
         float s = 0.f;
         for (int c = sub * 4; c < C; c += LPP * 4) {
-            f32x4 g = *reinterpret_cast<const f32x4*>(dout + p * lddo + c);
+            f32x4 g;
+            if constexpr (RANK1) g = *reinterpret_cast<const f32x4*>(hw + c) * dl[p];
+            else g = *reinterpret_cast<const f32x4*>(dout + p * lddo + c);
             if constexpr (POOL) g += pooled_grad4_at(dpool, ldp, pidx, C, pq, pk, c);
             f32x4 o = {1.f, 1.f, 1.f, 1.f};
             unsigned int m = 0xfu;
@@ -723,7 +753,7 @@
         for (int c = sub * 4; c < C; c += LPP * 4) {
             const f32x4 v = *reinterpret_cast<const f32x4*>(x + p * ld + c);
             const f32x4 k = *reinterpret_cast<const f32x4*>(w + c);
-            acc += v[0] * k[0] + v[1] * k[1] + v[2] * k[2] + v[3] * k[3];
+            acc += head_dot4(v, k);
         }
         acc = grp_sum16(acc);
         if (sub == 0) {
@@ -733,10 +763,11 @@
         }
     }
 }
+template <bool DX>
 __global__ __launch_bounds__(TPB) void outc_bwd_partial(const float* __restrict__ dprob, const float* __restrict__ prob,
                                                         const float* __restrict__ x, int ld, const float* __restrict__ w,
                                                         float* __restrict__ dx, int lddx, long P, int C, long pix_per_chunk,
-                                                        float* __restrict__ part) {
+                                                        float* __restrict__ part, float* __restrict__ dlout = nullptr) {
     extern __shared__ __attribute__((aligned(16))) float sm[];
     const int cvec = C / 4, rows = TPB / cvec, tid = threadIdx.x;
     const int col = tid % cvec, row = tid / cvec;
@@ -744,7 +775,8 @@
     const long p1 = p0 + pix_per_chunk < P ? p0 + pix_per_chunk : P;
     float sw[4] = {0, 0, 0, 0}, sb = 0.f;
     if (row < rows) {
-        const f32x4 wv = *reinterpret_cast<const f32x4*>(w + col * 4);
+        f32x4 wv = {0.f, 0.f, 0.f, 0.f};
+        if constexpr (DX) wv = *reinterpret_cast<const f32x4*>(w + col * 4);
         for (long p = p0 + row; p < p1; p += rows) {
             float dl = dprob[p];
             if (prob) {
@@ -755,7 +787,8 @@
 #pragma unroll
             for (int q = 0; q < 4; ++q) sw[q] += dl * v[q];
             if (col == 0) sb += dl;
-            *reinterpret_cast<f32x4*>(dx + p * lddx + col * 4) = wv * dl;
+            if constexpr (DX) *reinterpret_cast<f32x4*>(dx + p * lddx + col * 4) = wv * dl;
+            else if (col == 0) dlout[p] = dl;
         }
 #pragma unroll
         for (int q = 0; q < 4; ++q) sm[row * (C + 1) + col * 4 + q] = sw[q];
@@ -828,7 +861,7 @@
     auto kernel = dpool ? (relu_bits ? rb_bwd1_ex_kernel<true, true> : rb_bwd1_ex_kernel<true, false>)
                         : (relu_bits ? rb_bwd1_ex_kernel<false, true> : rb_bwd1_ex_kernel<false, false>);
     hipLaunchKernelGGL(kernel, dim3(gx, n_img), dim3(TPB), 0, (hipStream_t)stream, dout, lddo, dpool, ldp, pool_idx, out, ldo, relu_bits, t2, ld, A, B, sa,
-                       dv, lddv, dq, hw, w, c);
+                       dv, lddv, dq, hw, w, c, nullptr, nullptr);
 }
 
 template <bool BN>
@@ -950,6 +983,35 @@
     RUNET_CHECK_LAUNCH();
 }
 
+extern "C" int runet_rb_out_head_supported(int c) { return c == 4 * LPP ? 1 : 0; }
+
+extern "C" int runet_rb_out_head(const float* t2, int ld, const float* A, const float* B, const float* sa, const float* r, int ldr,
+                                 const float* rs, const float* rh, float* out, int ldo, unsigned char* relu_bits, const float* hw, const float* hb,
+                                 float* logit, float* prob, int n_img, int h, int w, int c, void* stream) {
+    RUNET_REQUIRE(t2 && A && B && sa && r && out && hw && hb && prob, "null pointer");
+    RUNET_REQUIRE(runet_rb_out_head_supported(c), "the fused head needs c == 64 (runet_rb_out_head_supported)");
+    RUNET_REQUIRE(n_img >= 1 && h >= 1 && w >= 1, "bad shape");
+    RUNET_REQUIRE((long)h * w < (1L << 31), "image too large");
+    int ppc;
+    const int chunks = stream_chunks(h * w, h * w, c, ppc);
+    hipLaunchKernelGGL(relu_bits ? rb_out_head_kernel<true> : rb_out_head_kernel<false>, dim3(chunks, n_img), dim3(TPB), 0, (hipStream_t)stream, t2, ld, A,
+                       B, sa, r, ldr, rs, rh, out, ldo, relu_bits, h * w, ppc, hw, hb, logit, prob);
+    RUNET_CHECK_LAUNCH();
+}
+
+extern "C" int runet_rb_bwd1_rank1(const float* dl, const float* hw, const unsigned char* relu_bits, const float* t2, int ld, const float* A,
+                                   const float* B, const float* sa, float* dv, int lddv, float* dq, int n_img, int h, int w, int c, void* stream) {
+    RUNET_REQUIRE(dl && hw && relu_bits && t2 && A && B && sa && dv && dq, "null pointer");
+    REQ_C4(c);
+    RUNET_REQUIRE(n_img >= 1 && h >= 1 && w >= 1 && (long)h * w < (1L << 31), "bad shape");
+    const int hwp = h * w;
+    int gx = px_grid(hwp);
+    if (gx > 8192 / n_img) gx = 8192 / n_img > 0 ? 8192 / n_img : 1;
+    hipLaunchKernelGGL((rb_bwd1_ex_kernel<false, true, true>), dim3(gx, n_img), dim3(TPB), 0, (hipStream_t)stream, nullptr, 0, nullptr, 0, nullptr, nullptr,
+                       0, relu_bits, t2, ld, A, B, sa, dv, lddv, dq, hwp, w, c, dl, hw);
+    RUNET_CHECK_LAUNCH();
+}
+
 extern "C" long runet_sa_conv7_bwd_workspace_floats(int n_img, int h, int w) { return (long)n_img * cdiv(h, 16) * cdiv(w, 16) * 98; }
 
 extern "C" int runet_sa_conv7_bwd(const float* smap, const float* dq, const float* wp, float* dsm, float* dwp, float* workspace,
@@ -1104,7 +1166,21 @@
     hipStream_t st = (hipStream_t)stream;
     long chunks, ppc;
     chunking(pixels, c, chunks, ppc);
-    hipLaunchKernelGGL(outc_bwd_partial, dim3((int)chunks), dim3(TPB), part_lds(c, c + 1), st, dprob, prob, x, ld, w, dx, lddx, pixels, c, ppc, workspace);
+    hipLaunchKernelGGL(outc_bwd_partial<true>, dim3((int)chunks), dim3(TPB), part_lds(c, c + 1), st, dprob, prob, x, ld, w, dx, lddx, pixels, c, ppc, workspace,
+                       nullptr);
     hipLaunchKernelGGL(reduce_rows_kernel, dim3(c + 1), dim3(256), 0, st, workspace, chunks, c + 1, dw_db);
     RUNET_CHECK_LAUNCH();
 }
+
+extern "C" int runet_outc_bwd_dl(const float* dprob, const float* prob, const float* x, int ld, float* dl, float* workspace, float* dw_db,
+                                 long pixels, int c, void* stream) {
+    RUNET_REQUIRE(dprob && x && dl && workspace && dw_db, "null pointer");
+    REQ_C4(c);
+    hipStream_t st = (hipStream_t)stream;
+    long chunks, ppc;
+    chunking(pixels, c, chunks, ppc);
+    hipLaunchKernelGGL(outc_bwd_partial<false>, dim3((int)chunks), dim3(TPB), part_lds(c, c + 1), st, dprob, prob, x, ld, nullptr, nullptr, 0, pixels, c, ppc,
+                       workspace, dl);
+    hipLaunchKernelGGL(reduce_rows_kernel, dim3(c + 1), dim3(256), 0, st, workspace, chunks, c + 1, dw_db);
+    RUNET_CHECK_LAUNCH();
+}
diff --git a/eusipco-2026-robust-unet_amd/csrc/conv_stem.hip b/eusipco-2026-robust-unet_amd/csrc/conv_stem.hip
--- a/eusipco-2026-robust-unet_amd/csrc/conv_stem.hip
+++ b/eusipco-2026-robust-unet_amd/csrc/conv_stem.hip
@@ -13,6 +13,7 @@
     float* y3; int ldy3; float* y1; int ldy1;
     int H, W, cin_w, cout;
     float* stats3; float* stats1;
+    int tiles_x, per_img, total_tiles;
 };
 
 __device__ __forceinline__ void load_halo(float* halo, const float* __restrict__ x, int ldx, int n, int r0, int c0, int H, int W) {
@@ -32,116 +33,166 @@
     return ((tap / 3) * HC + (tap % 3)) * 4 + c;
 }
 
+__device__ __forceinline__ int tap_of(int k, int cin_w) { return cin_w == 1 ? k : cin_w == 2 ? k >> 1 : (k * 11) >> 5; }
+__device__ __forceinline__ int tap_offset9(int k, int cin_w) {
+    if (k >= 9 * cin_w) return -1;
+    const int tap = tap_of(k, cin_w), c = k - tap * cin_w, tr = (tap * 11) >> 5;
+    return (tr * HC + (tap - 3 * tr)) * 4 + c;
+}
+
+__device__ __forceinline__ f32x4 halo_entry(const float* __restrict__ x, int ldx, int i, int n, int r0, int c0, int H, int W) {
+    const int hr = i / HC, hc = i - hr * HC;
+    const int ih = r0 + hr - 1, iw = c0 + hc - 1;
+    f32x4 v = {0.f, 0.f, 0.f, 0.f};
+    if ((unsigned)ih < (unsigned)H && (unsigned)iw < (unsigned)W) v = *reinterpret_cast<const f32x4*>(x + (((long)n * H + ih) * W + iw) * ldx);
+    return v;
+}
+
+constexpr int HALO_ENTRIES = (TR + 2) * HC;
 template <int NT>
-__global__ __launch_bounds__(256) void stem_conv_kernel(StemFwd a) {
-    __shared__ __attribute__((aligned(16))) float halo[HALO_FLOATS + 4];
+__global__ __launch_bounds__(256, 2) void stem_conv_kernel(StemFwd a) {
+    constexpr int PT = NT < 2 ? NT : 2;
+    constexpr int XCH = 4 * NT * 32 * 3;
+    static_assert(2 * XCH <= 32 * NT * 32, "the two exchange buffers live in bmat's storage");
+    static_assert(HALO_ENTRIES > 256 && HALO_ENTRIES <= 512, "two halo entries per thread");
+    __shared__ __attribute__((aligned(16))) float halo[2 * HALO_FLOATS + 4];
     __shared__ float bmat[32 * NT * 32];
     const int tid = threadIdx.x, lane = tid & 63, wid = tid >> 6, li = lane & 31, kk = lane >> 5;
-    const int tiles_x = (a.W + TC - 1) / TC;
-    const int n = blockIdx.y, ty = blockIdx.x / tiles_x, tx = blockIdx.x - ty * tiles_x;
-    const int r0 = ty * TR, c0 = tx * TC;
     const int n3 = a.cout / 32;
+#pragma unroll 4
     for (int i = tid; i < 32 * NT * 32; i += 256) {
         const int k = i / (NT * 32), col = i - k * (NT * 32);
         float v = 0.f;
         if (k < 9 * a.cin_w) {
             if (col < a.cout) v = a.w3[(long)k * a.cout + col];
             else {
-                const int tap = k / a.cin_w, c = k - tap * a.cin_w;
+                const int tap = tap_of(k, a.cin_w), c = k - tap * a.cin_w;
                 if (tap == 4) v = a.w1[(long)c * a.cout + (col - a.cout)];
             }
         }
         bmat[i] = v;
     }
-    load_halo(halo, a.x, a.ldx, n, r0, c0, a.H, a.W);
-    if (tid < 4) halo[HALO_FLOATS + tid] = 0.f;
+    int tile = blockIdx.x;
+    {
+        const int n = tile / a.per_img, rem = tile - n * a.per_img, ty = rem / a.tiles_x, tx = rem - ty * a.tiles_x;
+        for (int i = tid; i < HALO_ENTRIES; i += 256)
+            *reinterpret_cast<f32x4*>(halo + i * 4) = halo_entry(a.x, a.ldx, i, n, ty * TR, tx * TC, a.H, a.W);
+    }
+    if (tid < 4) halo[2 * HALO_FLOATS + tid] = 0.f;
     __syncthreads();
     float breg[16][NT];
     int aoff[16];
 #pragma unroll
     for (int s = 0; s < 16; ++s) {
-        aoff[s] = tap_offset(2 * s + kk, a.cin_w, 9);
+        aoff[s] = tap_offset9(2 * s + kk, a.cin_w);
 #pragma unroll
         for (int t = 0; t < NT; ++t) breg[s][t] = bmat[(2 * s + kk) * (NT * 32) + t * 32 + li];
     }
-    float scnt = 0.f, smean[NT], sm2[NT];
-#pragma unroll
-    for (int t = 0; t < NT; ++t) { smean[t] = 0.f; sm2[t] = 0.f; }
+    __syncthreads();
+    for (int cur = 0; tile < a.total_tiles; tile += gridDim.x, cur ^= 1) {
+        const int n = tile / a.per_img, rem = tile - n * a.per_img, ty = rem / a.tiles_x, tx = rem - ty * a.tiles_x;
+        const int r0 = ty * TR, c0 = tx * TC;
+        const int next = tile + gridDim.x;
+        const bool more = next < a.total_tiles;
+        f32x4 pre0 = {0.f, 0.f, 0.f, 0.f}, pre1 = pre0;
+        if (more) {
+            const int nn = next / a.per_img, nrem = next - nn * a.per_img, nty = nrem / a.tiles_x, ntx = nrem - nty * a.tiles_x;
+            pre0 = halo_entry(a.x, a.ldx, tid, nn, nty * TR, ntx * TC, a.H, a.W);
+            if (tid < HALO_ENTRIES - 256) pre1 = halo_entry(a.x, a.ldx, tid + 256, nn, nty * TR, ntx * TC, a.H, a.W);
+        }
+        float* hnext = halo + (cur ^ 1) * HALO_FLOATS;
+        auto put_next = [&]() {
+            if (more) {
+                *reinterpret_cast<f32x4*>(hnext + tid * 4) = pre0;
+                if (tid < HALO_ENTRIES - 256) *reinterpret_cast<f32x4*>(hnext + (tid + 256) * 4) = pre1;
+            }
+        };
+        const int hcur = cur * HALO_FLOATS, zero_slot = 2 * HALO_FLOATS;
+        float scnt = 0.f, smean[NT], sm2[NT];
+#pragma unroll
+        for (int t = 0; t < NT; ++t) { smean[t] = 0.f; sm2[t] = 0.f; }
 #pragma unroll 1
-    for (int seg = 0; seg < 2; ++seg) {
-        const int r = 2 * wid + seg;
-        if (r0 + r >= a.H) break;
-        const int base = (r * HC + li) * 4;
-        f32x16 acc[NT];
-#pragma unroll
-        for (int t = 0; t < NT; ++t)
-#pragma unroll
-            for (int i = 0; i < 16; ++i) acc[t][i] = 0.f;
-#pragma unroll
-        for (int s = 0; s < 16; ++s) {
-            const float av = halo[aoff[s] >= 0 ? base + aoff[s] : HALO_FLOATS];
-#pragma unroll
-            for (int t = 0; t < NT; ++t) acc[t] = __builtin_amdgcn_mfma_f32_32x32x2f32(av, breg[s][t], acc[t], 0, 0, 0);
-        }
-        const long rowpix = ((long)n * a.H + r0 + r) * a.W + c0;
-#pragma unroll
-        for (int t = 0; t < NT; ++t) {
-            float* y = t < n3 ? a.y3 : a.y1;
-            const int ldy = t < n3 ? a.ldy3 : a.ldy1;
-            const int ch = (t < n3 ? t : t - n3) * 32 + li;
-#pragma unroll
-            for (int i = 0; i < 16; ++i) {
-                const int m = (i & 3) + 8 * (i >> 2) + 4 * kk;
-                if (c0 + m < a.W) y[(rowpix + m) * ldy + ch] = acc[t][i];
-            }
-        }
+        for (int seg = 0; seg < 2; ++seg) {
+            const int r = 2 * wid + seg;
+            if (r0 + r >= a.H) break;
+            const int base = hcur + (r * HC + li) * 4;
+            const long rowpix = ((long)n * a.H + r0 + r) * a.W + c0;
+            float cnt = 0.f, nt = 0.f, f = 0.f, wgt = 0.f;
+            if (a.stats3) {
+#pragma unroll
+                for (int i = 0; i < 16; ++i) cnt += (c0 + (i & 3) + 8 * (i >> 2) + 4 * kk < a.W) ? 1.f : 0.f;
+                if (cnt > 0.f) { nt = scnt + cnt; f = cnt / nt; wgt = scnt * f; }
+            }
+#pragma unroll
+            for (int t0 = 0; t0 < NT; t0 += PT) {
+                f32x16 acc[PT];
+#pragma unroll
+                for (int t = 0; t < PT; ++t)
+#pragma unroll
+                    for (int i = 0; i < 16; ++i) acc[t][i] = 0.f;
+#pragma unroll
+                for (int s = 0; s < 16; ++s) {
+                    const float av = halo[aoff[s] >= 0 ? base + aoff[s] : zero_slot];
+#pragma unroll
+                    for (int t = 0; t < PT; ++t) acc[t] = __builtin_amdgcn_mfma_f32_32x32x2f32(av, breg[s][t0 + t], acc[t], 0, 0, 0);
+                }
+#pragma unroll
+                for (int t = 0; t < PT; ++t) {
+                    const int tt = t0 + t;
+                    float* y = tt < n3 ? a.y3 : a.y1;
+                    const int ldy = tt < n3 ? a.ldy3 : a.ldy1;
+                    const int ch = (tt < n3 ? tt : tt - n3) * 32 + li;
+#pragma unroll
+                    for (int i = 0; i < 16; ++i) {
+                        const int m = (i & 3) + 8 * (i >> 2) + 4 * kk;
+                        if (c0 + m < a.W) y[(rowpix + m) * ldy + ch] = acc[t][i];
+                    }
+                }
+                if (a.stats3 && cnt > 0.f) {
+#pragma unroll
+                    for (int t = 0; t < PT; ++t) {
+                        float s1 = 0.f, q = 0.f;
+#pragma unroll
+                        for (int i = 0; i < 16; ++i) s1 += (c0 + (i & 3) + 8 * (i >> 2) + 4 * kk < a.W) ? acc[t][i] : 0.f;
+                        const float mu = s1 / cnt;
+#pragma unroll
+                        for (int i = 0; i < 16; ++i) {
+                            const float d = acc[t][i] - mu;
+                            q += (c0 + (i & 3) + 8 * (i >> 2) + 4 * kk < a.W) ? d * d : 0.f;
+                        }
+                        const float dl = mu - smean[t0 + t];
+                        smean[t0 + t] += dl * f;
+                        sm2[t0 + t] += q + dl * dl * wgt;
+                    }
+                }
+            }
+            if (a.stats3 && cnt > 0.f) scnt = nt;
+        }
+        put_next();
+        float* xch = bmat + cur * XCH;
         if (a.stats3) {
-            float cnt = 0.f;
-#pragma unroll
-            for (int i = 0; i < 16; ++i) cnt += (c0 + (i & 3) + 8 * (i >> 2) + 4 * kk < a.W) ? 1.f : 0.f;
-            if (cnt > 0.f) {
-                const float nt = scnt + cnt, f = cnt / nt, wgt = scnt * f;
-#pragma unroll
-                for (int t = 0; t < NT; ++t) {
-                    float s1 = 0.f, q = 0.f;
-#pragma unroll
-                    for (int i = 0; i < 16; ++i) s1 += (c0 + (i & 3) + 8 * (i >> 2) + 4 * kk < a.W) ? acc[t][i] : 0.f;
-                    const float mu = s1 / cnt;
-#pragma unroll
-                    for (int i = 0; i < 16; ++i) {
-                        const float d = acc[t][i] - mu;
-                        q += (c0 + (i & 3) + 8 * (i >> 2) + 4 * kk < a.W) ? d * d : 0.f;
-                    }
-                    const float dl = mu - smean[t];
-                    smean[t] += dl * f;
-                    sm2[t] += q + dl * dl * wgt;
+            const float ocnt = __shfl_xor(scnt, 32, 64);
+#pragma unroll
+            for (int t = 0; t < NT; ++t) {
+                const float omean = __shfl_xor(smean[t], 32, 64), om2 = __shfl_xor(sm2[t], 32, 64);
+                const float nt = scnt + ocnt;
+                float mu = smean[t], q = sm2[t];
+                if (ocnt > 0.f) { const float f = ocnt / nt, dl = omean - mu; mu += dl * f; q += om2 + dl * dl * (scnt * f); }
+                if (kk == 0) { float* o = xch + ((wid * NT + t) * 32 + li) * 3; o[0] = nt; o[1] = mu; o[2] = q; }
+            }
+        }
+        __syncthreads();
+        if (a.stats3) {
+            for (int col = tid; col < NT * 32; col += 256) {
+                float cnt = 0.f, mu = 0.f, q = 0.f;
+                for (int wv = 0; wv < 4; ++wv) {
+                    const float* o = xch + (wv * NT * 32 + col) * 3;
+                    if (o[0] > 0.f) { const float nt = cnt + o[0], f = o[0] / nt, dl = o[1] - mu; mu += dl * f; q += o[2] + dl * dl * (cnt * f); cnt = nt; }
                 }
-                scnt = nt;
-            }
-        }
-    }
-    if (a.stats3) {
-        float* xch = bmat;
-        __syncthreads();
-        const float ocnt = __shfl_xor(scnt, 32, 64);
-#pragma unroll
-        for (int t = 0; t < NT; ++t) {
-            const float omean = __shfl_xor(smean[t], 32, 64), om2 = __shfl_xor(sm2[t], 32, 64);
-            const float nt = scnt + ocnt;
-            float mu = smean[t], q = sm2[t];
-            if (ocnt > 0.f) { const float f = ocnt / nt, dl = omean - mu; mu += dl * f; q += om2 + dl * dl * (scnt * f); }
-            if (kk == 0) { float* o = xch + ((wid * NT + t) * 32 + li) * 3; o[0] = nt; o[1] = mu; o[2] = q; }
-        }
-        __syncthreads();
-        for (int col = tid; col < NT * 32; col += 256) {
-            float cnt = 0.f, mu = 0.f, q = 0.f;
-            for (int wv = 0; wv < 4; ++wv) {
-                const float* o = xch + (wv * NT * 32 + col) * 3;
-                if (o[0] > 0.f) { const float nt = cnt + o[0], f = o[0] / nt, dl = o[1] - mu; mu += dl * f; q += o[2] + dl * dl * (cnt * f); cnt = nt; }
-            }
-            const int t = col >> 5;
-            float* dst = (t < n3 ? a.stats3 : a.stats1) + (((long)blockIdx.y * gridDim.x + blockIdx.x) * a.cout + (t < n3 ? t : t - n3) * 32 + (col & 31)) * 3;
-            dst[0] = cnt; dst[1] = mu; dst[2] = q;
+                const int t = col >> 5;
+                float* dst = (t < n3 ? a.stats3 : a.stats1) + ((long)tile * a.cout + (t < n3 ? t : t - n3) * 32 + (col & 31)) * 3;
+                dst[0] = cnt; dst[1] = mu; dst[2] = q;
+            }
         }
     }
 }
@@ -236,6 +287,20 @@
 
 int wgrad_blocks(int total_tiles) { return total_tiles < 1024 ? total_tiles : 1024; }
 
+int stem_conv_blocks(int total_tiles) {
+    static const int resident = [] {
+        int dev = 0, cus = 0;
+        if (hipGetDevice(&dev) != hipSuccess || hipDeviceGetAttribute(&cus, hipDeviceAttributeMultiprocessorCount, dev) != hipSuccess || cus < 1) cus = 256;
+        return 2 * cus;
+    }();
+    int blocks = resident;
+    if (const char* e = getenv("RUNET_STEM_CONV_BLOCKS")) {
+        const int v = atoi(e);
+        if (v >= 1) blocks = v;
+    }
+    return total_tiles < blocks ? total_tiles : blocks;
+}
+
 }
 
 extern "C" int runet_stem_supported(int cin_w, int cout) { return (cin_w >= 1 && cin_w <= 3 && cout % 32 == 0 && cout >= 32 && cout <= 64) ? 1 : 0; }
@@ -262,8 +327,10 @@
     RUNET_REQUIRE(runet_stem_supported(cin_w, cout), "stem kernel: 1..3 input channels, 32 or 64 output channels");
     RUNET_REQUIRE(ldx >= 4 && ldx % 4 == 0 && ((uintptr_t)x % 16) == 0, "x must be NHWC padded to (a multiple of) 4 channels, 16-byte aligned");
     RUNET_REQUIRE(n_img > 0 && h > 0 && w > 0 && ldy3 >= cout && (!w1 || ldy1 >= cout), "bad shape");
-    StemFwd a{x, ldx, w3, w1, y3, ldy3, y1, ldy1, h, w, cin_w, cout, stats3, stats1};
-    const dim3 grid(cdiv(h, TR) * cdiv(w, TC), n_img);
+    const int per_img = cdiv(h, TR) * cdiv(w, TC);
+    RUNET_REQUIRE((long)n_img * per_img < (1L << 31), "too many tiles");
+    StemFwd a{x, ldx, w3, w1, y3, ldy3, y1, ldy1, h, w, cin_w, cout, stats3, stats1, cdiv(w, TC), per_img, n_img * per_img};
+    const dim3 grid(stem_conv_blocks(a.total_tiles));
     const int nt = (cout / 32) * (w1 ? 2 : 1);
     hipStream_t st = (hipStream_t)stream;
     if (nt == 1) hipLaunchKernelGGL(stem_conv_kernel<1>, grid, dim3(256), 0, st, a);
diff --git a/eusipco-2026-robust-unet_amd/model.py b/eusipco-2026-robust-unet_amd/model.py
--- a/eusipco-2026-robust-unet_amd/model.py
+++ b/eusipco-2026-robust-unet_amd/model.py
@@ -482,12 +482,13 @@
         skips.append(cur)
     xd, C["bottleneck.1"] = B.dilated_forward(pooled, net.bottleneck[1].handles(), tr, save, hook)
     y, C["bottleneck.2"] = B.rb_forward(xd, rbs["bottleneck.2"].handles(), tr, masks["bottleneck.2"], save, hook)
+    w, b = ops.hwio(net.outc[0].weight), net.outc[0].bias
     for lvl in (4, 3, 2, 1):
         att, up = getattr(net, f"att{lvl}"), getattr(net, f"up{lvl}")
         cat, C[f"upgate{lvl}"] = B.upgate_forward(y, skips[lvl - 1], att.handles(up), tr, save, hook)
-        y, C[f"dec{lvl}"] = B.rb_forward(cat, rbs[f"dec{lvl}"].handles(), tr, masks[f"dec{lvl}"], save, hook)
-    w, b = ops.hwio(net.outc[0].weight), net.outc[0].bias
-    prob, logit = B.outc_forward(y, w, b, want_logit)
+        head = dict(w=w, b=b, want_logit=want_logit) if (lvl == 1 and B.fuses_head("fwd", rbs["dec1"].out_channels)) else None
+        y, C[f"dec{lvl}"] = B.rb_forward(cat, rbs[f"dec{lvl}"].handles(), tr, masks[f"dec{lvl}"], save, hook, head=head)
+    prob, logit = (head["prob"], head["logit"]) if head is not None else B.outc_forward(y, w, b, want_logit)
     if save:
         C["head"] = (y, w, prob)
         C["precision"] = net.precision
@@ -547,11 +548,13 @@
 
 def _net_backward(C, dprob, sink, done):
     y, w, prob = C["head"]
-    dy = B.outc_backward(dprob, prob, y, w, sink, pre="outc.0.")
+    rank1 = B.fuses_head("bwd", y.shape[3]) and C["dec1"].get("relu_bits") is not None
+    head_grad = (B.outc_backward_dl(dprob, prob, y, sink, pre="outc.0."), w) if rank1 else None
+    dy = None if rank1 else B.outc_backward(dprob, prob, y, w, sink, pre="outc.0.")
     done("outc.0")
     dskip = {}
     for lvl in (1, 2, 3, 4):
-        dcat = B.rb_backward(C[f"dec{lvl}"], dy, sink, pre=f"dec{lvl}.")
+        dcat = B.rb_backward(C[f"dec{lvl}"], dy, sink, pre=f"dec{lvl}.", head_grad=head_grad if lvl == 1 else None)
         done(f"dec{lvl}")
         dy, dskip[lvl] = B.upgate_backward(C[f"upgate{lvl}"], dcat, sink, f"att{lvl}.", f"up{lvl}.")
         done(f"up{lvl}")
diff --git a/include/runet_hip.h b/include/runet_hip.h
--- a/include/runet_hip.h
+++ b/include/runet_hip.h
@@ -87,6 +87,12 @@
 int runet_rb_bwd1_ex(const float* dout, int lddo, const float* dpool, int ldp, const unsigned char* pool_idx, const float* out, int ldo,
                      const unsigned char* relu_bits, const float* t2, int ld, const float* A, const float* B, const float* sa, float* dv,
                      int lddv, float* dq, int n_img, int h, int w, int c, void* stream);
+int runet_rb_out_head_supported(int c);
+int runet_rb_out_head(const float* t2, int ld, const float* A, const float* B, const float* sa, const float* r, int ldr, const float* rs,
+                      const float* rh, float* out, int ldo, unsigned char* relu_bits, const float* hw, const float* hb, float* logit,
+                      float* prob, int n_img, int h, int w, int c, void* stream);
+int runet_rb_bwd1_rank1(const float* dl, const float* hw, const unsigned char* relu_bits, const float* t2, int ld, const float* A,
+                        const float* B, const float* sa, float* dv, int lddv, float* dq, int n_img, int h, int w, int c, void* stream);
 long runet_sa_conv7_bwd_workspace_floats(int n_img, int h, int w);
 int runet_sa_conv7_bwd(const float* smap, const float* dq, const float* wp, float* dsm, float* dwp, float* workspace, int n_img, int h,
                        int w, void* stream);
@@ -126,6 +132,8 @@
 int runet_outc_fwd(const float* x, int ld, const float* w, const float* b, float* logit, float* prob, long pixels, int c, void* stream);
 int runet_outc_bwd(const float* dprob, const float* prob, const float* x, int ld, const float* w, float* dx, int lddx, float* workspace,
                    float* dw_db, long pixels, int c, void* stream);
+int runet_outc_bwd_dl(const float* dprob, const float* prob, const float* x, int ld, float* dl, float* workspace, float* dw_db,
+                      long pixels, int c, void* stream);
 
 int runet_maxpool2_fwd(const float* x, int ldx, float* y, int ldy, unsigned char* idx, int n_img, int h, int w, int c, void* stream);
 int runet_maxpool2_bwd(const float* dy, int lddy, const unsigned char* idx, float* dx, int lddx, int n_img, int h, int w, int c,
```

Result: faster. 612.5 images/s (median of 6 runs) (+1.1%).
